# RadiativeTransfer/RadiativeTransfer.jl

Hardware: AMD Instinct MI355X
Metric: spectral points/sec (whole node), O2-A band IQU scene (higher is better)
Workload: dtype f64; 1 GPU; C2: N=60 (20 streams x 3 Stokes), Nz=40, M=3, S=10000/GPU (10000 in total), sum(ndoubl)=185, Lambertian surface, 3 VZA; collective=none, devices=one GPU per rank

## Files before the change

### include/momcore.h

```cpp
#ifndef MOMCORE_H
#define MOMCORE_H

#include <stddef.h>

#ifdef __cplusplus
extern "C" {
#endif

typedef struct mom_handle mom_t;

enum {
  MOM_OK = 0,
  MOM_EINVAL = -1,
  MOM_EHIP = -2,
  MOM_ESTATE = -3,
  MOM_ESINGULAR = -4,
  MOM_EUNSUPPORTED = -5
};

enum {
  MOM_ADDED_R_PM = 0, MOM_ADDED_R_MP = 1, MOM_ADDED_T_MM = 2, MOM_ADDED_T_PP = 3,
  MOM_ADDED_J0P = 4, MOM_ADDED_J0M = 5,
  MOM_COMP_R_MP = 6, MOM_COMP_R_PM = 7, MOM_COMP_T_PP = 8, MOM_COMP_T_MM = 9,
  MOM_COMP_J0P = 10, MOM_COMP_J0M = 11,
  MOM_SURF_R_PM = 12, MOM_SURF_R_MP = 13, MOM_SURF_T_MM = 14, MOM_SURF_T_PP = 15,
  MOM_SURF_J0P = 16, MOM_SURF_J0M = 17
};


int mom_create(mom_t **out, int device, int N, int nStokes, int S, int max_m, int dtype);
int mom_destroy(mom_t *h);
const char *mom_last_error(const mom_t *h);
const char *mom_last_global_error(void);
int mom_sync(mom_t *h);
int mom_check(mom_t *h);

int mom_set_streams(mom_t *h, const double *qp_muN, const double *wt_muN, int N, int imu0_1based, double mu0,
                    const double *I0, const double *D, int strict_reference_indexing);


int mom_elemental(mom_t *h, int m, int ndoubl, const double *tau_sum, const double *dtau, const double *varpi,
                  const double *Zpp, const double *Zmp, int z_batch);

int mom_doubling(mom_t *h, int ndoubl, double *expk);

int mom_interaction(mom_t *h, int iface, int with_surface_layer);

int mom_copy_added_to_composite(mom_t *h);

int mom_surface_lambertian(mom_t *h, int m, double albedo, const double *tau_tot);

int mom_elemental_inelastic_rrs(mom_t *h, int m, int ndoubl, int nRaman, const int *i_l1l0, const double *varpi_l1l0,
                                const double *fscattRayl, const double *tau_sum, const double *dtau, const double *varpi,
                                const double *Zpp_l1l0, const double *Zmp_l1l0, double *ier_mp, double *iet_pp,
                                double *ier_pm, double *iet_mm, double *ieJ0p, double *ieJ0m);

enum {
  MOM_IE_ADDED_R_PM = 18, MOM_IE_ADDED_R_MP = 19, MOM_IE_ADDED_T_MM = 20, MOM_IE_ADDED_T_PP = 21,
  MOM_IE_ADDED_J0P = 22, MOM_IE_ADDED_J0M = 23,
  MOM_IE_COMP_R_MP = 24, MOM_IE_COMP_R_PM = 25, MOM_IE_COMP_T_PP = 26, MOM_IE_COMP_T_MM = 27,
  MOM_IE_COMP_J0P = 28, MOM_IE_COMP_J0M = 29
};
int mom_rrs_set(mom_t *h, int nRaman, const int *i_l1l0, const double *varpi_l1l0, int rrs_strict_reference);
int mom_rrs_set_shard(mom_t *h, int nSpec_global, int n_glob0, int n1_lo, int n1_hi);
int mom_rrs_elemental(mom_t *h, int m, int ndoubl, const double *tau_sum, const double *dtau, const double *varpi,
                      const double *Zpp, const double *Zmp, const double *fscattRayl, const double *Zpp_l1l0,
                      const double *Zmp_l1l0);
int mom_rrs_doubling(mom_t *h, int ndoubl, double *expk);
int mom_rrs_interaction(mom_t *h, int iface, int with_surface_layer);
int mom_rrs_copy_added_to_composite(mom_t *h);
int mom_rrs_surface_lambertian(mom_t *h, int m, double albedo, const double *tau_tot);
int mom_rrs_upload(mom_t *h, int which, const double *src);
int mom_rrs_download(mom_t *h, int which, double *dst);
int mom_scene_set_rrs(mom_t *h, const double *fscattRayl, const double *Zpp_l1l0, const double *Zmp_l1l0);
int mom_rt_run_rrs(mom_t *h);
int mom_get_RT_rrs(mom_t *h, double *R_SFI, double *T_SFI, double *ieR_SFI, double *ieT_SFI, double *gpu_ms);
int mom_get_hdr_rrs(mom_t *h, double *hdr, double *bhr_uw, double *bhr_dw);
int mom_rrs_timers(mom_t *h, double *ms, int *launches, int n);
int mom_rrs_check_padding(mom_t *h, unsigned long long *violations);
size_t mom_rrs_spectra_count(mom_t *h, int per);
int mom_get_spectra_rrs_device(mom_t *h, int per, void *d_local);
int mom_allgather_rrs_device(mom_t *h, int per, void *d_global);

int mom_batch_inv(mom_t *h, int n, int batch, const double *A, double *X);
int mom_batched_mul(mom_t *h, int n, int batch, const double *A, const double *B, double *C);
int mom_batched_mul_dual(mom_t *h, int n, int batch, int P, const double *A, const double *dA, const double *B,
                         const double *dB, double *C, double *dC);
int mom_batch_inv_dual(mom_t *h, int n, int batch, int P, const double *A, const double *dA, double *X, double *dX);

int mom_upload(mom_t *h, int which, const double *src);
int mom_download(mom_t *h, int which, double *dst);

int mom_postprocess(mom_t *h, int m, int nVza, const int *node_1based, const double *vaz_deg, double weight,
                    double *R_SFI, double *T_SFI);

int mom_scene_set(mom_t *h, int Nz, int K, int M, const double *tau, const double *varpi, const double *zw,
                  const double *Zpp, const double *Zmp, const int *ndoubl, const int *iface, const double *tau_sum,
                  double albedo, int nVza, const int *node_1based, const double *cos_mphi, const double *sin_mphi);

int mom_absorption_begin(mom_t *h, int Nz, const double *grid);
int mom_absorption_set_lines(mom_t *h, int nLines, const double *nu0, const double *S0, const double *gamma_air,
                             const double *gamma_self, const double *E_lower, const double *n_air, const double *delta_air,
                             const double *sqrt_mol_weight, const int *iso_index, int nIso, int nTmax, const int *nT,
                             const double *tips_T, const double *tips_Q, const double *tips_z);
int mom_voigt_tau_abs_layer(mom_t *h, int iz_1based, double pressure, double temperature, double vmr, double wing_cutoff,
                            double factor);
int mom_voigt_tau_abs_profile(mom_t *h, int Nz, const double *pressure, const double *temperature, double vmr, double wing_cutoff,
                              const double *factor, double *gpu_ms);
int mom_absorption_get_prefactors(mom_t *h, int n, double *nu, double *gamma_d, double *y, double *S, int *ind_start_1based,
                                  int *ind_stop_1based);
int mom_voigt_tau_abs(mom_t *h, int iz_1based, int nLines, const double *nu, const double *gamma_d, const double *y,
                      const double *S, const int *ind_start_1based, const int *ind_stop_1based, double factor);
int mom_absorption_set(mom_t *h, int Nz, const double *tau_abs);
int mom_absorption_get(mom_t *h, double *tau_abs);
int mom_voigt_tau_abs_dual(mom_t *h, int iz_1based, int nLines, const double *nu, const double *gamma_d, const double *y,
                           const double *S, const double *dnu, const double *dgamma_d, const double *dy, const double *dS,
                           const int *ind_start_1based, const int *ind_stop_1based, double factor);
int mom_voigt_tau_abs_profile_dual(mom_t *h, int Nz, const double *pressure, const double *temperature, double vmr,
                                   double wing_cutoff, const double *factor, double *gpu_ms);
int mom_absorption_get_partials(mom_t *h, double *dtau_abs);
int mom_absorption_get_prefactor_partials(mom_t *h, int n, double *dnu, double *dgamma_d, double *dy, double *dS);
enum { MOM_BROADENING_VOIGT = 0, MOM_BROADENING_DOPPLER = 1, MOM_BROADENING_LORENTZ = 2 };
enum { MOM_CEF_HW32SD = 0, MOM_CEF_HW32VOIGT = 1 };
int mom_absorption_set_model(mom_t *h, int broadening, int cef);
int mom_lineshape_tau_abs(mom_t *h, int iz_1based, int nLines, const double *nu, const double *gamma_d, const double *gamma_l,
                          const double *y, const double *S, const int *ind_start_1based, const int *ind_stop_1based, double factor);
int mom_lineshape_tau_abs_dual(mom_t *h, int iz_1based, int nLines, const double *nu, const double *gamma_d, const double *gamma_l,
                               const double *y, const double *S, const double *dnu, const double *dgamma_d, const double *dgamma_l,
                               const double *dy, const double *dS, const int *ind_start_1based, const int *ind_stop_1based,
                               double factor);
int mom_absorption_get_gamma_l(mom_t *h, int n, double *gamma_l, double *dgamma_l);
int mom_scene_set_optics(mom_t *h, int Nz, int nAer, int M, const double *tau_rayl, double varpi_rayl,
                         const double *tau_aer, const double *omega_aer, const double *ft_aer, const double *Zpp,
                         const double *Zmp, double albedo, int nVza, const int *node_1based, const double *cos_mphi,
                         const double *sin_mphi);
int mom_scene_get_layers(mom_t *h, int *ndoubl, int *iface, double *tau, double *varpi, double *zw, double *tau_sum);
int mom_scene_set_optics_bands(mom_t *h, int Nz, int nAer, int nBand, const int *band_start, int M, const double *tau_rayl,
                               const double *varpi_rayl, const double *tau_aer, const double *omega_aer, const double *ft_aer,
                               const double *Zpp, const double *Zmp, double albedo, int nVza, const int *node_1based,
                               const double *cos_mphi, const double *sin_mphi);

int mom_scene_set_surface(mom_t *h, int kind, int M, const double *Rsurf, const double *albedo_spec);

int mom_rt_run(mom_t *h);

int mom_scene_set_partials(mom_t *h, int P, const double *dtau, const double *dvarpi, const double *dzw, const double *dZpp,
                           const double *dZmp, const double *dalbedo, const double *dRsurf, const double *dalbedo_spec);
int mom_rt_run_dual(mom_t *h);
int mom_get_RT_partials(mom_t *h, double *dR_SFI, double *dT_SFI);
int mom_get_hdr_partials(mom_t *h, double *dhdr, double *dbhr_uw, double *dbhr_dw);
int mom_scene_set_optics_partials(mom_t *h, int P, const double *w_abs, const double *w_rayl, const double *dtau_aer,
                                  const double *domega_aer, const double *dft_aer, const double *dZpp, const double *dZmp,
                                  const double *dalbedo, const double *dRsurf, const double *dalbedo_spec);
int mom_scene_get_partials(mom_t *h, double *dtau, double *dvarpi, double *dzw);
int mom_scene_set_optics_bands_partials(mom_t *h, int P, const double *w_abs, const double *w_rayl, const double *dtau_aer,
                                        const double *domega_aer, const double *dft_aer, const double *dZpp, const double *dZmp,
                                        const double *dalbedo, const double *dRsurf, const double *dalbedo_spec);

int mom_rt_run_multisensor(mom_t *h, int nSensors, const int *sensor_levels, double *uwJ, double *dwJ);

int mom_get_RT(mom_t *h, double *R_SFI, double *T_SFI);
int mom_get_hdr(mom_t *h, double *hdr, double *bhr_uw, double *bhr_dw);
int mom_get_RT_device(mom_t *h, void *dR_SFI, void *dT_SFI);

enum { MOM_COMM_ID_BYTES = 128 };
int mom_comm_unique_id(void *id_out, size_t bytes);
int mom_comm_init(mom_t *h, int rank, int nranks, const void *nccl_id);
int mom_comm_destroy(mom_t *h);
int mom_allgather(mom_t *h, const void *d_local, void *d_global, size_t count);
int mom_allgather_RT_device(mom_t *h, void *d_global);
int mom_allgather_RT(mom_t *h, double *R_SFI_global, double *T_SFI_global);

int mom_timers(mom_t *h, double *ms, int n, int *kernel_launches);

int mom_set_option(mom_t *h, int option, int value);

int mom_strip2_resumed(mom_t *h, int *units, int *left);
enum { MOM_OPT_INVERSE = 0, MOM_OPT_FORCE_GENERIC = 1, MOM_OPT_M0_REDUCTION = 2, MOM_OPT_SMALL_WG = 3, MOM_OPT_STAGGER = 4,
       MOM_OPT_SMALL_N = 5, MOM_OPT_LAYER_SWEEP = 6, MOM_OPT_STRIP_PAD = 7, MOM_OPT_LEAN = 8, MOM_OPT_OVERLAP = 9,
       MOM_OPT_RRS_KERNELS = 10, MOM_OPT_DUAL_WORKSPACE_MB = 11, MOM_OPT_STRIP2 = 12, MOM_OPT_STRIP2_SCHED = 13,
       MOM_OPT_ZERO_SKIP = 14, MOM_OPT_LUT_BATCH = 15, MOM_OPT_SOURCES_ONLY = 16, MOM_OPT_ELEMENTAL = 17 };

int mom_lut_create(mom_t *h, int nNu, double nu_first, double nu_step, int nP, double p_first, double p_step, int nT, double t_first,
                   double t_step, int *lut);
int mom_lut_set_table(mom_t *h, int lut, const double *sigma);
int mom_lut_build(mom_t *h, int lut, double vmr, double wing_cutoff, double *gpu_ms);
int mom_lut_get_table(mom_t *h, int lut, double *sigma);
int mom_lut_get_coefficients(mom_t *h, int lut, double *c);
int mom_lut_xsec(mom_t *h, int lut, int n, const double *nu, double p, double T, double *sigma, double *J);
int mom_lut_tau_abs_profile(mom_t *h, int lut, int Nz, const double *pressure, const double *temperature, const double *factor,
                            double *gpu_ms);
int mom_lut_tau_abs_profile_dual(mom_t *h, int lut, int Nz, const double *pressure, const double *temperature, const double *factor,
                                 double *gpu_ms);
int mom_lut_destroy(mom_t *h, int lut);

int mom_voigt_xsec(int device, int nLines, const double *nu, const double *gamma_d, const double *y,
                   const double *S, const int *ind_start_1based, const int *ind_stop_1based, int nGrid,
                   const double *grid, double *sigma);

int mom_voigt_xsec_dual(int device, int nLines, const double *nu, const double *gamma_d, const double *y, const double *S,
                        const double *dnu, const double *dgamma_d, const double *dy, const double *dS,
                        const int *ind_start_1based, const int *ind_stop_1based, int nGrid, const double *grid,
                        double *sigma, double *dsigma);

int mom_lineshape_xsec(int device, int broadening, int cef, int nLines, const double *nu, const double *gamma_d,
                       const double *gamma_l, const double *y, const double *S, const int *ind_start_1based,
                       const int *ind_stop_1based, int nGrid, const double *grid, double *sigma);

int mom_lineshape_xsec_dual(int device, int broadening, int cef, int nLines, const double *nu, const double *gamma_d,
                            const double *gamma_l, const double *y, const double *S, const double *dnu,
                            const double *dgamma_d, const double *dgamma_l, const double *dy, const double *dS,
                            const int *ind_start_1based, const int *ind_stop_1based, int nGrid, const double *grid,
                            double *sigma, double *dsigma);

double mom_voigt_last_kernel_ms(void);

enum { MOM_MIE_MAX_WEIGHT_ROWS = 4, MOM_MIE_FULL_K = 1 };
int mom_mie_nai2(int device, int nR, const double *r, int nW, const double *w, double lambda, double n_r, double n_i,
                 int n_mu, const double *w_mu, int n_max, const double *pi_tab, const double *tau_tab, int l_max,
                 const double *P, const double *P2, const double *R2, const double *T2, int flags, double *bulk_f,
                 double *C, double *greek, double *gpu_ms);

int mom_mie_coefficients(int device, int nX, const double *x, double n_r, double n_i, int n_max, double *a_re, double *a_im,
                         double *b_re, double *b_im);

enum { MOM_MIE_DUAL_MAX_WEIGHT_ROWS = 3, MOM_MIE_INDEX_ROWS = 2 };
int mom_mie_nai2_dual(int device, int nR, const double *r, int nW, const double *w, double lambda, double n_r, double n_i,
                      int n_mu, const double *w_mu, int n_max, const double *pi_tab, const double *tau_tab, int l_max,
                      const double *P, const double *P2, const double *R2, const double *T2, int flags, double *bulk_f,
                      double *C, double *greek, double *gpu_ms);

int mom_mie_coefficients_dual(int device, int nX, const double *x, double n_r, double n_i, int n_max, double *a_re, double *a_im,
                              double *b_re, double *b_im, double *da_re, double *da_im, double *db_re, double *db_im);

int mom_mie_tables(int device, int n_mu, const double *mu, int n_max, int l_max, double *pi_tab, double *tau_tab, double *P,
                   double *P2, double *R2, double *T2);

int mom_mie_nai2_spectral(int device, int nR, const double *r, int nW, const double *w, int nL, const double *lambda,
                          const double *n_r, const double *n_i, int n_mu, const double *mu, const double *w_mu, int n_max,
                          int l_max, int flags, int max_batch, double *bulk_f, double *C, double *greek, double *gpu_ms);

int mom_mie_nai2_spectral_dual(int device, int nR, const double *r, int nW, const double *w, int nL, const double *lambda,
                               const double *n_r, const double *n_i, int n_mu, const double *mu, const double *w_mu, int n_max,
                               int l_max, int flags, int max_batch, double *bulk_f, double *C, double *greek, double *gpu_ms);

enum { MOM_PCW_MAX_ORDER = 640 };
int mom_mie_pcw(int device, int nR, const double *r, const double *w, double lambda, double n_r, double n_i, int N_max, int flags,
                double *greek, double *C, double *gpu_ms);

enum { MOM_WIGNER_MAX_TABLE_BYTES = 1073741824 };
int mom_wigner_tables(int device, int m_max, int n_max, int l_max, double *A, double *B);

int mom_pcw_pair_averages(int device, int nR, const double *r, const double *w, double lambda, double n_r, double n_i, int N_max,
                          double *anam_re, double *anam_im, double *anbm_re, double *anbm_im, double *bnam_re, double *bnam_im,
                          double *bnbm_re, double *bnbm_im);

int mom_z_moments(int device, int nStokes, int n_mu, const double *mu, int nG, int l_pad, const int *l_max, const double *greek,
                  int m_first, int M, int set_inner, double *Zpp, double *Zmp, double *gpu_ms);

int mom_scene_stage_greeks(mom_t *h, int which, int nG, int l_pad, const int *l_max, const double *greek, int M);
int mom_scene_stage_greek_partials(mom_t *h, int P, int nD, const int *basis, const int *partial, int l_pad, const int *l_max,
                                   const double *dgreek);
int mom_scene_get_bases(mom_t *h, int which, int *edge, int *blocks, double *Zpp, double *Zmp);

#ifdef __cplusplus
}
#endif
#endif
```

### radiativetransfer.jl_amd/_lib.py

```python
from __future__ import annotations

import ctypes as C
import os
from pathlib import Path

import numpy as np

PKG_DIR = Path(__file__).resolve().parent
LIB_PATH = Path(os.environ["MOM_LIBRARY"]) if os.environ.get("MOM_LIBRARY") else PKG_DIR / "libmomcore.so"

c_dp = C.POINTER(C.c_double)
c_ip = C.POINTER(C.c_int)
c_h = C.c_void_p

MOM_OK, MOM_EINVAL, MOM_EHIP, MOM_ESTATE, MOM_ESINGULAR, MOM_EUNSUPPORTED = 0, -1, -2, -3, -4, -5
_CODES = {MOM_EINVAL: "MOM_EINVAL", MOM_EHIP: "MOM_EHIP", MOM_ESTATE: "MOM_ESTATE", MOM_ESINGULAR: "MOM_ESINGULAR",
          MOM_EUNSUPPORTED: "MOM_EUNSUPPORTED"}

ADDED = dict(r_pm=0, r_mp=1, t_mm=2, t_pp=3, j0p=4, j0m=5)
COMP = dict(R_mp=6, R_pm=7, T_pp=8, T_mm=9, J0p=10, J0m=11)
SURF = dict(r_pm=12, r_mp=13, t_mm=14, t_pp=15, j0p=16, j0m=17)
IE_ADDED = dict(ier_pm=18, ier_mp=19, iet_mm=20, iet_pp=21, ieJ0p=22, ieJ0m=23)
IE_COMP = dict(ieR_mp=24, ieR_pm=25, ieT_pp=26, ieT_mm=27, ieJ0p=28, ieJ0m=29)

MOM_OPT_INVERSE, MOM_OPT_FORCE_GENERIC, MOM_OPT_M0_REDUCTION, MOM_OPT_SMALL_WG, MOM_OPT_STAGGER, MOM_OPT_SMALL_N, MOM_OPT_LAYER_SWEEP = 0, 1, 2, 3, 4, 5, 6
MOM_OPT_STRIP_PAD = 7
MOM_OPT_LEAN = 8
MOM_OPT_OVERLAP = 9
MOM_OPT_RRS_KERNELS = 10
MOM_OPT_DUAL_WORKSPACE_MB = 11
MOM_OPT_STRIP2 = 12
MOM_OPT_STRIP2_SCHED = 13
MOM_OPT_ZERO_SKIP = 14
MOM_OPT_LUT_BATCH = 15
MOM_OPT_SOURCES_ONLY = 16
MOM_OPT_ELEMENTAL = 17

BROADENING_VOIGT, BROADENING_DOPPLER, BROADENING_LORENTZ = 0, 1, 2
CEF_HW32SD, CEF_HW32VOIGT = 0, 1
MOM_MIE_FULL_K = 1
MOM_PCW_MAX_ORDER, MOM_WIGNER_MAX_TABLE_BYTES = 640, 1 << 30
MOM_MIE_DUAL_MAX_WEIGHT_ROWS, MOM_MIE_INDEX_ROWS = 3, 2


class MomError(RuntimeError):
    def __init__(self, code, msg):
        super().__init__(f"{_CODES.get(code, code)}: {msg}")
        self.code = code


SIGNATURES = {
    "mom_create": (C.c_int, [C.POINTER(c_h), C.c_int, C.c_int, C.c_int, C.c_int, C.c_int, C.c_int]),
    "mom_destroy": (C.c_int, [c_h]),
    "mom_last_error": (C.c_char_p, [c_h]),
    "mom_last_global_error": (C.c_char_p, []),
    "mom_sync": (C.c_int, [c_h]),
    "mom_check": (C.c_int, [c_h]),
    "mom_set_streams": (C.c_int, [c_h, c_dp, c_dp, C.c_int, C.c_int, C.c_double, c_dp, c_dp, C.c_int]),
    "mom_elemental": (C.c_int, [c_h, C.c_int, C.c_int, c_dp, c_dp, c_dp, c_dp, c_dp, C.c_int]),
    "mom_doubling": (C.c_int, [c_h, C.c_int, c_dp]),
    "mom_interaction": (C.c_int, [c_h, C.c_int, C.c_int]),
    "mom_copy_added_to_composite": (C.c_int, [c_h]),
    "mom_surface_lambertian": (C.c_int, [c_h, C.c_int, C.c_double, c_dp]),
    "mom_elemental_inelastic_rrs": (C.c_int, [c_h, C.c_int, C.c_int, C.c_int, c_ip] + [c_dp] * 13),
    "mom_rrs_set": (C.c_int, [c_h, C.c_int, c_ip, c_dp, C.c_int]),
    "mom_rrs_set_shard": (C.c_int, [c_h, C.c_int, C.c_int, C.c_int, C.c_int]),
    "mom_rrs_elemental": (C.c_int, [c_h, C.c_int, C.c_int] + [c_dp] * 8),
    "mom_rrs_doubling": (C.c_int, [c_h, C.c_int, c_dp]),
    "mom_rrs_interaction": (C.c_int, [c_h, C.c_int, C.c_int]),
    "mom_rrs_copy_added_to_composite": (C.c_int, [c_h]),
    "mom_rrs_surface_lambertian": (C.c_int, [c_h, C.c_int, C.c_double, c_dp]),
    "mom_rrs_upload": (C.c_int, [c_h, C.c_int, c_dp]),
    "mom_rrs_download": (C.c_int, [c_h, C.c_int, c_dp]),
    "mom_scene_set_rrs": (C.c_int, [c_h, c_dp, c_dp, c_dp]),
    "mom_rt_run_rrs": (C.c_int, [c_h]),
    "mom_get_RT_rrs": (C.c_int, [c_h, c_dp, c_dp, c_dp, c_dp, c_dp]),
    "mom_get_hdr_rrs": (C.c_int, [c_h, c_dp, c_dp, c_dp]),
    "mom_rrs_timers": (C.c_int, [c_h, c_dp, c_ip, C.c_int]),
    "mom_batch_inv": (C.c_int, [c_h, C.c_int, C.c_int, c_dp, c_dp]),
    "mom_batched_mul": (C.c_int, [c_h, C.c_int, C.c_int, c_dp, c_dp, c_dp]),
    "mom_batched_mul_dual": (C.c_int, [c_h, C.c_int, C.c_int, C.c_int, c_dp, c_dp, c_dp, c_dp, c_dp, c_dp]),
    "mom_batch_inv_dual": (C.c_int, [c_h, C.c_int, C.c_int, C.c_int, c_dp, c_dp, c_dp, c_dp]),
    "mom_upload": (C.c_int, [c_h, C.c_int, c_dp]),
    "mom_download": (C.c_int, [c_h, C.c_int, c_dp]),
    "mom_scene_set": (C.c_int, [c_h, C.c_int, C.c_int, C.c_int, c_dp, c_dp, c_dp, c_dp, c_dp, c_ip, c_ip, c_dp,
                                C.c_double, C.c_int, c_ip, c_dp, c_dp]),
    "mom_absorption_begin": (C.c_int, [c_h, C.c_int, c_dp]),
    "mom_absorption_set_lines": (C.c_int, [c_h, C.c_int] + [c_dp] * 8 + [c_ip, C.c_int, C.c_int, c_ip, c_dp, c_dp, c_dp]),
    "mom_voigt_tau_abs_layer": (C.c_int, [c_h, C.c_int, C.c_double, C.c_double, C.c_double, C.c_double, C.c_double]),
    "mom_voigt_tau_abs_profile": (C.c_int, [c_h, C.c_int, c_dp, c_dp, C.c_double, C.c_double, c_dp, c_dp]),
    "mom_absorption_get_prefactors": (C.c_int, [c_h, C.c_int, c_dp, c_dp, c_dp, c_dp, c_ip, c_ip]),
    "mom_voigt_tau_abs": (C.c_int, [c_h, C.c_int, C.c_int, c_dp, c_dp, c_dp, c_dp, c_ip, c_ip, C.c_double]),
    "mom_absorption_set": (C.c_int, [c_h, C.c_int, c_dp]),
    "mom_absorption_get": (C.c_int, [c_h, c_dp]),
    "mom_voigt_tau_abs_dual": (C.c_int, [c_h, C.c_int, C.c_int] + [c_dp] * 8 + [c_ip, c_ip, C.c_double]),
    "mom_voigt_tau_abs_profile_dual": (C.c_int, [c_h, C.c_int, c_dp, c_dp, C.c_double, C.c_double, c_dp, c_dp]),
    "mom_absorption_get_partials": (C.c_int, [c_h, c_dp]),
    "mom_absorption_get_prefactor_partials": (C.c_int, [c_h, C.c_int, c_dp, c_dp, c_dp, c_dp]),
    "mom_absorption_set_model": (C.c_int, [c_h, C.c_int, C.c_int]),
    "mom_lineshape_tau_abs": (C.c_int, [c_h, C.c_int, C.c_int] + [c_dp] * 5 + [c_ip, c_ip, C.c_double]),
    "mom_lineshape_tau_abs_dual": (C.c_int, [c_h, C.c_int, C.c_int] + [c_dp] * 10 + [c_ip, c_ip, C.c_double]),
    "mom_absorption_get_gamma_l": (C.c_int, [c_h, C.c_int, c_dp, c_dp]),
    "mom_scene_set_optics": (C.c_int, [c_h, C.c_int, C.c_int, C.c_int, c_dp, C.c_double, c_dp, c_dp, c_dp, c_dp, c_dp,
                                       C.c_double, C.c_int, c_ip, c_dp, c_dp]),
    "mom_scene_set_optics_bands": (C.c_int, [c_h, C.c_int, C.c_int, C.c_int, c_ip, C.c_int, c_dp, c_dp, c_dp, c_dp, c_dp, c_dp, c_dp,
                                             C.c_double, C.c_int, c_ip, c_dp, c_dp]),
    "mom_scene_set_optics_bands_partials": (C.c_int, [c_h, C.c_int] + [c_dp] * 10),
    "mom_scene_get_layers": (C.c_int, [c_h, c_ip, c_ip, c_dp, c_dp, c_dp, c_dp]),
    "mom_scene_set_surface": (C.c_int, [c_h, C.c_int, C.c_int, c_dp, c_dp]),
    "mom_rt_run": (C.c_int, [c_h]),
    "mom_scene_set_partials": (C.c_int, [c_h, C.c_int] + [c_dp] * 8),
    "mom_scene_set_optics_partials": (C.c_int, [c_h, C.c_int] + [c_dp] * 10),
    "mom_scene_get_partials": (C.c_int, [c_h, c_dp, c_dp, c_dp]),
    "mom_rt_run_dual": (C.c_int, [c_h]),
    "mom_get_RT_partials": (C.c_int, [c_h, c_dp, c_dp]),
    "mom_get_hdr_partials": (C.c_int, [c_h, c_dp, c_dp, c_dp]),
    "mom_rt_run_multisensor": (C.c_int, [c_h, C.c_int, c_ip, c_dp, c_dp]),
    "mom_get_RT": (C.c_int, [c_h, c_dp, c_dp]),
    "mom_get_hdr": (C.c_int, [c_h, c_dp, c_dp, c_dp]),
    "mom_get_RT_device": (C.c_int, [c_h, C.c_void_p, C.c_void_p]),
    "mom_postprocess": (C.c_int, [c_h, C.c_int, C.c_int, c_ip, c_dp, C.c_double, c_dp, c_dp]),
    "mom_comm_unique_id": (C.c_int, [C.c_void_p, C.c_size_t]),
    "mom_comm_init": (C.c_int, [c_h, C.c_int, C.c_int, C.c_void_p]),
    "mom_comm_destroy": (C.c_int, [c_h]),
    "mom_allgather": (C.c_int, [c_h, C.c_void_p, C.c_void_p, C.c_size_t]),
    "mom_rrs_check_padding": (C.c_int, [c_h, C.POINTER(C.c_ulonglong)]),
    "mom_rrs_spectra_count": (C.c_size_t, [c_h, C.c_int]),
    "mom_get_spectra_rrs_device": (C.c_int, [c_h, C.c_int, C.c_void_p]),
    "mom_allgather_rrs_device": (C.c_int, [c_h, C.c_int, C.c_void_p]),
    "mom_allgather_RT_device": (C.c_int, [c_h, C.c_void_p]),
    "mom_allgather_RT": (C.c_int, [c_h, c_dp, c_dp]),
    "mom_timers": (C.c_int, [c_h, c_dp, C.c_int, c_ip]),
    "mom_set_option": (C.c_int, [c_h, C.c_int, C.c_int]),
    "mom_strip2_resumed": (C.c_int, [c_h, c_ip, c_ip]),
    "mom_lut_create": (C.c_int, [c_h, C.c_int, C.c_double, C.c_double, C.c_int, C.c_double, C.c_double, C.c_int, C.c_double, C.c_double,
                                 c_ip]),
    "mom_lut_set_table": (C.c_int, [c_h, C.c_int, c_dp]),
    "mom_lut_build": (C.c_int, [c_h, C.c_int, C.c_double, C.c_double, c_dp]),
    "mom_lut_get_table": (C.c_int, [c_h, C.c_int, c_dp]),
    "mom_lut_get_coefficients": (C.c_int, [c_h, C.c_int, c_dp]),
    "mom_lut_xsec": (C.c_int, [c_h, C.c_int, C.c_int, c_dp, C.c_double, C.c_double, c_dp, c_dp]),
    "mom_lut_tau_abs_profile": (C.c_int, [c_h, C.c_int, C.c_int, c_dp, c_dp, c_dp, c_dp]),
    "mom_lut_tau_abs_profile_dual": (C.c_int, [c_h, C.c_int, C.c_int, c_dp, c_dp, c_dp, c_dp]),
    "mom_lut_destroy": (C.c_int, [c_h, C.c_int]),
    "mom_voigt_xsec": (C.c_int, [C.c_int, C.c_int, c_dp, c_dp, c_dp, c_dp, c_ip, c_ip, C.c_int, c_dp, c_dp]),
    "mom_voigt_xsec_dual": (C.c_int, [C.c_int, C.c_int] + [c_dp] * 8 + [c_ip, c_ip, C.c_int, c_dp, c_dp, c_dp]),
    "mom_lineshape_xsec": (C.c_int, [C.c_int, C.c_int, C.c_int, C.c_int] + [c_dp] * 5 + [c_ip, c_ip, C.c_int, c_dp, c_dp]),
    "mom_lineshape_xsec_dual": (C.c_int, [C.c_int, C.c_int, C.c_int, C.c_int] + [c_dp] * 10 + [c_ip, c_ip, C.c_int, c_dp, c_dp, c_dp]),
    "mom_voigt_last_kernel_ms": (C.c_double, []),
    "mom_mie_nai2": (C.c_int, [C.c_int, C.c_int, c_dp, C.c_int, c_dp, C.c_double, C.c_double, C.c_double, C.c_int, c_dp, C.c_int, c_dp,
                               c_dp, C.c_int, c_dp, c_dp, c_dp, c_dp, C.c_int, c_dp, c_dp, c_dp, c_dp]),
    "mom_mie_coefficients": (C.c_int, [C.c_int, C.c_int, c_dp, C.c_double, C.c_double, C.c_int, c_dp, c_dp, c_dp, c_dp]),
    "mom_mie_nai2_dual": (C.c_int, [C.c_int, C.c_int, c_dp, C.c_int, c_dp, C.c_double, C.c_double, C.c_double, C.c_int, c_dp, C.c_int,
                                    c_dp, c_dp, C.c_int, c_dp, c_dp, c_dp, c_dp, C.c_int, c_dp, c_dp, c_dp, c_dp]),
    "mom_mie_coefficients_dual": (C.c_int, [C.c_int, C.c_int, c_dp, C.c_double, C.c_double, C.c_int] + [c_dp] * 8),
    "mom_mie_tables": (C.c_int, [C.c_int, C.c_int, c_dp, C.c_int, C.c_int] + [c_dp] * 6),
    "mom_mie_nai2_spectral": (C.c_int, [C.c_int, C.c_int, c_dp, C.c_int, c_dp, C.c_int, c_dp, c_dp, c_dp, C.c_int, c_dp, c_dp, C.c_int,
                                        C.c_int, C.c_int, C.c_int, c_dp, c_dp, c_dp, c_dp]),
    "mom_mie_nai2_spectral_dual": (C.c_int, [C.c_int, C.c_int, c_dp, C.c_int, c_dp, C.c_int, c_dp, c_dp, c_dp, C.c_int, c_dp, c_dp,
                                             C.c_int, C.c_int, C.c_int, C.c_int, c_dp, c_dp, c_dp, c_dp]),
    "mom_mie_pcw": (C.c_int, [C.c_int, C.c_int, c_dp, c_dp, C.c_double, C.c_double, C.c_double, C.c_int, C.c_int, c_dp, c_dp, c_dp]),
    "mom_wigner_tables": (C.c_int, [C.c_int, C.c_int, C.c_int, C.c_int, c_dp, c_dp]),
    "mom_pcw_pair_averages": (C.c_int, [C.c_int, C.c_int, c_dp, c_dp, C.c_double, C.c_double, C.c_double, C.c_int] + [c_dp] * 8),
    "mom_z_moments": (C.c_int, [C.c_int, C.c_int, C.c_int, c_dp, C.c_int, C.c_int, c_ip, c_dp, C.c_int, C.c_int, C.c_int, c_dp, c_dp, c_dp]),
    "mom_scene_stage_greeks": (C.c_int, [c_h, C.c_int, C.c_int, C.c_int, c_ip, c_dp, C.c_int]),
    "mom_scene_stage_greek_partials": (C.c_int, [c_h, C.c_int, C.c_int, c_ip, c_ip, C.c_int, c_ip, c_dp]),
    "mom_scene_get_bases": (C.c_int, [c_h, C.c_int, c_ip, c_ip, c_dp, c_dp]),
}

_lib = None


def load():
    global _lib
    if _lib is not None:
        return _lib
    if not LIB_PATH.exists():
        raise MomError(MOM_EHIP, f"{LIB_PATH} not found - build it with `make -C {PKG_DIR / 'csrc'}` "
                                 "(hipcc --offload-arch=gfx950); there is no CPU fallback")
    lib = C.CDLL(str(LIB_PATH))
    for name, (res, args) in SIGNATURES.items():
        fn = getattr(lib, name)
        fn.restype = res
        fn.argtypes = args
    _lib = lib
    return lib


def f64(a):
    return np.ascontiguousarray(a, dtype=np.float64)


def i32(a):
    return np.ascontiguousarray(a, dtype=np.int32)


def dp(a: np.ndarray):
    assert a.dtype == np.float64 and a.flags["C_CONTIGUOUS"]
    return a.ctypes.data_as(c_dp)


def ip(a: np.ndarray):
    assert a.dtype == np.int32 and a.flags["C_CONTIGUOUS"]
    return a.ctypes.data_as(c_ip)


class Handle:

    def __init__(self, N: int, nStokes: int, S: int, max_m: int = 1, device: int = 0, dtype: int = 0):
        self.lib = load()
        self.N, self.nS, self.S, self.M = int(N), int(nStokes), int(S), int(max_m)
        self._h = c_h()
        rc = self.lib.mom_create(C.byref(self._h), device, self.N, self.nS, self.S, self.M, int(dtype))
        if rc != MOM_OK:
            msg = self.lib.mom_last_global_error().decode()
            if self._h:
                self.lib.mom_destroy(self._h)
                self._h = c_h()
            raise MomError(rc, msg)

    def check(self, rc):
        if rc != MOM_OK:
            raise MomError(rc, self.lib.mom_last_error(self._h).decode())

    def close(self):
        if getattr(self, "_h", None):
            self.lib.mom_destroy(self._h)
            self._h = c_h()

    def __del__(self):
        try:
            self.close()
        except Exception:
            pass

    def __enter__(self):
        return self

    def __exit__(self, *a):
        self.close()

    def set_option(self, option, value):
        self.check(self.lib.mom_set_option(self._h, option, value))

    def sync(self):
        self.check(self.lib.mom_sync(self._h))

    def check_async(self):
        self.check(self.lib.mom_check(self._h))

    def set_streams(self, qp_muN, wt_muN, imu0_1based, mu0, I0, D, strict=True):
        qp, wt, I0, D = f64(qp_muN), f64(wt_muN), f64(I0), f64(D)
        self.check(self.lib.mom_set_streams(self._h, dp(qp), dp(wt), len(qp), int(imu0_1based), float(mu0), dp(I0),
                                            dp(D), 1 if strict else 0))

    def elemental(self, m, nd, tau_sum, dtau, varpi, Zpp, Zmp, z_batch):
        a = [f64(x) for x in (tau_sum, dtau, varpi, Zpp, Zmp)]
        self.check(self.lib.mom_elemental(self._h, int(m), int(nd), *[dp(x) for x in a], int(z_batch)))

    def doubling(self, nd, expk):
        e = f64(expk).copy()
        self.check(self.lib.mom_doubling(self._h, int(nd), dp(e)))
        return e

    def interaction(self, iface, with_surface_layer=False):
        self.check(self.lib.mom_interaction(self._h, int(iface), 1 if with_surface_layer else 0))

    def copy_added_to_composite(self):
        self.check(self.lib.mom_copy_added_to_composite(self._h))

    def surface_lambertian(self, m, albedo, tau_tot):
        t = f64(tau_tot)
        self.check(self.lib.mom_surface_lambertian(self._h, int(m), float(albedo), dp(t)))

    def upload(self, which, src):
        s = f64(src).reshape(-1)
        self.check(self.lib.mom_upload(self._h, int(which), dp(s)))

    def download(self, which):
        k = which % 6
        out = np.empty((self.N * self.N if k < 4 else self.N) * self.S)
        self.check(self.lib.mom_download(self._h, int(which), dp(out)))
        return out

    def elemental_inelastic_rrs(self, m, ndoubl, i_l1l0, varpi_l1l0, fscatt, tau_sum, dtau, varpi, Zpp, Zmp):
        il = i32(i_l1l0)
        nR = len(il)
# ... 289 lines not shown
                               cos_mphi, sin_mphi):
        bs = i32(np.asarray(band_start).reshape(-1))
        nBand = bs.size - 1
        tr = np.ascontiguousarray(np.asarray(tau_rayl, dtype=np.float64).T).reshape(-1)
        ta = np.asarray(tau_aer, dtype=np.float64)
        nAer = ta.shape[1] if ta.ndim == 3 and ta.size else 0
        vr = f64(varpi_rayl).reshape(-1)
        taf = np.ascontiguousarray(ta.transpose(0, 2, 1)).reshape(-1) if nAer else np.zeros(1)
        om, ft = (f64(omega_aer).reshape(-1), f64(ft_aer).reshape(-1)) if nAer else (np.zeros(1), np.zeros(1))
        assert vr.size == max(nBand, 1) and (not nAer or (ta.shape[0] == nBand and om.size == ft.size == nBand * nAer))
        zp, zm = (None if z is None else dp(f64(z).reshape(-1)) for z in (Zpp, Zmp))
        node = i32(node)
        cm, sm = f64(cos_mphi).reshape(-1), f64(sin_mphi).reshape(-1)
        self.nVza = len(node)
        self._Nz, self._K = int(Nz), 1 + nAer * nBand
        self.check(self.lib.mom_scene_set_optics_bands(self._h, int(Nz), nAer, nBand, ip(bs), int(M), dp(tr), dp(vr), dp(taf), dp(om),
                                                       dp(ft), zp, zm, float(albedo), len(node), ip(node), dp(cm), dp(sm)))

    def scene_stage_greeks(self, greeks, M, which=0):
        nG, l_pad, l_max, greek = pack_greeks(greeks, "scene_stage_greeks")
        self.check(self.lib.mom_scene_stage_greeks(self._h, int(which), nG, l_pad, ip(l_max), dp(greek), int(M)))

    def scene_stage_greek_partials(self, P, pairs):
        nD, l_pad, l_max, greek = pack_greeks([g for _, g in pairs], "scene_stage_greek_partials")
        basis, partial = i32([kp[0] for kp, _ in pairs]), i32([kp[1] for kp, _ in pairs])
        self.check(self.lib.mom_scene_stage_greek_partials(self._h, int(P), nD, ip(basis), ip(partial), l_pad, ip(l_max), dp(greek)))

    def scene_get_bases(self, which=0):
        e, b = np.zeros(1, dtype=np.int32), np.zeros(1, dtype=np.int32)
        self.check(self.lib.mom_scene_get_bases(self._h, int(which), ip(e), ip(b), None, None))
        edge, blocks = int(e[0]), int(b[0])
        Zpp, Zmp = np.empty((blocks, edge, edge)), np.empty((blocks, edge, edge))
        if Zpp.size:
            self.check(self.lib.mom_scene_get_bases(self._h, int(which), ip(e), ip(b), dp(Zpp), dp(Zmp)))
        return edge, Zpp, Zmp

    def scene_get_layers(self, Nz, K, arrays=True):
        nd, iface = np.zeros(Nz, dtype=np.int32), np.zeros(Nz, dtype=np.int32)
        S = self.S
        bufs = [np.empty(S * Nz), np.empty(S * Nz), np.empty(K * S * Nz), np.empty(S * (Nz + 1))] if arrays else [None] * 4
        self.check(self.lib.mom_scene_get_layers(self._h, ip(nd), ip(iface), *[dp(b) if b is not None else None for b in bufs]))
        return (nd, iface) + tuple(bufs)

    def scene_set_surface(self, kind, M=0, Rsurf=None, albedo_spec=None):
        r = f64(Rsurf).reshape(-1) if Rsurf is not None else None
        al = f64(albedo_spec).reshape(-1) if albedo_spec is not None else None
        self.check(self.lib.mom_scene_set_surface(self._h, int(kind), int(M), dp(r) if r is not None else None,
                                                  dp(al) if al is not None else None))

    def rt_run(self):
        self.check(self.lib.mom_rt_run(self._h))

    def scene_set_partials(self, P, dtau=None, dvarpi=None, dzw=None, dZpp=None, dZmp=None, dalbedo=None, dRsurf=None,
                           dalbedo_spec=None):
        bufs = [None if x is None else f64(x).reshape(-1) for x in (dtau, dvarpi, dzw, dZpp, dZmp, dalbedo, dRsurf, dalbedo_spec)]
        self.dual_P = int(P)
        self.check(self.lib.mom_scene_set_partials(self._h, int(P), *[None if b is None else dp(b) for b in bufs]))

    def scene_set_optics_partials(self, P, w_abs=None, w_rayl=None, dtau_aer=None, domega_aer=None, dft_aer=None, dZpp=None,
                                  dZmp=None, dalbedo=None, dRsurf=None, dalbedo_spec=None):
        bufs = [None if x is None else f64(x).reshape(-1)
                for x in (w_abs, w_rayl, dtau_aer, domega_aer, dft_aer, dZpp, dZmp, dalbedo, dRsurf, dalbedo_spec)]
        self.check(self.lib.mom_scene_set_optics_partials(self._h, int(P), *[None if b is None else dp(b) for b in bufs]))
        self.dual_P = int(P)

    def scene_set_optics_bands_partials(self, P, w_abs=None, w_rayl=None, dtau_aer=None, domega_aer=None, dft_aer=None, dZpp=None,
                                        dZmp=None, dalbedo=None, dRsurf=None, dalbedo_spec=None):
        bufs = [None if x is None else f64(x).reshape(-1)
                for x in (w_abs, w_rayl, dtau_aer, domega_aer, dft_aer, dZpp, dZmp, dalbedo, dRsurf, dalbedo_spec)]
        self.check(self.lib.mom_scene_set_optics_bands_partials(self._h, int(P), *[None if b is None else dp(b) for b in bufs]))
        self.dual_P = int(P)

    def scene_get_partials(self):
        P, S, Nz, K = getattr(self, "dual_P", 0), self.S, getattr(self, "_Nz", 1), getattr(self, "_K", 1)
        n = max(P * S * Nz, 1)
        dt, dv, dz = np.empty(n), np.empty(n), np.empty(K * n)
        self.check(self.lib.mom_scene_get_partials(self._h, dp(dt), dp(dv), dp(dz)))
        tr = lambda a: np.transpose(a.reshape(P, Nz, S), (0, 2, 1)).copy()
        return tr(dt), tr(dv), np.transpose(dz.reshape(P, Nz, S, K), (0, 3, 2, 1)).copy()

    def rt_run_dual(self):
        self.check(self.lib.mom_rt_run_dual(self._h))

    def get_RT_partials(self):
        P = self.dual_P
        n = self.nVza * self.nS * self.S * P
        dR, dT = np.empty(n), np.empty(n)
        self.check(self.lib.mom_get_RT_partials(self._h, dp(dR), dp(dT)))
        shp = (P, self.S, self.nS, self.nVza)
        return np.transpose(dR.reshape(shp), (0, 3, 2, 1)).copy(), np.transpose(dT.reshape(shp), (0, 3, 2, 1)).copy()

    def get_hdr_partials(self):
        P = self.dual_P
        n, f = self.nVza * self.nS * self.S * P, self.nS * self.S * P
        dH, up, dw = np.empty(n), np.empty(f), np.empty(f)
        self.check(self.lib.mom_get_hdr_partials(self._h, dp(dH), dp(up), dp(dw)))
        tr = lambda x: np.transpose(x.reshape(P, self.S, self.nS), (0, 2, 1)).copy()
        return np.transpose(dH.reshape(P, self.S, self.nS, self.nVza), (0, 3, 2, 1)).copy(), tr(up), tr(dw)

    def rt_run_multisensor(self, sensor_levels):
        lv = np.ascontiguousarray(sensor_levels, dtype=np.int32)
        n = self.nVza * self.nS * self.S * len(lv)
        uw, dw = np.empty(n), np.empty(n)
        self.check(self.lib.mom_rt_run_multisensor(self._h, len(lv), ip(lv), dp(uw), dp(dw)))
        shp = (len(lv), self.S, self.nS, self.nVza)
        tr = lambda a: np.transpose(a.reshape(shp), (0, 3, 2, 1)).copy()
        return tr(uw), tr(dw)

    def get_RT(self):
        n = self.nVza * self.nS * self.S
        R, T = np.empty(n), np.empty(n)
        self.check(self.lib.mom_get_RT(self._h, dp(R), dp(T)))
        shp = (self.S, self.nS, self.nVza)
        return np.transpose(R.reshape(shp), (2, 1, 0)).copy(), np.transpose(T.reshape(shp), (2, 1, 0)).copy()

    def get_hdr(self):
        n = self.nVza * self.nS * self.S
        H, up, dw = np.empty(n), np.empty(self.nS * self.S), np.empty(self.nS * self.S)
        self.check(self.lib.mom_get_hdr(self._h, dp(H), dp(up), dp(dw)))
        return (np.transpose(H.reshape(self.S, self.nS, self.nVza), (2, 1, 0)).copy(),
                up.reshape(self.S, self.nS).T.copy(), dw.reshape(self.S, self.nS).T.copy())

    def get_RT_device(self, dR_ptr: int, dT_ptr: int):
        self.check(self.lib.mom_get_RT_device(self._h, C.c_void_p(dR_ptr), C.c_void_p(dT_ptr)))

    def postprocess(self, m, node_1based, vaz_deg, weight, R_SFI, T_SFI):
        node, vaz = i32(node_1based), f64(vaz_deg)
        self.check(self.lib.mom_postprocess(self._h, int(m), len(node), ip(node), dp(vaz), float(weight), dp(R_SFI),
                                            dp(T_SFI)))

    def comm_init(self, rank: int, nranks: int, nccl_id: bytes):
        buf = C.create_string_buffer(bytes(nccl_id), COMM_ID_BYTES)
        self.check(self.lib.mom_comm_init(self._h, int(rank), int(nranks), C.cast(buf, C.c_void_p)))
        self.comm_size = int(nranks)

    def comm_destroy(self):
        self.check(self.lib.mom_comm_destroy(self._h))

    def allgather_RT_device(self, d_global_ptr: int):
        self.check(self.lib.mom_allgather_RT_device(self._h, C.c_void_p(d_global_ptr)))

    def allgather_RT(self):
        n = self.nVza * self.nS * self.S * self.comm_size
        R, T = np.empty(n), np.empty(n)
        self.check(self.lib.mom_allgather_RT(self._h, dp(R), dp(T)))
        shp = (self.S * self.comm_size, self.nS, self.nVza)
        return np.transpose(R.reshape(shp), (2, 1, 0)).copy(), np.transpose(T.reshape(shp), (2, 1, 0)).copy()

    def strip2_resumed(self):
        u, l = C.c_int(0), C.c_int(0)
        self.check(self.lib.mom_strip2_resumed(self._h, C.byref(u), C.byref(l)))
        return u.value, l.value

    def timers(self):
        ms = np.zeros(8)
        nl = C.c_int(0)
        self.check(self.lib.mom_timers(self._h, dp(ms), 8, C.byref(nl)))
        return dict(layers_ms=ms[0], surface_ms=ms[1], postprocess_ms=ms[2], total_ms=ms[3], layer_launches=nl.value,
                    full_layers_ms=ms[4], reduced_layers_ms=ms[5], full_launches=int(ms[6]), reduced_launches=int(ms[7]))


COMM_ID_BYTES = 128


def comm_unique_id() -> bytes:
    buf = C.create_string_buffer(COMM_ID_BYTES)
    rc = load().mom_comm_unique_id(C.cast(buf, C.c_void_p), COMM_ID_BYTES)
    if rc != MOM_OK:
        raise MomError(rc, load().mom_last_global_error().decode())
    return buf.raw


def voigt_xsec(nu, gamma_d, y, S, ind_start, ind_stop, grid, device: int = 0):
    lib = load()
    a = [f64(x) for x in (nu, gamma_d, y, S)]
    i0, i1, g = i32(ind_start), i32(ind_stop), f64(grid)
    sigma = np.empty(len(g))
    rc = lib.mom_voigt_xsec(device, len(a[0]), *[dp(x) for x in a], ip(i0), ip(i1), len(g), dp(g), dp(sigma))
    if rc != MOM_OK:
        raise MomError(rc, lib.mom_last_global_error().decode())
    return sigma


def _partials(x, n):
    if x is None:
        return None
    x = np.asarray(x, dtype=np.float64)
    assert x.shape == (n, 2), f"partials must be [nLines, 2], got {x.shape}"
    return np.ascontiguousarray(x.T).reshape(-1)


def voigt_xsec_dual(nu, gamma_d, y, S, dnu, dgamma_d, dy, dS, ind_start, ind_stop, grid, device: int = 0):
    lib = load()
    a = [f64(x) for x in (nu, gamma_d, y, S)]
    d = [_partials(x, len(a[0])) for x in (dnu, dgamma_d, dy, dS)]
    i0, i1, g = i32(ind_start), i32(ind_stop), f64(grid)
    sigma, dsigma = np.empty(len(g)), np.empty(2 * len(g))
    rc = lib.mom_voigt_xsec_dual(device, len(a[0]), *[dp(x) for x in a], *[None if x is None else dp(x) for x in d], ip(i0), ip(i1),
                                 len(g), dp(g), dp(sigma), dp(dsigma))
    if rc != MOM_OK:
        raise MomError(rc, lib.mom_last_global_error().decode())
    return sigma, dsigma.reshape(2, len(g)).T.copy()


def lineshape_xsec(broadening, cef, nu, gamma_d, gamma_l, y, S, ind_start, ind_stop, grid, device: int = 0):
    lib = load()
    a = [None if x is None else f64(x) for x in (nu, gamma_d, gamma_l, y, S)]
    i0, i1, g = i32(ind_start), i32(ind_stop), f64(grid)
    sigma = np.empty(len(g))
    rc = lib.mom_lineshape_xsec(device, int(broadening), int(cef), len(a[0]), *[None if x is None else dp(x) for x in a], ip(i0),
                                ip(i1), len(g), dp(g), dp(sigma))
    if rc != MOM_OK:
        raise MomError(rc, lib.mom_last_global_error().decode())
    return sigma


def lineshape_xsec_dual(broadening, cef, nu, gamma_d, gamma_l, y, S, dnu, dgamma_d, dgamma_l, dy, dS, ind_start, ind_stop, grid,
                        device: int = 0):
    lib = load()
    a = [None if x is None else f64(x) for x in (nu, gamma_d, gamma_l, y, S)]
    d = [_partials(x, len(a[0])) for x in (dnu, dgamma_d, dgamma_l, dy, dS)]
    i0, i1, g = i32(ind_start), i32(ind_stop), f64(grid)
    sigma, dsigma = np.empty(len(g)), np.empty(2 * len(g))
    rc = lib.mom_lineshape_xsec_dual(device, int(broadening), int(cef), len(a[0]), *[None if x is None else dp(x) for x in a],
                                     *[None if x is None else dp(x) for x in d], ip(i0), ip(i1), len(g), dp(g), dp(sigma), dp(dsigma))
    if rc != MOM_OK:
        raise MomError(rc, lib.mom_last_global_error().decode())
    return sigma, dsigma.reshape(2, len(g)).T.copy()


def voigt_last_kernel_ms() -> float:
    return float(load().mom_voigt_last_kernel_ms())


def _mie_nai2(dual: bool, r, w, lam, n_r, n_i, w_mu, pi_tab, tau_tab, P, P2, R2, T2, flags, device):
    lib = load()
    name = "mie_nai2_dual" if dual else "mie_nai2"
    r, w, w_mu = f64(r), f64(np.atleast_2d(w)), f64(w_mu)
    tabs = [f64(np.asarray(t, dtype=np.float64).T) for t in (pi_tab, tau_tab, P, P2, R2, T2)]
    nW, nR, n_mu = w.shape[0], len(r), len(w_mu)
    if w.shape[1] != nR or any(t.shape[1] != n_mu for t in tabs) or tabs[0].shape != tabs[1].shape or \
            any(t.shape != tabs[2].shape for t in tabs[3:]):
        raise ValueError(f"{name}: array shapes do not agree")
    n_max, l_max = tabs[0].shape[0], tabs[2].shape[0]
    nO = nW + MOM_MIE_INDEX_ROWS if dual else nW
    bulk, Cx, greek, ms = np.empty((nO, 4, n_mu)), np.empty((nO, 2)), np.empty((nO, 6, l_max)), np.zeros(3)
    fn = lib.mom_mie_nai2_dual if dual else lib.mom_mie_nai2
    rc = fn(device, nR, dp(r), nW, dp(w), float(lam), float(n_r), float(n_i), n_mu, dp(w_mu), n_max, dp(tabs[0]), dp(tabs[1]), l_max,
            *[dp(t) for t in tabs[2:]], int(flags), dp(bulk), dp(Cx), dp(greek), dp(ms))
    if rc != MOM_OK:
        raise MomError(rc, lib.mom_last_global_error().decode())
    return bulk, Cx, greek, ms


def mie_nai2(r, w, lam, n_r, n_i, w_mu, pi_tab, tau_tab, P, P2, R2, T2, flags: int = 0, device: int = 0):
    return _mie_nai2(False, r, w, lam, n_r, n_i, w_mu, pi_tab, tau_tab, P, P2, R2, T2, flags, device)


def mie_nai2_dual(r, w, lam, n_r, n_i, w_mu, pi_tab, tau_tab, P, P2, R2, T2, flags: int = 0, device: int = 0):
    return _mie_nai2(True, r, w, lam, n_r, n_i, w_mu, pi_tab, tau_tab, P, P2, R2, T2, flags, device)


def mie_coefficients(x, n_r, n_i, n_max: int, device: int = 0):
    lib = load()
    x = f64(np.atleast_1d(x))
    out = [np.empty((int(n_max), len(x))) for _ in range(4)]
    rc = lib.mom_mie_coefficients(device, len(x), dp(x), float(n_r), float(n_i), int(n_max), *[dp(o) for o in out])
    if rc != MOM_OK:
        raise MomError(rc, lib.mom_last_global_error().decode())
    return out[0] + 1j * out[1], out[2] + 1j * out[3]


def mie_coefficients_dual(x, n_r, n_i, n_max: int, device: int = 0):
    lib = load()
    x = f64(np.atleast_1d(x))
    out = [np.empty((int(n_max), len(x))) for _ in range(8)]
    rc = lib.mom_mie_coefficients_dual(device, len(x), dp(x), float(n_r), float(n_i), int(n_max), *[dp(o) for o in out])
    if rc != MOM_OK:
        raise MomError(rc, lib.mom_last_global_error().decode())
    return out[0] + 1j * out[1], out[2] + 1j * out[3], out[4] + 1j * out[5], out[6] + 1j * out[7]


def mie_tables(mu, n_max: int, l_max: int, device: int = 0):
    lib = load()
    mu = f64(np.atleast_1d(mu))
    n_mu, n_max, l_max = len(mu), int(n_max), int(l_max)
    out = [np.empty((max(n_max, 0), n_mu)) for _ in range(2)] + [np.empty((max(l_max, 0), n_mu)) for _ in range(4)]
    rc = lib.mom_mie_tables(device, n_mu, dp(mu), n_max, l_max, *[dp(o) for o in out])
    if rc != MOM_OK:
        raise MomError(rc, lib.mom_last_global_error().decode())
    return tuple(o.T for o in out)


def _mie_nai2_spectral(dual: bool, r, w, lam, n_r, n_i, mu, w_mu, n_max, l_max, flags, max_batch, device):
    lib = load()
    name = "mie_nai2_spectral_dual" if dual else "mie_nai2_spectral"
    r, w, mu, w_mu = f64(r), f64(np.atleast_2d(w)), f64(mu), f64(w_mu)
    lam, n_r, n_i = (f64(np.atleast_1d(a)) for a in (lam, n_r, n_i))
    nW, nR, n_mu, nL, l_max = w.shape[0], len(r), len(w_mu), len(lam), int(l_max)
    if w.shape[1] != nR or len(mu) != n_mu or len(n_r) != nL or len(n_i) != nL:
        raise ValueError(f"{name}: array shapes do not agree")
    nO = nW + MOM_MIE_INDEX_ROWS if dual else nW
    bulk, Cx = np.empty((nL, nO, 4, n_mu)), np.empty((nL, nO, 2))
    greek, ms = np.empty((nL, nO, 6, max(l_max, 0))), np.zeros(4)
    fn = lib.mom_mie_nai2_spectral_dual if dual else lib.mom_mie_nai2_spectral
    rc = fn(device, nR, dp(r), nW, dp(w), nL, dp(lam), dp(n_r), dp(n_i), n_mu, dp(mu), dp(w_mu), int(n_max), l_max, int(flags),
# ... 83 lines not shown
```

### radiativetransfer.jl_amd/csrc/mom_handle.hpp

```cpp
#pragma once
#include <hip/hip_runtime.h>

#include <algorithm>
#include <cmath>
#include <cstdio>
#include <cstdlib>
#include <string>
#include <vector>

#include "momcore.h"

#include "mom_diag.hpp"
#include "mom_entry.hpp"
#include "mom_host.hpp"

namespace momr { struct State; }

struct MomLut {
  bool live = false;
  int n[3] = {};
  double first[3] = {}, step[3] = {};
  bool has_table = false, has_coef = false;
  MomDevBuf<double> d_table;
  MomDevBuf<double> d_coef;
  MomDevBuf<double> d_nu;
};

struct MomGreekStage {
  bool live = false;
  int nG = 0, l_pad = 0, M = 0, P = 0;
  std::vector<int> l_max, basis, partial;
  std::vector<double> greek;
  void drop() { *this = MomGreekStage{}; }
};

struct mom_handle : MomSceneBufs<double> {
  int device = 0, N = 0, nS = 0, S = 0, M = 0;
  int dtype = 0;
  momf_scene *f32 = nullptr;
  bool lds_mode = true;
  int opt_inverse = 0, opt_force_generic = 0;
  hipStream_t stream = nullptr;
  mom::DevStreams q{};
  bool streams_set = false;
  std::vector<double> h_mu, h_wt;
  int strict = 1;
  MomDevBuf<double> added[6], surf[6], comp[6];
  bool op_layers = false;
  bool comp_pitched = false;
  bool comp_on_chip = false;
  MomDevBuf<double> d_post;
  void *comm = nullptr;
  int comm_rank = 0, comm_size = 1;
  MomDevBuf<double> d_gather;
  MomDevBuf<double> d_rrs_send;
  MomDevBuf<double> d_tau_abs, d_grid, d_lines, d_tau_rayl, d_layer_max, d_aer;
  MomDevBuf<int> d_aer_mode;
  int abs_Nz = 0;
  size_t lines_per = 0;
  int lines_nz = 1;
  int abs_broadening = 0, abs_cef = 0;
  MomDevBuf<double> d_prof;
  MomDevBuf<double> d_dtau_abs;
  MomDevBuf<double> d_dlines;
  bool optics_scene = false;
  bool optics_tables = false;
  int optics_nAer = 0;
  int optics_nBand = 0;
  std::vector<double> h_varpi_rayl;
  std::vector<double> h_tau_aer, h_omega_aer, h_ft_aer;
  MomDevBuf<int> d_band_start;
  MomDevBuf<double> d_varpi_band;
  MomDevBuf<double> d_optics_prm;
  MomDevBuf<double> d_vec[4];
  MomDevBuf<double> d_Zop[2];
  bool scene_set = false;
  MomGreekStage stage_z, stage_r, stage_d;
  int opt_m0 = 1;
  int opt_w4 = 1;
  int opt_stagger = 1;
  int opt_rrs_kernels = -1;
  int opt_overlap = 1;
  hipStream_t stream2 = nullptr;
  hipEvent_t ev_fork = nullptr, ev_join = nullptr, ev_go = nullptr;
  int dual_P = 0;
  bool dual_ran = false;
  MomDevBuf<double> d_dual_in[8];
  MomDevBuf<double> d_dual_out, d_dual_ts;
  MomDevBuf<char> dual_work;
  size_t opt_dual_budget = 0;
  MomDevBuf<double> d_Rsurf0;
  int opt_sweep = 1;
  MomDevBuf<double> comp_top[6];
  MomDevBuf<double> d_msJ[2];
  std::vector<MomDevBuf<double>> ms_comp;
  MomDevBuf<double> d_ms_out;
  int opt_pad = 1;
  int opt_lean = 3;
  MomDevBuf<int> d_resume;
  int opt_strip2 = 1;
  MomDevBuf<int> d_resume2;
  size_t resume2_units = 0;
  int resume2_nz = 0;
  int opt_strip2_sched = 1;
  MomDevBuf<int> d_sched2;
  int opt_zero_skip = 7;
  int opt_sources_only = 1;
  int opt_elemental = 1;
  MomDevBuf<double> d_etab, d_etab0;
  int nbw_0 = 0;
  int Nk = 0;
  mom::DevStreams qk{};
  int opt_small = 1;
  bool red0 = false;
  int N0 = 0, nS0 = 0;
  mom::DevStreams q0{};
  MomDevBuf<double> d_mu0, d_wt0, d_sg0, d_Zpp0, d_Zmp0, d_hdrJ0, d_scratch0;
  MomDevBuf<double> comp0[6];
  int G = 0;
  int num_cu = 256;
  MomDevBuf<int> d_info;
  hipEvent_t ev[4] = {};
  hipEvent_t ev_voigt[2] = {};
  std::vector<hipEvent_t> ev_full, ev_red;
  int launches = 0, launches_full = 0, launches_red = 0;
  momr::State *rrs = nullptr;
  MomDevBuf<double> d_fscatt, d_Zr[2];
  MomDevBuf<double> d_rrs_op[8];
  bool rrs_scene = false;
  double rrs_ms = 0.0;
  MomDevBuf<char> ws[4];
  MomLineTable lt{};
  MomDevBuf<double> d_lt;
  MomDevBuf<int> d_lt_i;
  double lt_Tmin = 0.0, lt_Tmax = 0.0;
  std::vector<MomLut> luts;
  MomDevBuf<double> d_lut_cp;
  MomDevBuf<double> d_lut_prm;
  MomDevBuf<double> d_lut_io;
  int opt_lut_batch = 0;
  double grid_min = 0.0, grid_max = 0.0;
  int grid_order = 0;
  std::string err;
};

#pragma GCC visibility push(hidden)
int fail(mom_t *h, int code, const char *msg);
int check_info(mom_t *h);
inline int mom_absorption_state(mom_t *h, const char *fn, bool table, bool lines) {
  const bool no_table = table && (!h->d_tau_abs || !h->d_grid);
  if (!no_table && !(lines && !h->d_lt)) return MOM_OK;
  char buf[200];
  snprintf(buf, sizeof buf, no_table ? "%s: call mom_absorption_begin with the spectral grid first" : "%s: call mom_absorption_set_lines first", fn);
  return fail(h, MOM_ESTATE, buf);
}
inline int mom_tips_range(mom_t *h, double T) {
  if (h->lt.nIso <= 0 || (h->lt_Tmin < T && T < h->lt_Tmax)) return MOM_OK;
  char buf[160];
  snprintf(buf, sizeof buf, "TIPS2017: T (%g) must be between %g K and %g K.", T, h->lt_Tmin, h->lt_Tmax);
  return fail(h, MOM_EINVAL, buf);
}
hipError_t mom_launch_combine(const mom::InterArgs &a, bool lds, int grid, size_t smem, hipStream_t st);
int scene_common(mom_t *h, int Nz, int K, int M, const double *Zpp, const double *Zmp, double albedo, int nVza,
                 const int *node_1based, const double *cos_mphi, const double *sin_mphi);
int mom_stage_claim(mom_t *h, const char *fn, int K, int M);
extern void (*g_rccl_destroy)(void *);
int mom_comm_allreduce_max(mom_t *h, double *d_buf, size_t count);
#pragma GCC visibility pop

#define HIPCHK(h, call)                                                                            \
  do {                                                                                             \
    hipError_t e__ = (call);                                                                       \
    if (e__ != hipSuccess) {                                                                       \
      char buf__[512];                                                                             \
      snprintf(buf__, sizeof buf__, "%s failed: %s (%s:%d)", #call, hipGetErrorString(e__), __FILE__, __LINE__); \
      return fail(h, MOM_EHIP, buf__);                                                             \
    }                                                                                              \
  } while (0)

#define F64_ONLY(h, name)                                                                                 \
  if ((h) && (h)->dtype != 0)                                                                             \
  return fail(h, MOM_EINVAL, name ": not available on a Float32 (dtype = 1) handle (scene-level path only)")
```

### radiativetransfer.jl_amd/csrc/mom_image_variants.hpp

```cpp
#pragma once
#include "mom_images.hpp"

constexpr int kSkipVariants = 4;
constexpr int kS2Skip[kSkipVariants] = {0, 1, 2, 3};
constexpr int kQ4Skip[kSkipVariants] = {0, 1, 2, 4};

inline int mom_skip_variant(const int (&skip)[kSkipVariants], int KS, int nbw) {
  if (nbw < 1 || nbw > KS) return 0;
  int v = 0;
  for (int c = 1; c < kSkipVariants; ++c)
    if (KS - skip[c] >= nbw) v = c;
  return v;
}
constexpr bool s2_row_blocks_change(int KS, int KW) { return KW < KS || 4 * ((KS + 3) / 4) - 1 > KS; }
inline bool s2_row_blocks_for(int KS, const MomLaunchForm &f) {
  return f.row_blocks && s2_row_blocks_change(KS, KS - kS2Skip[mom_skip_variant(kS2Skip, KS, f.nbw)]);
}
```

### radiativetransfer.jl_amd/csrc/mom_images.hpp

```cpp
#pragma once
#include <hip/hip_runtime.h>

#include <cstddef>

struct MomLaunchForm {
  int nbw = 0;
  bool row_blocks = false;
  bool sources_only = false;
  bool elemental_tab = false;
  int sched_mode = 0;
};

struct MomLayerImage {
  int N;
  hipError_t (*launch)(const void *layer_args, const MomLaunchForm &form, int grid, hipStream_t st);
  size_t (*lds_bytes)(int ns, int nS, int K);
  int (*per_cu)();
};

enum MomImageFamily {
  MOM_IMG_STRIP8,
  MOM_IMG_STRIP4,
  MOM_IMG_LEAN,
  MOM_IMG_LEAN6,
  MOM_IMG_STRIP2,
  MOM_IMG_QUAD,
  MOM_IMG_F32_STRIP8,
  MOM_IMG_F32_STRIP4,
};

#define MOM_IMAGE_LIST(X)                                                                                \
  X(STRIP8, 11) X(STRIP8, 13) X(STRIP8, 14) X(STRIP8, 15)                                               \
  X(STRIP4, 9) X(STRIP4, 10) X(STRIP4, 11)                                                              \
  X(LEAN, 9) X(LEAN, 10)                                                                                \
  X(LEAN6, 9) X(LEAN6, 10)                                                                              \
  X(STRIP2, 13) X(STRIP2, 14) X(STRIP2, 15)                                                             \
  X(QUAD, 5) X(QUAD, 6) X(QUAD, 7) X(QUAD, 8) X(QUAD, 9) X(QUAD, 10)                                    \
  X(F32_STRIP8, 11) X(F32_STRIP8, 13) X(F32_STRIP8, 14) X(F32_STRIP8, 15)                               \
  X(F32_STRIP4, 9) X(F32_STRIP4, 10) X(F32_STRIP4, 11) X(F32_STRIP4, 13) X(F32_STRIP4, 14) X(F32_STRIP4, 15)

#define MOM_IMAGE_SYM_(F, KS) mom_image_##F##_##KS
#define MOM_IMAGE_SYM(F, KS) MOM_IMAGE_SYM_(F, KS)
#define MOM_DEFINE_IMAGE(F, KS, ...)                                 \
  const MomLayerImage *MOM_IMAGE_SYM(F, KS)() {                      \
    static const MomLayerImage image = {4 * (KS), __VA_ARGS__};      \
    return &image;                                                   \
  }

#define MOM_IMAGE_DECL(F, KS) const MomLayerImage *MOM_IMAGE_SYM_(F, KS)();
MOM_IMAGE_LIST(MOM_IMAGE_DECL)
#undef MOM_IMAGE_DECL

inline const MomLayerImage *mom_find_image(MomImageFamily family, int N) {
  struct Entry { MomImageFamily family; const MomLayerImage *image; };
#define MOM_IMAGE_ENTRY(F, KS) {MOM_IMG_##F, MOM_IMAGE_SYM_(F, KS)()},
  static const Entry all[] = {MOM_IMAGE_LIST(MOM_IMAGE_ENTRY)};
#undef MOM_IMAGE_ENTRY
  for (const Entry &e : all)
    if (e.family == family && e.image->N == N) return e.image;
  return nullptr;
}

constexpr size_t kMomStrip2SchedInts = 1 + 2048;
```

### radiativetransfer.jl_amd/csrc/mom_q4.hpp

```cpp
#pragma once
#include "mom_entry.hpp"
#include "mom_elemental_tab.hpp"

namespace MOM_NS {

static_assert(kWaves == 1, "mom_q4.hpp: one wavefront per workgroup (-DMOM_WAVES=1)");

__device__ __forceinline__ real mma4(real a, real b, real c) { return __builtin_amdgcn_mfma_f64_4x4x4f64(a, b, c, 0, 0, 0); }

#ifndef Q4_MUL_VARIANT
#define Q4_MUL_VARIANT 0
#endif
template <int KS>
struct Q4Geom {
  static constexpr int N = 4 * KS, NB = KS, NJ = (KS + 3) / 4, LD = N;
  static constexpr int CP = 16 * ((N + 15) / 16);
};
__host__ __device__ inline size_t q4_lds_bytes(int N) { return ((size_t)3 * N * N + 8 * (size_t)N) * sizeof(real); }
__host__ __device__ inline bool q4_applies(int N, int ns, int K) {
  const int Nq = N / (ns > 0 ? ns : 1);
  return kF64 && N >= 20 && N <= 40 && N % 4 == 0 && ns >= 2 && N % ns == 0 && K <= 60 &&
         3 * Nq * Nq + 2 * ns * N + 3 + K <= N * N &&
         4 * q4_lds_bytes(N) <= kLdsPerCU;
}

struct Q4Lane {
  int k, c16;
  __device__ __forceinline__ Q4Lane() {
    int l = wg_lane();
    asm volatile("" : "+v"(l));
    k = l >> 4;
    c16 = l & 15;
  }
};

template <int KS> using Q4Mat = real[Q4Geom<KS>::NB][Q4Geom<KS>::NJ];

template <int KS>
__device__ __forceinline__ void q4_zero(real (&W)[Q4Geom<KS>::NB][Q4Geom<KS>::NJ]) {
#pragma unroll
  for (int K = 0; K < Q4Geom<KS>::NB; ++K)
#pragma unroll
    for (int J = 0; J < Q4Geom<KS>::NJ; ++J) W[K][J] = 0.0;
}
template <int KS>
__device__ __forceinline__ void q4_copy(real (&D)[Q4Geom<KS>::NB][Q4Geom<KS>::NJ], const real (&S)[Q4Geom<KS>::NB][Q4Geom<KS>::NJ]) {
#pragma unroll
  for (int K = 0; K < Q4Geom<KS>::NB; ++K)
#pragma unroll
    for (int J = 0; J < Q4Geom<KS>::NJ; ++J) D[K][J] = S[K][J];
}

template <int KS>
__device__ __forceinline__ void q4_load_T(const real *X, const Q4Lane &q, real (&W)[Q4Geom<KS>::NB][Q4Geom<KS>::NJ]) {
  using G = Q4Geom<KS>;
  const real *base = X + q.c16 + q.k * G::LD;
#pragma unroll
  for (int K = 0; K < G::NB; ++K)
#pragma unroll
    for (int J = 0; J < G::NJ; ++J) W[K][J] = (16 * J + q.c16 < G::N) ? base[16 * J + 4 * K * G::LD] : 0.0;
}
template <int KS>
__device__ __forceinline__ void q4_store_T(real *X, const Q4Lane &q, const real (&W)[Q4Geom<KS>::NB][Q4Geom<KS>::NJ]) {
  using G = Q4Geom<KS>;
  real *base = X + q.c16 + q.k * G::LD;
#pragma unroll
  for (int K = 0; K < G::NB; ++K)
#pragma unroll
    for (int J = 0; J < G::NJ; ++J)
      if (16 * J + q.c16 < G::N) base[16 * J + 4 * K * G::LD] = W[K][J];
}
template <int KS>
__device__ __forceinline__ void q4_load_glb_T(const gdouble *__restrict__ X, const Q4Lane &q, real (&W)[Q4Geom<KS>::NB][Q4Geom<KS>::NJ]) {
  using G = Q4Geom<KS>;
  const gdouble *base = X + q.c16 + q.k * G::CP;
#pragma unroll
  for (int K = 0; K < G::NB; ++K)
#pragma unroll
    for (int J = 0; J < G::NJ; ++J) W[K][J] = (16 * J + q.c16 < G::N) ? MOM_NT_LOAD(base + 16 * J + 4 * K * G::CP) : 0.0;
}
template <int KS>
__device__ __forceinline__ void q4_store_glb_T(gdouble *__restrict__ X, const Q4Lane &q, const real (&W)[Q4Geom<KS>::NB][Q4Geom<KS>::NJ]) {
  using G = Q4Geom<KS>;
  gdouble *base = X + q.c16 + q.k * G::CP;
#pragma unroll
  for (int K = 0; K < G::NB; ++K)
#pragma unroll
    for (int J = 0; J < G::NJ; ++J)
      if (16 * J + q.c16 < G::N) MOM_NT_STORE(W[K][J], base + 16 * J + 4 * K * G::CP);
}

template <int KS, int NV = 0, bool ZERO = false, int NBW = Q4Geom<KS>::NB>
__device__ __forceinline__ void q4_mul_c(const real *M, const real (&X)[Q4Geom<KS>::NB][Q4Geom<KS>::NJ],
                                         const real (&C0)[Q4Geom<KS>::NB][Q4Geom<KS>::NJ],
                                         real (&acc)[Q4Geom<KS>::NB][Q4Geom<KS>::NJ], const real *ride = nullptr,
                                         real (*accR)[Q4Geom<KS>::NJ] = nullptr) {
  using G = Q4Geom<KS>;
  static_assert(NBW >= 1 && NBW <= G::NB, "q4_mul_c: 1 <= NBW <= NB");
  constexpr int NZ = G::NB - NBW;
  int l = wg_lane();
  asm volatile("" : "+v"(l));
  const int k = l >> 4, i = l & 3;
  const real *base = M + k + i * G::LD;
#define Q4_XLIVE(K, J) ((K) < NBW || (J) == ((K) >> 2))
#if Q4_MUL_VARIANT == 2
#pragma unroll
  for (int I = 0; I < G::NB; ++I) {
    if (I >= NBW) {
#pragma unroll
      for (int J = 0; J < G::NJ; ++J) acc[I][J] = ZERO ? (real)0 : C0[I][J];
    }
#pragma unroll
    for (int K = 0; K < G::NB; ++K) {
      if (I >= NBW && K != I) continue;
      const real a = base[4 * K + 4 * I * G::LD];
#pragma unroll
      for (int J = 0; J < G::NJ; ++J)
        if (Q4_XLIVE(K, J)) acc[I][J] = mma4(a, X[K][J], (I < NBW && K == 0) ? (ZERO ? (real)0 : C0[I][J]) : acc[I][J]);
    }
  }
  if constexpr (NV > 0) {
    const real *rb = ride + k + i * G::N;
#pragma unroll
    for (int K = 0; K < G::NB; ++K) {
      const real a = (i < NV) ? rb[4 * K] : 0.0;
#pragma unroll
      for (int J = 0; J < G::NJ; ++J)
        if (Q4_XLIVE(K, J)) (*accR)[J] = mma4(a, X[K][J], (*accR)[J]);
    }
  }
  return;
#endif
  constexpr int NP = (NBW + 1) / 2;
  real an[2][G::NB];
  const real *rb = NV > 0 ? ride + k + i * G::N : nullptr;
#pragma unroll
  for (int h = 0; h < 2; ++h)
#pragma unroll
    for (int K = 0; K < G::NB; ++K) {
      if (h < NBW) an[h][K] = base[4 * K + 4 * h * G::LD];
      else if (NV > 0 && h == NBW) an[h][K] = (i < NV) ? rb[4 * K] : 0.0;
      else an[h][K] = 0.0;
    }
  real ad[NZ > 0 ? NZ : 1];
#pragma unroll
  for (int d = 0; d < NZ; ++d) ad[d] = base[4 * (NBW + d) + 4 * (NBW + d) * G::LD];
#pragma unroll
  for (int Pp = 0; Pp < NP; ++Pp) {
    const int I0 = 2 * Pp;
    const bool two = I0 + 1 < NBW;
    real ac[2][G::NB];
#pragma unroll
    for (int h = 0; h < 2; ++h)
#pragma unroll
      for (int K = 0; K < G::NB; ++K) ac[h][K] = an[h][K];
#pragma unroll
    for (int h = 0; h < 2; ++h) {
      const int In = I0 + 2 + h;
      if (In < NBW) {
#pragma unroll
        for (int K = 0; K < G::NB; ++K) an[h][K] = base[4 * K + 4 * In * G::LD];
      } else if (NV > 0 && In == NBW) {
#pragma unroll
        for (int K = 0; K < G::NB; ++K) an[h][K] = (i < NV) ? rb[4 * K] : 0.0;
      }
    }
#if Q4_MUL_VARIANT != 1
    __builtin_amdgcn_sched_barrier(0);
#endif
#pragma unroll
    for (int K = 0; K < G::NB; ++K) {
#pragma unroll
      for (int J = 0; J < G::NJ; ++J)
        if (Q4_XLIVE(K, J)) acc[I0][J] = mma4(ac[0][K], X[K][J], K == 0 ? (ZERO ? (real)0 : C0[I0][J]) : acc[I0][J]);
      if (two) {
#pragma unroll
        for (int J = 0; J < G::NJ; ++J)
          if (Q4_XLIVE(K, J)) acc[I0 + 1][J] = mma4(ac[1][K], X[K][J], K == 0 ? (ZERO ? (real)0 : C0[I0 + 1][J]) : acc[I0 + 1][J]);
      } else if (NV > 0) {
#pragma unroll
        for (int J = 0; J < G::NJ; ++J)
          if (Q4_XLIVE(K, J)) (*accR)[J] = mma4(ac[1][K], X[K][J], (*accR)[J]);
      }
    }
#if Q4_MUL_VARIANT != 1
    __builtin_amdgcn_sched_barrier(0);
#endif
  }
  if constexpr (NV > 0 && (NBW % 2) == 0) {
#pragma unroll
    for (int K = 0; K < G::NB; ++K) {
#pragma unroll
      for (int J = 0; J < G::NJ; ++J)
        if (Q4_XLIVE(K, J)) (*accR)[J] = mma4(an[0][K], X[K][J], (*accR)[J]);
    }
  }
#pragma unroll
  for (int d = 0; d < NZ; ++d) {
    const int I = NBW + d;
#pragma unroll
    for (int J = 0; J < G::NJ; ++J) {
      const real c0 = ZERO ? (real)0 : C0[I][J];
      acc[I][J] = (J == (I >> 2)) ? mma4(ad[d], X[I][J], c0) : c0;
    }
  }
#undef Q4_XLIVE
}

template <int KS, int NV, int NBW = Q4Geom<KS>::NB>
__device__ __forceinline__ void q4_ride(const real *ride, const real (&X)[Q4Geom<KS>::NB][Q4Geom<KS>::NJ], real (&accR)[Q4Geom<KS>::NJ]) {
  using G = Q4Geom<KS>;
  static_assert(NV >= 1 && NBW >= 1 && NBW <= G::NB, "q4_ride: NV >= 1, 1 <= NBW <= NB");
  int l = wg_lane();
  asm volatile("" : "+v"(l));
  const int k = l >> 4, i = l & 3;
  const real *rb = ride + k + i * G::N;
  real a[G::NB];
#pragma unroll
  for (int K = 0; K < G::NB; ++K) a[K] = (i < NV) ? rb[4 * K] : 0.0;
#pragma unroll
  for (int K = 0; K < G::NB; ++K)
#pragma unroll
    for (int J = 0; J < G::NJ; ++J)
      if (K < NBW || J == (K >> 2)) accR[J] = mma4(a[K], X[K][J], accR[J]);
}

template <int KS, int NV = 0, int NBW = Q4Geom<KS>::NB>
__device__ __forceinline__ void q4_mul(const real *M, const real (&X)[Q4Geom<KS>::NB][Q4Geom<KS>::NJ],
                                       real (&acc)[Q4Geom<KS>::NB][Q4Geom<KS>::NJ], const real *ride = nullptr,
                                       real (*accR)[Q4Geom<KS>::NJ] = nullptr) {
  q4_mul_c<KS, NV, false, NBW>(M, X, acc, acc, ride, accR);
}
template <int KS, int NV = 0, int NBW = Q4Geom<KS>::NB>
__device__ __forceinline__ void q4_mul_z(const real *M, const real (&X)[Q4Geom<KS>::NB][Q4Geom<KS>::NJ],
                                         real (&acc)[Q4Geom<KS>::NB][Q4Geom<KS>::NJ], const real *ride = nullptr,
                                         real (*accR)[Q4Geom<KS>::NJ] = nullptr) {
  q4_mul_c<KS, NV, true, NBW>(M, X, acc, acc, ride, accR);
}

#ifndef Q4_HORNER_SITES
#define Q4_HORNER_SITES 1
#endif
template <int KS, int NBW = Q4Geom<KS>::NB>
__device__ __forceinline__ void q4_horner(const real *M, const real (&C0)[Q4Geom<KS>::NB][Q4Geom<KS>::NJ], int p,
                                          real (&Y)[Q4Geom<KS>::NB][Q4Geom<KS>::NJ]) {
  q4_copy<KS>(Y, C0);
  MOM_STAMP(82);
#if Q4_HORNER_SITES == 2
  int n = p - 1;
#pragma nounroll
  for (; n >= 2; n -= 2) {
    real Z[Q4Geom<KS>::NB][Q4Geom<KS>::NJ];
    q4_mul_c<KS, 0, false, NBW>(M, Y, C0, Z);
    q4_mul_c<KS, 0, false, NBW>(M, Z, C0, Y);
  }
  if (n == 1) {
    real acc[Q4Geom<KS>::NB][Q4Geom<KS>::NJ];
    q4_mul_c<KS, 0, false, NBW>(M, Y, C0, acc);
    q4_copy<KS>(Y, acc);
  }
#else
#pragma nounroll
  for (int kk = 1; kk < p; ++kk) {
    real acc[Q4Geom<KS>::NB][Q4Geom<KS>::NJ];
    MOM_STAMP(74);
    q4_mul_c<KS, 0, false, NBW>(M, Y, C0, acc);
#ifdef MOM_DIAG_STAMPS
    if (kk == 1) { MOM_STAMP(75); } else { MOM_STAMP(77); }
    if (threadIdx.x == 0 && blockIdx.x == (gridDim.x >> 1)) mom_diag_acc[kk == 1 ? 78 : 79] += 1;
#endif
    q4_copy<KS>(Y, acc);
    MOM_STAMP(76);
  }
#endif
}

template <int KS>
__device__ __forceinline__ unsigned q4_sign_mask(const real *sg, const Q4Lane &q) {
  unsigned m = 0;
#pragma unroll
  for (int K = 0; K < Q4Geom<KS>::NB; ++K)
    if (sg[4 * K + q.k] < 0.0) m |= 1u << K;
  return m;
}
template <int KS>
__device__ __forceinline__ void q4_flip(real (&W)[Q4Geom<KS>::NB][Q4Geom<KS>::NJ], unsigned mask) {
#pragma unroll
  for (int K = 0; K < Q4Geom<KS>::NB; ++K)
#pragma unroll
    for (int J = 0; J < Q4Geom<KS>::NJ; ++J) {
      const real v = W[K][J];
      W[K][J] = ((mask >> K) & 1u) ? -v : v;
    }
}
__device__ __forceinline__ void q4_fence() { __builtin_amdgcn_fence(__ATOMIC_ACQ_REL, "workgroup"); __builtin_amdgcn_s_barrier(); }

__device__ __forceinline__ real q4_wave_sum(real v) {
  union { real d; int w[2]; } a, b;
#define Q4_DPP_ADD(ctrl)                                                                      \
  a.d = v;                                                                                    \
  b.w[0] = __builtin_amdgcn_update_dpp(0, a.w[0], ctrl, 0xf, 0xf, false);                     \
  b.w[1] = __builtin_amdgcn_update_dpp(0, a.w[1], ctrl, 0xf, 0xf, false);                     \
  v += b.d;
  Q4_DPP_ADD(0x111)
  Q4_DPP_ADD(0x112)
  Q4_DPP_ADD(0x114)
  Q4_DPP_ADD(0x118)
#undef Q4_DPP_ADD
  a.d = v;
  real s = 0.0;
#pragma unroll
  for (int row = 0; row < 4; ++row) {
    union { real d; int w[2]; } t;
    t.w[0] = __builtin_amdgcn_readlane(a.w[0], 16 * row + 15);
    t.w[1] = __builtin_amdgcn_readlane(a.w[1], 16 * row + 15);
    s += t.d;
  }
  return s;
}

__device__ __forceinline__ void make_ctx_q4(Ctx &c, int N, int inv_mode, real *smem) {
  c.N = N; c.Np = N; c.nc = N; c.ld = N; c.ldv = N;
  c.fd.init(N);
  c.inv_mode = inv_mode;
  c.qpre = 0; c.slot = 0; c.ptab = nullptr;
  const size_t msz = (size_t)N * N;
  c.r = smem; c.t = smem + msz; c.P = smem + 2 * msz; c.Q = nullptr; c.X = nullptr;
  real *p = smem + 3 * msz;
  c.mu = p; c.wt = p + N; c.sg = p + 2 * N; c.jp = p + 3 * N; c.jm = p + 4 * N; c.ei = p + 5 * N; c.v1 = p + 6 * N; c.v2 = p + 7 * N;
  c.j1p = c.j1m = c.Jp = c.Jm = c.prow = c.pcol = c.rowk = c.part = c.thr = nullptr;
  c.ipiv = c.sh = nullptr;
  c.bad = reinterpret_cast<int *>(c.P + msz - 2);
  c.tabE = c.tabZS = nullptr;
}

template <int KS, int NBW = Q4Geom<KS>::NB>
__device__ __forceinline__ real doubling_run_q4(Ctx &c, int nd, real expk, bool &bail) {
  using G = Q4Geom<KS>;
  constexpr int N = G::N, NB = G::NB, NJ = G::NJ;
  bail = false;
  if (nd == 0) return expk;
  const Q4Lane q;
  real *r = c.r, *t = c.t, *P = c.P;
  for (int it = 0; it < nd; ++it) {
    real rj[NJ];
    real ss = 0.0;
    real Rn[NB][NJ], T0[NB][NJ];
    q4_load_T<KS>(r, q, Rn);
    q4_load_T<KS>(t, q, T0);
    {
      real B[NB][NJ];
#pragma unroll
      for (int J = 0; J < NJ; ++J) rj[J] = 0.0;
      q4_mul_z<KS, 2, NBW>(r, Rn, B, c.jp, &rj);
#pragma unroll
      for (int K = 0; K < NB; ++K)
#pragma unroll
        for (int J = 0; J < NJ; ++J) ss += B[K][J] * B[K][J];
      q4_store_T<KS>(P, q, B);
    }
    MOM_STAMP(70);
    ss = q4_wave_sum(ss);
    const int p = __builtin_amdgcn_readfirstlane(neumann_terms_12(ss));
    if (p > kStripMaxP || c.inv_mode != 0) {
      bail = true;
      return expk;
    }
    MOM_STAMP(80);
#pragma unroll
    for (int J = 0; J < NJ; ++J) {
      const int col = 16 * J + q.c16;
      if (col < N) {
        if (q.k == 0) c.ei[col] = c.jm[col] * expk + rj[J];
        if (q.k == 1) c.v1[col] = c.jp[col] + expk * rj[J];
      }
    }
    q4_fence();
    MOM_STAMP(81);
    real Y[NB][NJ];
    q4_horner<KS, NBW>(P, T0, p, Y);
    MOM_STAMP(71);
    real aw[NJ];
    real Tn[NB][NJ];
    {
      real Zt[NB][NJ];
#pragma unroll
      for (int J = 0; J < NJ; ++J) aw[J] = 0.0;
      q4_mul_z<KS, 2, NBW>(r, Y, Zt, c.ei, &aw);
      q4_mul<KS, 0, NBW>(t, Zt, Rn);
    }
    q4_mul_z<KS, 0, NBW>(t, Y, Tn);
    const bool last = (it == nd - 1);
#pragma unroll
    for (int J = 0; J < NJ; ++J) {
      const int col = 16 * J + q.c16;
      const real sc = (last && col < N) ? c.sg[col] : 1.0;
#pragma unroll
      for (int K = 0; K < NB; ++K) Rn[K][J] = Rn[K][J] * sc;
      if (col < N) {
        if (q.k == 0) c.jm[col] = (c.jm[col] + aw[J]) * sc;
        if (q.k == 1) c.jp[col] = c.jp[col] * expk + aw[J];
      }
    }
    q4_store_T<KS>(r, q, Rn);
    q4_store_T<KS>(t, q, Tn);
    q4_fence();
    MOM_STAMP(72);
    expk = expk * expk;
  }
  MOM_STAMP(73);
  return expk;
}

template <int KS, int NBW = Q4Geom<KS>::NB, bool SRC = false>
__device__ __forceinline__ bool interaction_q4(Ctx &c, const CompPtrs &g) {
  using G = Q4Geom<KS>;
  constexpr int N = G::N, NB = G::NB, NJ = G::NJ, NN = N * N;
  const Q4Lane q;
  const int lane = wg_lane();
  real *r = c.r, *t = c.t, *P = c.P;
  {
    constexpr int U = (NN + 63) / 64;
    real vr[U];
#pragma unroll
    for (int u = 0; u < U; ++u) {
      const int e = lane + 64 * u;
      if (e < NN) {
        int i, j;
        c.fd.split(e, i, j);
        vr[u] = MOM_NT_LOAD(g.R_pm + i + j * G::CP);
      }
    }
#pragma unroll
    for (int u = 0; u < U; ++u) {
      const int e = lane + 64 * u;
      if (e < NN) P[e] = vr[u];
    }
  }
  q4_fence();
  MOM_STAMP(50);
  real W0[NB][NJ];
  real ss = 0.0;
  {
    real Bs[NB][NJ];
    {
      real rT[NB][NJ];
      q4_load_T<KS>(r, q, rT);
      q4_mul_z<KS, 0, NBW>(P, rT, Bs);
    }
#pragma unroll
    for (int K = 0; K < NB; ++K)
#pragma unroll
      for (int J = 0; J < NJ; ++J) ss += Bs[K][J] * Bs[K][J];
    {
      real tT[NB][NJ];
      q4_load_T<KS>(t, q, tT);
      q4_mul_z<KS, 0, NBW>(P, tT, W0);
    }
    q4_fence();
    q4_store_T<KS>(P, q, Bs);
  }
  q4_fence();
  ss = q4_wave_sum(ss);
  const int p = __builtin_amdgcn_readfirstlane(neumann_terms_12(ss));
  if (p > kStripMaxP) return false;
  MOM_STAMP(52);
  const unsigned mask = q4_sign_mask<KS>(c.sg, q);
  real Y1[NB][NJ], Y2[NB][NJ];
  constexpr int UT = (NN + 63) / 64;
  real vt[UT], vj;
  {
    real T1[NB][NJ];
    q4_load_glb_T<KS>(g.T_mm, q, T1);
    __builtin_amdgcn_sched_barrier(0);
    q4_horner<KS, NBW>(P, W0, p, Y2);
    if constexpr (!SRC) {
#pragma unroll
      for (int u = 0; u < UT; ++u) {
        const int e = lane + 64 * u;
        if (e < NN) {
          int i, j;
          c.fd.split(e, i, j);
          vt[u] = MOM_NT_LOAD(g.T_pp + i + j * G::CP);
        }
      }
    }
    vj = (lane < N) ? g.J0p[lane] : 0.0;
    __builtin_amdgcn_sched_barrier(0);
    q4_horner<KS, NBW>(P, T1, p, Y1);
  }
  q4_fence();
  MOM_STAMP(55);
  if constexpr (!SRC) {
#pragma unroll
    for (int u = 0; u < UT; ++u) {
      const int e = lane + 64 * u;
      if (e < NN) P[e] = vt[u];
    }
  }
  if (lane < N) c.v1[lane] = vj;
  real Radd[NB][NJ];
  if constexpr (!SRC) q4_load_glb_T<KS>(g.R_mp, q, Radd);
  q4_fence();
  MOM_STAMP(56);
  {
    {
      real Yf[NB][NJ], o[NB][NJ];
      q4_copy<KS>(Yf, Y1);
      q4_flip<KS>(Yf, mask);
      q4_mul_z<KS, 0, NBW>(t, Yf, o);
      q4_flip<KS>(o, mask);
      q4_store_glb_T<KS>(g.T_mm, q, o);
    }
    real V[NB][NJ], Vr[NJ], Rr[NJ];
#pragma unroll
    for (int J = 0; J < NJ; ++J) { Vr[J] = 0.0; Rr[J] = 0.0; }
    q4_mul_z<KS, 1, NBW>(r, Y1, V, c.jm, &Vr);
    if constexpr (SRC) {
      q4_ride<KS, 1, NBW>(c.v1, V, Rr);
    } else {
      q4_mul<KS, 1, NBW>(P, V, Radd, c.v1, &Rr);
      q4_store_glb_T<KS>(g.R_mp, q, Radd);
    }
#pragma unroll
    for (int J = 0; J < NJ; ++J) {
      const int col = 16 * J + q.c16;
      if (col < N && q.k == 0) g.J0m[col] = g.J0m[col] + (Rr[J] + Vr[J]);
    }
  }
  MOM_STAMP(58);
  {
    real T21[NB][NJ], Tr[NJ], Or[NJ];
    q4_load_T<KS>(t, q, T21);
#pragma unroll
    for (int J = 0; J < NJ; ++J) { Tr[J] = 0.0; Or[J] = 0.0; }
    q4_mul<KS, 1, NBW>(r, Y2, T21, c.jm, &Tr);
    if constexpr (SRC) {
      q4_ride<KS, 1, NBW>(c.v1, T21, Or);
    } else {
      real o[NB][NJ];
      q4_mul_z<KS, 1, NBW>(P, T21, o, c.v1, &Or);
      q4_store_glb_T<KS>(g.T_pp, q, o);
    }
#pragma unroll
    for (int J = 0; J < NJ; ++J) {
      const int col = 16 * J + q.c16;
      if (col < N && q.k == 0) g.J0p[col] = c.jp[col] + (Or[J] + Tr[J]);
    }
    real acc[NB][NJ];
    q4_load_T<KS>(r, q, acc);
#pragma unroll
    for (int J = 0; J < NJ; ++J) {
      const int col = 16 * J + q.c16;
      const real sc = (col < N) ? c.sg[col] : 1.0;
#pragma unroll
      for (int K = 0; K < NB; ++K) acc[K][J] = acc[K][J] * sc;
    }
    q4_flip<KS>(Y2, mask);
    q4_mul<KS, 0, NBW>(t, Y2, acc);
    q4_flip<KS>(acc, mask);
    q4_store_glb_T<KS>(g.R_pm, q, acc);
  }
  q4_fence();
  MOM_STAMP(59);
  return true;
}

#if MOM_STRIP_KS >= 9
#define MOM_Q4_ATTR __attribute__((amdgpu_waves_per_eu(1, 1)))
#else
#define MOM_Q4_ATTR
#endif
template <int KS, int NBW = Q4Geom<KS>::NB, bool SRC = false, bool EL = false>
__global__ void __launch_bounds__(64) MOM_Q4_ATTR k_layer_q4(const LayerArgs a) {
  using G = Q4Geom<KS>;
  constexpr int N = G::N;
  const size_t total = (size_t)a.S * a.M;
  Ctx c;
  make_ctx_q4(c, N, a.q.inv_mode, mom_smem);
  const int ns = a.q.regular ? a.q.nS : 1, Nq = N / ns;
  c.tabE = c.P;
  c.tabZS = c.P + 3 * Nq * Nq;
  real *lay = c.tabZS + 2 * ns * N;
  const int nz = a.Nz_sweep;
  const int lane = wg_lane();
#ifdef MOM_DIAG_STAMPS
  if (threadIdx.x == 0 && blockIdx.x == (gridDim.x >> 1)) mom_diag_last = mom_diag_now();
#endif
  load_streams(c, a.q);
  q4_fence();
  for (size_t pt = blockIdx.x; pt < total; pt += gridDim.x) {
    const int n = (int)(pt % a.S), mrel = (int)(pt / a.S), m = a.m_first + mrel;
    const size_t NNs = (size_t)N * N;
    CompPtrs g = comp_ptrs(a.comp, N, comp_pitch(N), pt);
    int done = nz;
    for (int z = 0; z < nz; ++z) {
      const int LW = 3 + a.K;
      if (lane < LW) {
        const size_t o = (size_t)n + (size_t)a.S * z;
        lay[lane] = (lane == 0) ? as_global(a.tau)[o] : (lane == 1) ? as_global(a.varpi)[o] : (lane == 2) ? as_global(a.tau_sum)[o]
                                                                                                          : as_global(a.zw)[(size_t)a.K * o + (lane - 3)];
      }
      q4_fence();
      MOM_STAMP(43);
      const int nd = a.nd_z[z];
      const bool first = (z == 0) && (a.first != 0);
      const real tau = lay[0], varpi = lay[1], tau_sum = lay[2];
      const real dtau = ldexp(tau, -nd);
      real expk = exp(-dtau / a.q.mu0);
      ZMix zpp{as_global(a.Zpp) + NNs * a.K * mrel, lay + 3, a.K, N};
      ZMix zmp{as_global(a.Zmp) + NNs * a.K * mrel, lay + 3, a.K, N};
      if constexpr (EL) elemental_build_tab<false, 4, N, N>(c, a.q, a.etab, m, nd, tau_sum, dtau, varpi, zpp, zmp);
      else elemental_build(c, a.q, m, nd, tau_sum, dtau, varpi, zpp, zmp);
      MOM_STAMP(41);
      bool bail;
      expk = doubling_run_q4<KS, NBW>(c, nd, expk, bail);
      if (!bail) {
        if (first) {
          store_added_as_composite(c, g);
          q4_fence();
          MOM_STAMP(42);
        } else {
          bail = !interaction_q4<KS, NBW, SRC>(c, g);
        }
      }
      if (bail) {
        done = z;
        break;
      }
    }
    if (lane == 0) a.resume[pt] = done;
  }
}

}
```

### radiativetransfer.jl_amd/csrc/mom_scene.hip

```cpp
#include "mom_handle.hpp"
#include "mom_elemental_tab.hpp"
#include "mom_images.hpp"
#include "mom_reduce.hpp"

using namespace mom;

struct PostArgs {
  int N, nS, S, M, nVza, red0, N0, nS0;
  int hdr_all;
  int zeroT_hi;
  const int *node;
  const double *cos_mphi, *sin_mphi;
  const double *J0p, *J0m;
  const double *J0p0, *J0m0;
  const double *hdrJ;
  const double *hdrJm;
  double *R, *T, *hdr;
};
__global__ void k_postprocess(PostArgs a) {
  const size_t idx = (size_t)blockIdx.x * blockDim.x + threadIdx.x;
  const size_t total = (size_t)a.nVza * a.nS * a.S;
  if (idx >= total) return;
  const int v = (int)(idx % a.nVza);
  const int k = (int)((idx / a.nVza) % a.nS);
  const size_t s = idx / ((size_t)a.nVza * a.nS);
  const int row = (a.node[v] - 1) * a.nS + k;
  double r = 0.0, t = 0.0, h = 0.0;
  for (int m = 0; m < a.M; ++m) {
    const double weight = (m == 0) ? 0.5 : 1.0;
    const double cs = weight * ((k < 2) ? a.cos_mphi[v + (size_t)a.nVza * m] : a.sin_mphi[v + (size_t)a.nVza * m]);
    if (m == 0 && a.red0) {
      if (k < a.nS0) {
        const size_t o = (size_t)(a.node[v] - 1) * a.nS0 + k + (size_t)a.N0 * s;
        r += cs * a.J0m0[o];
        t += cs * a.J0p0[o];
        h += cs * a.hdrJ[o];
      }
    } else {
      const size_t o = row + (size_t)a.N * (s + (size_t)a.S * m);
      r += cs * a.J0m[o];
      if (!(a.zeroT_hi && m > 0)) t += cs * a.J0p[o];
      if (m == 0) h += cs * a.hdrJ[row + (size_t)a.N * s];
      else if (a.hdr_all) h += cs * a.hdrJm[o];
    }
  }
  a.R[idx] = r;
  a.T[idx] = t;
  a.hdr[idx] = h;
}

__global__ void k_stream_tables(const double *mu, int ns, int Nq, double *out) {
  const int e = blockIdx.x * blockDim.x + threadIdx.x;
  if (e >= Nq * Nq) return;
  const int jq = e / Nq, iq = e - jq * Nq;
  const double mui = mu[iq * ns], muj = mu[jq * ns];
  out[e] = (1 / mui) + (1 / muj);
  out[Nq * Nq + e] = muj / (mui + muj);
  out[2 * Nq * Nq + e] = muj / (mui - muj);
}
static int stream_tables(mom_t *h, const DevStreams &q, MomDevBuf<double> &buf) {
  buf.reset();
  if (!q.regular || q.nS < 1 || q.N % q.nS != 0) return MOM_OK;
  const int Nq = q.N / q.nS;
  HIPCHK(h, buf.renew(3 * (size_t)Nq * Nq));
  hipLaunchKernelGGL(k_stream_tables, dim3((Nq * Nq + 255) / 256), dim3(256), 0, h->stream, q.mu, q.nS, Nq, buf.get());
  HIPCHK(h, hipGetLastError());
  return MOM_OK;
}

static bool strip_size(int N) { return mom_find_image(MOM_IMG_STRIP4, N) || mom_find_image(MOM_IMG_STRIP8, N); }
static int strip_pad(int N) { return mom_strip_pad(strip_size, N); }

static std::vector<double> stream_mu(const mom_t *h) {
  std::vector<double> mu((size_t)(h->N / h->nS));
  for (size_t i = 0; i < mu.size(); ++i) mu[i] = h->h_mu[i * h->nS];
  return mu;
}
static int stage_greeks(mom_t *h, const char *fn, MomGreekStage &st, int nG, int l_pad, const int *l_max, const double *greek, int M) {
  const std::string f(fn);
  if (h->dtype != 0) return fail(h, MOM_EUNSUPPORTED, (f + ": Greek coefficients are staged on Float64 handles only").c_str());
  if (!h->streams_set) return fail(h, MOM_ESTATE, (f + ": call mom_set_streams first").c_str());
  if (h->N % h->nS != 0) return fail(h, MOM_EINVAL, (f + ": the operator edge is not a whole number of streams").c_str());
  if (M > h->M) return fail(h, MOM_EINVAL, (f + ": more moments than the handle was created for").c_str());
  const std::vector<double> mu = stream_mu(h);
  if (const char *bad = mom_zmom_check(h->nS, (int)mu.size(), mu.data(), nG, l_pad, l_max, greek, 0, M))
    return fail(h, MOM_EINVAL, (f + ": " + bad).c_str());
  st.drop();
  st.nG = nG; st.l_pad = l_pad; st.M = M;
  st.l_max.assign(l_max, l_max + nG);
  st.greek.assign(greek, greek + (size_t)nG * 6 * l_pad);
  st.live = true;
  return MOM_OK;
}

extern "C" int mom_scene_stage_greeks(mom_t *h, int which, int nG, int l_pad, const int *l_max, const double *greek, int M) {
  if (!h) return fail(nullptr, MOM_EINVAL, "null handle");
  if (which != 0 && which != 1) return fail(h, MOM_EINVAL, "mom_scene_stage_greeks: which must be 0 (elastic bases) or 1 (the Raman set)");
  if (which == 0 && nG > 64) return fail(h, MOM_EINVAL, "mom_scene_stage_greeks: at most 64 phase-matrix bases");
  if (which == 1 && nG != 1) return fail(h, MOM_EINVAL, "mom_scene_stage_greeks: the Raman stage is one Greek set (nG = 1)");
  return stage_greeks(h, "mom_scene_stage_greeks", which ? h->stage_r : h->stage_z, nG, l_pad, l_max, greek, M);
}

extern "C" int mom_scene_stage_greek_partials(mom_t *h, int P, int nD, const int *basis, const int *partial, int l_pad,
                                              const int *l_max, const double *dgreek) {
  if (!h) return fail(nullptr, MOM_EINVAL, "null handle");
  const char *fn = "mom_scene_stage_greek_partials";
  if (P < 1 || P > 64 || nD < 1 || !basis || !partial) return fail(h, MOM_EINVAL, "mom_scene_stage_greek_partials: 1 <= P <= 64, nD >= 1, basis and partial given");
  for (int d = 0; d < nD; ++d) {
    if (basis[d] < 0 || basis[d] >= 64 || partial[d] < 0 || partial[d] >= P)
      return fail(h, MOM_EINVAL, "mom_scene_stage_greek_partials: basis within 0..63 and partial within 0..P-1");
    for (int e = 0; e < d; ++e)
      if (basis[e] == basis[d] && partial[e] == partial[d]) {
        char buf[160];
        snprintf(buf, sizeof buf, "%s: the pair (basis %d, partial %d) is named twice", fn, basis[d], partial[d]);
        return fail(h, MOM_EINVAL, buf);
      }
  }
  MomGreekStage st;
  const int rc = stage_greeks(h, fn, st, nD, l_pad, l_max, dgreek, 1);
  if (rc) return rc;
  st.P = P;
  st.basis.assign(basis, basis + nD);
  st.partial.assign(partial, partial + nD);
  h->stage_d = std::move(st);
  return MOM_OK;
}

int mom_stage_claim(mom_t *h, const char *fn, int K, int M) {
  const MomGreekStage &st = h->stage_z;
  char buf[256];
  if (!st.live) {
    snprintf(buf, sizeof buf, "%s: bad argument", fn);
    return fail(h, MOM_EINVAL, buf);
  }
  if (st.nG == K && st.M == M) return MOM_OK;
  snprintf(buf, sizeof buf, "%s: K = %d, M = %d, but the staged Greek sets (mom_scene_stage_greeks) are K = %d, M = %d", fn, K, M, st.nG, st.M);
  return fail(h, MOM_EINVAL, buf);
}

static int stage_bases(mom_t *h, int K, int M, int Nk, int N0, bool *red_ok) {
  MomGreekStage st = std::move(h->stage_z);
  h->stage_z.drop();
  if (!st.live || st.nG != K || st.M != M) return fail(h, MOM_EINVAL, "the scene's setter: no staged Greek sets of this K and M");
  const std::vector<double> mu = stream_mu(h);
  std::vector<int> slot((size_t)K * M);
  for (size_t e = 0; e < slot.size(); ++e) slot[e] = (int)e;
  const size_t nZ = (size_t)Nk * Nk * K * M, nZ0 = (size_t)N0 * N0 * K;
  MomZmomPlan pl;
  HIPCHK(h, mom_zmom_plan(pl, h->nS, (int)mu.size(), mu.data(), K, st.l_pad, st.l_max.data(), st.greek.data(), 0, M, slot.data(), h->stream));
  HIPCHK(h, h->d_Zpp.renew(nZ));
  HIPCHK(h, h->d_Zmp.renew(nZ));
  if (Nk != h->N) {
    HIPCHK(h, hipMemsetAsync(h->d_Zpp, 0, nZ * sizeof(double), h->stream));
    HIPCHK(h, hipMemsetAsync(h->d_Zmp, 0, nZ * sizeof(double), h->stream));
  }
  if (N0 > 0) {
    HIPCHK(h, h->d_Zpp0.renew(nZ0));
    HIPCHK(h, h->d_Zmp0.renew(nZ0));
    HIPCHK(h, hipMemsetAsync(h->d_Zpp0, 0, nZ0 * sizeof(double), h->stream));
    HIPCHK(h, hipMemsetAsync(h->d_Zmp0, 0, nZ0 * sizeof(double), h->stream));
  }
  HIPCHK(h, mom_zmom_launch(pl, h->stream, h->d_Zpp, h->d_Zmp, Nk, N0 > 0 ? h->d_Zpp0.get() : nullptr, N0 > 0 ? h->d_Zmp0.get() : nullptr, N0));
  int coupled = 0;
  if (N0 > 0) HIPCHK(h, mom_zmom_couples(pl, h->stream, K, h->d_Zpp, h->d_Zmp, Nk, &coupled));
  HIPCHK(h, hipStreamSynchronize(h->stream));
  if (coupled) {
    *red_ok = false;
    h->d_Zpp0.reset(); h->d_Zmp0.reset();
  }
  return MOM_OK;
}

extern "C" int mom_scene_set(mom_t *h, int Nz, int K, int M, const double *tau, const double *varpi, const double *zw,
                             const double *Zpp, const double *Zmp, const int *ndoubl, const int *iface,
                             const double *tau_sum, double albedo, int nVza, const int *node_1based,
                             const double *cos_mphi, const double *sin_mphi) {
  if (!h) return fail(nullptr, MOM_EINVAL, "null handle");
  if (!h->streams_set) return fail(h, MOM_ESTATE, "mom_scene_set: call mom_set_streams first");
  if (Nz <= 0 || K <= 0 || M <= 0 || M > h->M || nVza <= 0 || !tau || !varpi || !zw || (Zpp == nullptr) != (Zmp == nullptr) || !ndoubl ||
      !iface || !tau_sum || !node_1based || !cos_mphi || !sin_mphi)
    return fail(h, MOM_EINVAL, "mom_scene_set: bad argument");
  if (!Zpp) {
    const int rc = mom_stage_claim(h, "mom_scene_set", K, M);
    if (rc) return rc;
  }
  if (K > 64) return fail(h, MOM_EINVAL, "mom_scene_set: at most 64 phase-matrix bases (Rayleigh + aerosol types)");
  for (int z = 0; z < Nz; ++z)
    if (ndoubl[z] < 0 || ndoubl[z] > 60 || iface[z] < 0 || iface[z] > 3)
      return fail(h, MOM_EINVAL, "mom_scene_set: ndoubl/iface out of range");
  HIPCHK(h, hipSetDevice(h->device));
  const size_t S = h->S;
  h->scene_set = false;
  h->optics_scene = false;
  int rc;
  if (h->f32) {
    for (int v = 0; v < nVza; ++v)
      if (node_1based[v] < 1 || node_1based[v] * h->nS > h->N) return fail(h, MOM_EINVAL, "mom_scene_set: bad view node");
    if ((rc = momf_scene_set(h->f32, Nz, K, M, tau, varpi, zw, Zpp, Zmp, ndoubl, iface, tau_sum, albedo, nVza, node_1based,
                             cos_mphi, sin_mphi)))
      return fail(h, rc, momf_error(h->f32));
    h->Nz = Nz; h->K = K; h->scene_M = M; h->nVza = nVza; h->albedo = albedo; h->surf_kind = 0;
    h->nd.assign(ndoubl, ndoubl + Nz);
    h->iface.assign(iface, iface + Nz);
    h->scene_set = true;
    return MOM_OK;
  }
  HIPCHK(h, mom_upload(h->d_tau, tau, S * Nz, h->stream));
  HIPCHK(h, mom_upload(h->d_varpi, varpi, S * Nz, h->stream));
  HIPCHK(h, mom_upload(h->d_zw, zw, (size_t)K * S * Nz, h->stream));
  HIPCHK(h, mom_upload(h->d_tau_sum, tau_sum, S * (Nz + 1), h->stream));
  if ((rc = scene_common(h, Nz, K, M, Zpp, Zmp, albedo, nVza, node_1based, cos_mphi, sin_mphi))) return rc;
  h->nd.assign(ndoubl, ndoubl + Nz);
  h->iface.assign(iface, iface + Nz);
  h->scene_set = true;
  return MOM_OK;
}

int scene_common(mom_t *h, int Nz, int K, int M, const double *Zpp, const double *Zmp, double albedo, int nVza,
                 const int *node_1based, const double *cos_mphi, const double *sin_mphi) {
  for (int v = 0; v < nVza; ++v)
    if (node_1based[v] < 1 || node_1based[v] * h->nS > h->N) return fail(h, MOM_EINVAL, "mom_scene_set: bad view node");
  const size_t S = h->S, NN = (size_t)h->N * h->N;
  for (auto &b : h->d_dual_in) b.reset();
  h->dual_P = 0; h->dual_ran = false;
  h->stage_d.drop();
  const int Nk = (h->opt_pad && !(h->N <= 32 && h->opt_small)) ? strip_pad(h->N) : h->N;
  h->Nk = Nk;
  h->qk = h->q;
  h->qk.N = Nk;
  h->nbw_0 = 0;
  const bool staged = !Zpp;
  bool red_ok = h->opt_m0 && h->nS >= 3 && h->q.regular && !(h->N <= 4 && h->opt_small && nVza <= 4 && K <= 4) &&
                (staged ? mom_m0_source(h->q.I0, h->nS) : mom_m0_reducible(h->q.I0, h->N, h->nS, K, Zpp, Zmp));
  int N0 = 0;
  if (red_ok) {
    const int N0r = mom_m0_edge(h->N, h->nS);
    N0 = h->opt_pad ? strip_pad(N0r) : N0r;
    if (h->opt_pad && h->opt_lean >= 3 && N0 == N0r && N0r > 16 && N0r < 32 && (N0r % 4) != 0) N0 = N0r + 2;
  }
  for (MomDevBuf<double> *b : {&h->d_mu0, &h->d_wt0, &h->d_sg0, &h->d_Zpp0, &h->d_Zmp0, &h->d_hdrJ0, &h->d_scratch0}) b->reset();
  if (staged) {
    const int rc = stage_bases(h, K, M, Nk, N0, &red_ok);
    if (rc) return rc;
  } else if (Nk == h->N) {
    HIPCHK(h, mom_upload(h->d_Zpp, Zpp, NN * K * M, h->stream));
    HIPCHK(h, mom_upload(h->d_Zmp, Zmp, NN * K * M, h->stream));
  } else {
    const std::vector<double> zp = mom_pad_blocks(Zpp, h->N, Nk, (size_t)K * M), zm = mom_pad_blocks(Zmp, h->N, Nk, (size_t)K * M);
    HIPCHK(h, mom_upload(h->d_Zpp, zp.data(), zp.size(), h->stream));
    HIPCHK(h, mom_upload(h->d_Zmp, zm.data(), zm.size(), h->stream));
    HIPCHK(h, hipStreamSynchronize(h->stream));
  }
  HIPCHK(h, mom_upload(h->d_node, node_1based, (size_t)nVza, h->stream));
  HIPCHK(h, mom_upload(h->d_cos, cos_mphi, (size_t)nVza * M, h->stream));
  HIPCHK(h, mom_upload(h->d_sin, sin_mphi, (size_t)nVza * M, h->stream));
  h->d_R.reset(); h->d_hdr.reset(); h->d_T = nullptr;
  HIPCHK(h, h->d_R.renew(2 * (size_t)nVza * h->nS * S));
  h->d_T = h->d_R + (size_t)nVza * h->nS * S;
  HIPCHK(h, h->d_hdr.renew((size_t)nVza * h->nS * S));
  if (!h->d_hdrJ) {
    HIPCHK(h, h->d_hdrJ.renew((size_t)(h->N + kMomPadMax) * S));
    HIPCHK(h, h->d_bhr_uw.renew((size_t)h->nS * S));
    HIPCHK(h, h->d_bhr_dw.renew((size_t)h->nS * S));
  }
  {
    const int N = h->N, nS = h->nS;
    const bool ok = red_ok;
    for (auto &b : h->comp0) b.reset();
    h->red0 = ok;
    if (ok) {
      const int nS0 = kMomM0Stokes;
      h->N0 = N0; h->nS0 = nS0;
      const MomM0Cut cut = staged ? mom_m0_cut_streams(h->h_mu.data(), h->h_wt.data(), N, nS, N0)
                                  : mom_m0_cut(h->h_mu.data(), h->h_wt.data(), N, nS, K, N0, Zpp, Zmp);
      h->nbw_0 = mom_q4_nbw(cut.wt.data(), N0);
      HIPCHK(h, mom_upload(h->d_mu0, cut.mu.data(), (size_t)N0, h->stream));
      HIPCHK(h, mom_upload(h->d_wt0, cut.wt.data(), (size_t)N0, h->stream));
      HIPCHK(h, mom_upload(h->d_sg0, cut.sg.data(), (size_t)N0, h->stream));
      if (!staged) {
        HIPCHK(h, mom_upload(h->d_Zpp0, cut.Zpp.data(), cut.Zpp.size(), h->stream));
        HIPCHK(h, mom_upload(h->d_Zmp0, cut.Zmp.data(), cut.Zmp.size(), h->stream));
      }
      for (int k = 0; k < 6; ++k) {
        const size_t cnt = ((k < 4) ? (size_t)comp_pitch(N0) * N0 : (size_t)N0) * S;
        HIPCHK(h, h->comp0[k].renew(cnt));
        HIPCHK(h, hipMemsetAsync(h->comp0[k], 0, cnt * sizeof(double), h->stream));
      }
      HIPCHK(h, h->d_hdrJ0.renew((size_t)N0 * S));
      const size_t scr = (size_t)h->G * kGenericBufs * mat_elems(N0) + (size_t)ld_for(N0) * np_for(N0);
      HIPCHK(h, h->d_scratch0.renew(scr));
      HIPCHK(h, hipMemsetAsync(h->d_scratch0, 0, scr * sizeof(double), h->stream));
      HIPCHK(h, hipMemsetAsync(h->d_bhr_uw, 0, (size_t)h->nS * S * sizeof(double), h->stream));
      HIPCHK(h, hipMemsetAsync(h->d_bhr_dw, 0, (size_t)h->nS * S * sizeof(double), h->stream));
      DevStreams &q0 = h->q0;
      q0 = h->q;
      q0.mu = h->d_mu0; q0.wt = h->d_wt0; q0.sg = h->d_sg0;
      q0.N = N0; q0.nS = nS0;
      for (int k = nS0; k < 4; ++k) { q0.I0[k] = 0.0; q0.D[k] = 1.0; }
    }
  }
  {
    int rc;
    if ((rc = stream_tables(h, h->qk, h->d_etab))) return rc;
    h->d_etab0.reset();
    if (h->red0 && (rc = stream_tables(h, h->q0, h->d_etab0))) return rc;
  }
  HIPCHK(h, hipStreamSynchronize(h->stream));
  h->Nz = Nz; h->K = K; h->scene_M = M; h->nVza = nVza; h->albedo = albedo;
  h->surf_kind = 0;
  return MOM_OK;
}

extern "C" int mom_scene_set_surface(mom_t *h, int kind, int M, const double *Rsurf, const double *albedo_spec) {
  if (!h) return fail(nullptr, MOM_EINVAL, "null handle");
  if (!h->scene_set) return fail(h, MOM_ESTATE, "mom_scene_set_surface: call mom_scene_set first");
  if (kind < 0 || kind > 2 || (kind == 1 && (!Rsurf || M != h->scene_M)) || (kind == 2 && !albedo_spec))
    return fail(h, MOM_EINVAL, "mom_scene_set_surface: bad argument");
  HIPCHK(h, hipSetDevice(h->device));
  const int N = h->N, nS = h->nS;
  const size_t NN = (size_t)N * N, S = h->S;
  int rc;
  if (h->f32) {
    if ((rc = momf_scene_set_surface(h->f32, kind, M, Rsurf, albedo_spec))) return fail(h, rc, momf_error(h->f32));
    h->surf_kind = kind;
    return MOM_OK;
  }
  if (kind == 1) {
    if (h->Nk == N) {
      HIPCHK(h, mom_upload(h->d_Rsurf, Rsurf, NN * M, h->stream));
    } else {
      const std::vector<double> rp = mom_pad_blocks(Rsurf, N, h->Nk, (size_t)M);
      HIPCHK(h, mom_upload(h->d_Rsurf, rp.data(), rp.size(), h->stream));
      HIPCHK(h, hipStreamSynchronize(h->stream));
    }
    HIPCHK(h, h->d_hdrJm.renew((size_t)h->Nk * S * M));
    if (h->red0) {
      std::vector<double> r0;
      if (!mom_m0_cut_brdf(Rsurf, N, nS, h->N0, r0)) return fail(h, MOM_EINVAL, kMomM0BrdfCouples);
      HIPCHK(h, mom_upload(h->d_Rsurf0, r0.data(), r0.size(), h->stream));
    }
  } else if (kind == 2) {
    HIPCHK(h, mom_upload(h->d_albedo_spec, albedo_spec, S, h->stream));
  }
  HIPCHK(h, hipStreamSynchronize(h->stream));
  h->surf_kind = kind;
  return MOM_OK;
}

static int single_launch_begin(mom_t *h) {
  while (h->ev_full.size() < 2) { hipEvent_t e; HIPCHK(h, hipEventCreate(&e)); h->ev_full.push_back(e); }
  HIPCHK(h, hipEventRecord(h->ev[0], h->stream));
  HIPCHK(h, hipEventRecord(h->ev_full[0], h->stream));
  return MOM_OK;
}
static int single_launch_end(mom_t *h) {
  HIPCHK(h, hipEventRecord(h->ev_full[1], h->stream));
  for (int k = 1; k < 4; ++k) HIPCHK(h, hipEventRecord(h->ev[k], h->stream));
  h->launches = 1; h->launches_full = 1; h->launches_red = 0;
  return MOM_OK;
}

static int rt_run_small(mom_t *h) {
  const int Nz = h->Nz;
  if (!h->d_smtab) HIPCHK(h, h->d_smtab.renew(3 * 16));
  double tab[48];
  mom_small_tables(h->h_mu.data(), h->N, tab);
  HIPCHK(h, hipMemcpyAsync(h->d_smtab, tab, sizeof tab, hipMemcpyHostToDevice, h->stream));
  {
    HIPCHK(h, h->d_ndif.reserve(2 * (size_t)Nz, h->stream));
    std::vector<int> v(h->nd);
    v.insert(v.end(), h->iface.begin(), h->iface.end());
    HIPCHK(h, hipMemcpyAsync(h->d_ndif, v.data(), v.size() * sizeof(int), hipMemcpyHostToDevice, h->stream));
    HIPCHK(h, hipStreamSynchronize(h->stream));
  }
  if (h->K > 4) return fail(h, MOM_EINVAL, "mom_rt_run: the N <= 4 sweep kernel handles at most 4 phase-matrix bases");
  MomSmallSweepArgs a{};
  HIPCHK(h, mom_fill_small_args(a, *h, h->q, h->S, h->d_info, h->opt_small != 2, h->stream));
  int rc = single_launch_begin(h);
  if (rc) return rc;
  HIPCHK(h, momsm_launch_sweep(&a, h->N, h->stream));
  return single_launch_end(h);
}

static bool wave_sweep_applies(const mom_t *h) { return mom_wave_sweep_applies(*h, h->N, h->nS, h->opt_small, h->opt_force_generic); }
static int rt_run_wave(mom_t *h) {
  const int Nz = h->Nz;
  HIPCHK(h, h->d_ndif.reserve(2 * (size_t)Nz, h->stream));
  HIPCHK(h, hipMemcpyAsync(h->d_ndif, h->nd.data(), (size_t)Nz * sizeof(int), hipMemcpyHostToDevice, h->stream));
  MomWaveSweepArgs a{};
  mom_fill_wave_args(a, *h, h->q, h->S, h->d_info, h->opt_small == 1);
  int rc = single_launch_begin(h);
  if (rc) return rc;
  HIPCHK(h, momw_launch_sweep(&a, h->stream));
  if ((rc = single_launch_end(h))) return rc;
  HIPCHK(h, hipStreamSynchronize(h->stream));
  return MOM_OK;
}

enum Finisher { kFinStrip4, kFinStrip8, kFinGen4, kFinGen8 };

static Finisher choose_finisher(const mom_t *h, const DevStreams &q, int ns_tab, bool lds) {
  const MomLayerImage *s4 = mom_find_image(MOM_IMG_STRIP4, q.N);
  if (lds && h->opt_w4 && np_for(q.N) <= 48 &&
      2 * (s4 ? s4->lds_bytes(ns_tab, q.nS, h->K) : mom4_lds_bytes(q.N, true)) + 2048 <= 160 * 1024)
    return s4 ? kFinStrip4 : kFinGen4;
  return (lds && mom_find_image(MOM_IMG_STRIP8, q.N)) ? kFinStrip8 : kFinGen8;
}

struct FirstStage {
  const MomLayerImage *image;
  MomImageFamily family;
};
static FirstStage choose_first_stage(const mom_t *h, Finisher fin, const DevStreams &q, int ns_tab) {
  auto applying = [&](MomImageFamily f) {
    const MomLayerImage *im = mom_find_image(f, q.N);
    return FirstStage{(im && im->lds_bytes(ns_tab, q.nS, h->K) > 0) ? im : nullptr, f};
  };
  if (fin == kFinGen4 && h->opt_lean >= 3) return applying(MOM_IMG_QUAD);
  if (fin == kFinStrip8 && h->opt_strip2) return applying(MOM_IMG_STRIP2);
  if (fin == kFinStrip4 && h->opt_lean) {
    const FirstStage lean = applying(MOM_IMG_LEAN);
    if (lean.image && h->opt_lean >= 2) {
      const FirstStage alt = applying(h->opt_lean >= 3 ? MOM_IMG_QUAD : MOM_IMG_LEAN6);
      if (alt.image) return alt;
    }
    return lean;
  }
  return FirstStage{nullptr, MOM_IMG_LEAN};
}

static int launch_first_stage(mom_t *h, const FirstStage &fs, LayerArgs &a, int nbw, bool multi_target, bool sources_only, hipStream_t st) {
  const int nzr = a.Nz_sweep;
  bool ok = fs.image && nzr > 0 && !multi_target && a.q.inv_mode == 0;
  for (int k = 1; k < nzr && ok; ++k) ok = (a.iface_z[k] == 3);
  if (ok && !a.first) ok = (a.iface_z[0] == 3);
  if (!ok) return MOM_OK;
  const size_t units = (size_t)a.S * a.M;
  const bool two_buffer = (fs.family == MOM_IMG_STRIP2);
  MomDevBuf<int> &table = two_buffer ? h->d_resume2 : h->d_resume;
  HIPCHK(h, table.reserve(units, st));
  a.resume = table;
  int per_cu = fs.image->per_cu();
  const bool quad = (fs.family == MOM_IMG_QUAD);
  MomLaunchForm form;
  if (h->opt_zero_skip & (quad ? 1 : two_buffer ? 2 : 0)) form.nbw = nbw;
  form.row_blocks = two_buffer && (h->opt_zero_skip & 4);
  form.sources_only = sources_only && (two_buffer || quad);
  form.elemental_tab = (two_buffer || quad) && mom_elemental_tab_applies(a.q, a.K, a.etab);
  if (two_buffer) {
    h->resume2_units = units; h->resume2_nz = nzr;
    if (h->opt_strip2_sched) {
      const size_t ints = kMomStrip2SchedInts;
      if (!h->d_sched2) HIPCHK(h, h->d_sched2.renew(ints));
      HIPCHK(h, hipMemsetAsync(h->d_sched2, 0, ((h->opt_strip2_sched & 2) ? ints : 1) * sizeof(int), st));
      a.sched = h->d_sched2;
      form.sched_mode = h->opt_strip2_sched;
    }
  }
#ifdef MOM_EXPERIMENTS
  if (fs.family == MOM_IMG_LEAN || fs.family == MOM_IMG_LEAN6) {
    static const int lean_per_cu = getenv("MOM_LEAN_PER_CU") ? atoi(getenv("MOM_LEAN_PER_CU")) : 0;
    if (lean_per_cu > 0) per_cu = lean_per_cu;
  }
#endif
  const int grid = (int)std::min<size_t>(units, (size_t)per_cu * h->num_cu);
  HIPCHK(h, fs.image->launch(&a, form, grid, st));
  h->launches++;
  return MOM_OK;
}

static int launch_layer_images(mom_t *h, LayerArgs &a, int nbw, bool multi_target, bool sources_only, hipStream_t st) {
  const DevStreams &q = a.q;
  const size_t units = (size_t)a.S * a.M;
  const bool lds = (q.N <= 64) && !h->opt_force_generic;
  const int ns_tab = q.regular ? q.nS : 1;
  const Finisher fin = choose_finisher(h, q, ns_tab, lds);
  const int rc = launch_first_stage(h, choose_first_stage(h, fin, q, ns_tab), a, nbw, multi_target, sources_only, st);
  if (rc) return rc;
  if (fin == kFinStrip4 || fin == kFinStrip8) {
    const MomLayerImage *im = mom_find_image(fin == kFinStrip4 ? MOM_IMG_STRIP4 : MOM_IMG_STRIP8, q.N);
    if (fin == kFinStrip8 && units >= 8 * (size_t)h->num_cu && h->opt_stagger && a.resume == nullptr) {
      const double f = (double)q.N / 60.0, unit_us = f * f * f * (44.0 + 17.0 * a.nd);
      a.stagger = (int)(unit_us * 100.0 / 32.0);
    }
    const int grid = (int)std::min<size_t>(units, (size_t)im->per_cu() * h->num_cu);
    HIPCHK(h, im->launch(&a, MomLaunchForm{}, grid, st));
  } else if (fin == kFinGen4) {
    HIPCHK(h, mom4_launch_layer(&a, a.iface, true, (int)((a.S >= 2048) ? a.S : units), mom4_lds_bytes(q.N, true), st));
  } else {
    const int grid = lds ? (int)((a.S >= 2048) ? a.S : units) : (int)std::min<size_t>(units, (size_t)h->G);
    HIPCHK(h, mom_gen_launch_layer(&a, a.iface, lds, grid, lds_bytes(q.N, lds), st));
  }
  h->launches++;
  return MOM_OK;
}

struct TargetSpec {
  int ntgt = 0;
  double *tgt[kMaxTargets][6] = {};
  std::vector<signed char> act;
};

template <class Comp6>
static int rt_run_core(mom_t *h, int za, int zb, bool allow_red, const Comp6 &compF, bool do_surface, bool do_post,
                       bool cont = false, const TargetSpec *tg = nullptr) {
  const size_t S = h->S;
  const int M = h->scene_M;
  const bool red0 = h->red0 && allow_red;
  const int nzr = zb - za;
  while (h->ev_full.size() < 2 * (size_t)h->Nz + 2) { hipEvent_t e; HIPCHK(h, hipEventCreate(&e)); h->ev_full.push_back(e); }
  while (h->ev_red.size() < 2 * (size_t)h->Nz + 2) { hipEvent_t e; HIPCHK(h, hipEventCreate(&e)); h->ev_red.push_back(e); }
  const int Nk = h->Nk;
  const size_t NN = (size_t)Nk * Nk;
  bool can_sweep = h->opt_sweep && nzr <= kMaxSweepLayers && nzr > 1;
  for (int z = za + 2; z < zb && can_sweep; ++z) can_sweep = (h->iface[z] == h->iface[za + 1]);
  if (cont && can_sweep) can_sweep = (h->iface[za] == h->iface[za + 1]);
  for (int z = za; z < zb && can_sweep; ++z) can_sweep = (h->nd[z] <= 127);
  hipStream_t cur = h->stream;
  const int nbw_k = mom_q4_nbw(h->h_wt.data(), h->N);
  auto launch_layer = [&](int z, const DevStreams &q, int nbw, int m_first, int Mcount, const double *Zpp, const double *Zmp,
                          const auto &comp, double *scratch) -> int {
    LayerArgs a{};
    a.q = q; a.S = h->S; a.M = Mcount; a.K = h->K; a.m_first = m_first;
    const bool sweep = z < 0;
    if (sweep) {
      z = za;
      a.Nz_sweep = nzr;
      int ndsum = 0;
      for (int k = 0; k < nzr; ++k) { a.nd_z[k] = (signed char)h->nd[za + k]; a.iface_z[k] = (signed char)h->iface[za + k]; ndsum += h->nd[za + k]; }
      a.nd = ndsum / nzr; a.iface = h->iface[za + 1]; a.first = cont ? 0 : 1;
    } else {
      a.nd = h->nd[z]; a.iface = h->iface[z]; a.first = (z == za) && !cont;
    }
    a.tau = h->d_tau + S * z; a.varpi = h->d_varpi + S * z; a.zw = h->d_zw + (size_t)h->K * S * z;
    a.tau_sum = h->d_tau_sum + S * z;
    a.Zpp = Zpp; a.Zmp = Zmp;
    for (int k = 0; k < 6; ++k) a.comp[k] = comp[k];
    if (tg) {
      a.ntgt = tg->ntgt;
      for (int t = 0; t < tg->ntgt; ++t)
        for (int k = 0; k < 6; ++k) a.tgt[t][k] = tg->tgt[t][k];
      const int rows = sweep ? nzr : 1, r0 = sweep ? 0 : (z - za);
      for (int r = 0; r < rows; ++r)
        for (int t = 0; t < kMaxTargets; ++t) a.act_z[r][t] = tg->act[(size_t)(r0 + r) * kMaxTargets + t];
    }
    a.scratch = scratch; a.info = h->d_info;
    if (h->opt_elemental) a.etab = (&q == &h->q0) ? h->d_etab0.get() : h->d_etab.get();
    const bool unobserved = h->opt_sources_only && allow_red && !tg && (&q == &h->q0 || m_first >= 1);
    return launch_layer_images(h, a, nbw, tg != nullptr, unobserved, cur);
  };
  const bool two = red0 && can_sweep && h->opt_overlap && M > 1 && !tg && h->stream2 && !h->opt_force_generic &&
                   mom_find_image(MOM_IMG_STRIP2, Nk) != nullptr;
  HIPCHK(h, hipEventRecord(h->ev[0], h->stream));
  for (int z = (can_sweep ? -1 : za); z < (can_sweep ? 0 : zb); ++z) {
    int rc;
    const int e = can_sweep ? 0 : z - za;
    if (red0) {
      if (two) {
        HIPCHK(h, hipEventRecord(h->ev_fork, h->stream));
        HIPCHK(h, hipStreamWaitEvent(h->stream2, h->ev_fork, 0));
        cur = h->stream2;
        HIPCHK(h, hipEventRecord(h->ev_go, cur));
        HIPCHK(h, hipStreamWaitEvent(h->stream, h->ev_go, 0));
        HIPCHK(h, hipEventRecord(h->ev_red[2 * e], cur));
        if ((rc = launch_layer(z, h->q0, h->nbw_0, 0, 1, h->d_Zpp0, h->d_Zmp0, h->comp0, h->d_scratch0))) return rc;
        HIPCHK(h, hipEventRecord(h->ev_red[2 * e + 1], cur));
        h->launches_red++;
        cur = h->stream;
      }
      if (M > 1) {
        double *comp1[6];
        for (int k = 0; k < 6; ++k) comp1[k] = compF[k] + ((k < 4) ? (size_t)comp_pitch(Nk) * Nk : (size_t)Nk) * S;
        HIPCHK(h, hipEventRecord(h->ev_full[2 * e], h->stream));
        if ((rc = launch_layer(z, h->qk, nbw_k, 1, M - 1, h->d_Zpp + NN * h->K, h->d_Zmp + NN * h->K, comp1, h->d_scratch))) return rc;
        HIPCHK(h, hipEventRecord(h->ev_full[2 * e + 1], h->stream));
        h->launches_full++;
      }
      if (!two) {
        HIPCHK(h, hipEventRecord(h->ev_red[2 * e], h->stream));
        if ((rc = launch_layer(z, h->q0, h->nbw_0, 0, 1, h->d_Zpp0, h->d_Zmp0, h->comp0, h->d_scratch0))) return rc;
        HIPCHK(h, hipEventRecord(h->ev_red[2 * e + 1], h->stream));
        h->launches_red++;
      }
    } else {
      HIPCHK(h, hipEventRecord(h->ev_full[2 * e], h->stream));
      if ((rc = launch_layer(z, h->qk, nbw_k, 0, M, h->d_Zpp, h->d_Zmp, compF, h->d_scratch))) return rc;
      HIPCHK(h, hipEventRecord(h->ev_full[2 * e + 1], h->stream));
      h->launches_full++;
    }
  }
  HIPCHK(h, hipEventRecord(h->ev[1], h->stream));
  for (int m = 0; do_surface && m < ((h->surf_kind == 1) ? M : 1); ++m) {
    SurfArgs a{};
    const bool red = red0 && m == 0;
    const DevStreams &q = red ? h->q0 : h->qk;
    a.q = q; a.S = h->S; a.iface = h->iface[h->Nz - 1];
    a.albedo = h->albedo; a.tau_tot = h->d_tau_sum + S * h->Nz;
    a.kind = h->surf_kind; a.m = m; a.albedo_spec = h->d_albedo_spec;
    a.Rsurf = (h->surf_kind == 1) ? (red ? h->d_Rsurf0 : h->d_Rsurf + NN * m) : nullptr;
    for (int k = 0; k < 6; ++k)
      a.comp[k] = red ? h->comp0[k] : compF[k] + ((k < 4) ? (size_t)comp_pitch(Nk) * Nk : (size_t)Nk) * S * m;
    a.hdrJ = red ? h->d_hdrJ0 : (m == 0 ? h->d_hdrJ : h->d_hdrJm + (size_t)Nk * S * m);
    a.bhr_uw = h->d_bhr_uw; a.bhr_dw = h->d_bhr_dw; a.nS_out = h->nS;
    a.scratch = red ? h->d_scratch0 : h->d_scratch; a.info = h->d_info;
    const bool lds = (q.N <= 64) && !h->opt_force_generic;
    const size_t sm = lds_bytes(q.N, lds);
    const int grid = lds ? (int)S : (int)std::min<size_t>(S, (size_t)h->G);
    const hipStream_t sst = (two && red) ? h->stream2 : h->stream;
    if (lds && h->opt_w4 && np_for(q.N) <= 48 && 2 * mom4_lds_bytes(q.N, true) + 2048 <= 160 * 1024) {
      HIPCHK(h, mom4_launch_surface(&a, true, (int)S, mom4_lds_bytes(q.N, true), sst));
    } else {
      HIPCHK(h, mom_launch_ldsm(MOM_LDSM(k_surface), lds, grid, kThreads, sm, sst, a));
    }
  }
  if (two) {
    HIPCHK(h, hipEventRecord(h->ev_join, h->stream2));
    HIPCHK(h, hipStreamWaitEvent(h->stream, h->ev_join, 0));
  }
  HIPCHK(h, hipEventRecord(h->ev[2], h->stream));
  if (do_post) {
    const size_t total = (size_t)h->nVza * h->nS * S;
    PostArgs pa{};
    pa.N = Nk; pa.nS = h->nS; pa.S = h->S; pa.M = M; pa.nVza = h->nVza; pa.red0 = red0 ? 1 : 0;
    pa.N0 = h->N0; pa.nS0 = h->nS0;
    pa.node = h->d_node; pa.cos_mphi = h->d_cos; pa.sin_mphi = h->d_sin;
    pa.J0p = compF[4]; pa.J0m = compF[5]; pa.J0p0 = h->comp0[4]; pa.J0m0 = h->comp0[5];
    pa.hdrJ = red0 ? h->d_hdrJ0 : h->d_hdrJ;
    pa.hdr_all = (h->surf_kind == 1) ? 1 : 0; pa.zeroT_hi = (h->surf_kind == 2) ? 1 : 0; pa.hdrJm = h->d_hdrJm;
    pa.R = h->d_R; pa.T = h->d_T; pa.hdr = h->d_hdr;
    hipLaunchKernelGGL(k_postprocess, dim3((unsigned)((total + 255) / 256)), dim3(256), 0, h->stream, pa);
    HIPCHK(h, hipGetLastError());
  }
  HIPCHK(h, hipEventRecord(h->ev[3], h->stream));
  return MOM_OK;
}

extern "C" int mom_rt_run(mom_t *h) {
  if (!h) return fail(nullptr, MOM_EINVAL, "null handle");
  if (!h->scene_set) return fail(h, MOM_ESTATE, "mom_rt_run: call mom_scene_set first");
  HIPCHK(h, hipSetDevice(h->device));
  if (h->f32) {
    const int rc = momf_rt_run(h->f32);
    return rc ? fail(h, rc, momf_error(h->f32)) : MOM_OK;
  }
  h->launches = 0; h->launches_full = 0; h->launches_red = 0;
  h->comp_pitched = true;
  h->comp_on_chip = true;
  if (h->N <= 4 && h->opt_small && !h->opt_force_generic && h->nVza <= 4 && h->surf_kind == 0 && h->K <= 4) return rt_run_small(h);
  if (wave_sweep_applies(h)) return rt_run_wave(h);
  h->comp_on_chip = false;
  return rt_run_core(h, 0, h->Nz, true, h->comp, true, true);
}

extern "C" int mom_rt_run_multisensor(mom_t *h, int nSensors, const int *sensor_levels, double *uwJ, double *dwJ) {
  if (!h) return fail(nullptr, MOM_EINVAL, "null handle");
  F64_ONLY(h, "mom_rt_run_multisensor");
  if (!h->scene_set) return fail(h, MOM_ESTATE, "mom_rt_run_multisensor: call mom_scene_set first");
  if (nSensors <= 0 || !sensor_levels || !uwJ || !dwJ) return fail(h, MOM_EINVAL, "mom_rt_run_multisensor: bad argument");
  for (int i = 0; i < nSensors; ++i)
    if (sensor_levels[i] < 0 || sensor_levels[i] >= h->Nz)
      return fail(h, MOM_EINVAL, "mom_rt_run_multisensor: sensor level must be in 0..Nz-1 (0 = TOA/BOA, L = below layer L)");
  HIPCHK(h, hipSetDevice(h->device));
  const size_t S = h->S;
  const int M = h->scene_M, Nk = h->Nk;
  const size_t out1 = (size_t)h->nVza * h->nS * S;
  h->launches = 0; h->launches_full = 0; h->launches_red = 0;
  h->comp_pitched = true;
  h->comp_on_chip = false;
  if (!h->comp_top[0]) {
    const int Na = h->N + kMomPadMax;
    for (int k = 0; k < 6; ++k) {
      const size_t perc = (k < 4) ? (size_t)comp_pitch(Na) * Na : (size_t)Na;
      HIPCHK(h, h->comp_top[k].renew(perc * S * h->M));
    }
    for (int k = 0; k < 2; ++k) HIPCHK(h, h->d_msJ[k].renew((size_t)Na * S * h->M));
  }
  HIPCHK(h, h->d_ms_out.reserve(2 * out1 * nSensors, h->stream));
  double *d_uw = h->d_ms_out, *d_dw = h->d_ms_out + out1 * nSensors;
  const int Na = h->N + kMomPadMax;
  const size_t blk[6] = {(size_t)comp_pitch(Na) * Na, (size_t)comp_pitch(Na) * Na, (size_t)comp_pitch(Na) * Na,
                         (size_t)comp_pitch(Na) * Na, (size_t)Na, (size_t)Na};
  const int per_chunk = (kMaxTargets - 1) / 2;
  for (int c0 = 0; c0 < nSensors; c0 += per_chunk) {
    const int nc = std::min(per_chunk, nSensors - c0);
    const size_t need = (size_t)2 * nc;
    if (h->ms_comp.size() < 6 * need) h->ms_comp.resize(6 * need);
    for (size_t sidx = 0; sidx < need; ++sidx)
      for (int k = 0; k < 6; ++k) HIPCHK(h, h->ms_comp[6 * sidx + k].reserve(blk[k] * S * h->M, h->stream));
    std::vector<int> ord(nc);
    for (int i = 0; i < nc; ++i) ord[i] = c0 + i;
    std::stable_sort(ord.begin(), ord.end(), [&](int x, int y) { return sensor_levels[x] < sensor_levels[y]; });
    TargetSpec tg;
    tg.act.assign((size_t)h->Nz * kMaxTargets, 0);
    int maxL = 0;
    for (int i = 0; i < nc; ++i) maxL = std::max(maxL, sensor_levels[c0 + i]);
    int nt = 0;
    for (int k = 0; k < 6; ++k) tg.tgt[0][k] = h->comp_top[k];
    nt = 1;
    for (int z = 0; z < maxL; ++z) tg.act[(size_t)z * kMaxTargets + 0] = (z == 0) ? 1 : 2;
    std::vector<int> snap_t(nc, -1), bot_t(nc, -1);
    for (int i = 0; i < nc; ++i) {
      const int L = sensor_levels[ord[i]], Lnext = (i + 1 < nc) ? sensor_levels[ord[i + 1]] : h->Nz;
      if (L > 0) {
        snap_t[i] = nt;
        for (int k = 0; k < 6; ++k) tg.tgt[nt][k] = h->ms_comp[(size_t)(2 * i) * 6 + k];
        tg.act[(size_t)(L - 1) * kMaxTargets + nt] = 3;
        ++nt;
      }
      bot_t[i] = nt;
      for (int k = 0; k < 6; ++k) tg.tgt[nt][k] = h->ms_comp[(size_t)(2 * i + 1) * 6 + k];
      for (int z = L; z < Lnext; ++z) tg.act[(size_t)z * kMaxTargets + nt] = (z == L) ? 1 : 2;
      ++nt;
    }
    tg.ntgt = nt;
    int rc;
    if ((rc = rt_run_core(h, 0, h->Nz, false, h->comp, false, false, false, &tg))) return rc;
    for (int i = nc - 2; i >= 0; --i) {
      const int L = sensor_levels[ord[i]], Lnext = sensor_levels[ord[i + 1]];
      if (L == Lnext) {
        for (int k = 0; k < 6; ++k)
          HIPCHK(h, hipMemcpyAsync(tg.tgt[bot_t[i]][k], tg.tgt[bot_t[i + 1]][k], blk[k] * S * h->M * sizeof(double), hipMemcpyDeviceToDevice, h->stream));
        continue;
      }
      InterArgs a{};
      a.q = h->qk; a.S = h->S; a.M = M;
      for (int k = 0; k < 6; ++k) { a.top[k] = tg.tgt[bot_t[i]][k]; a.bot[k] = tg.tgt[bot_t[i + 1]][k]; }
      a.scratch = h->d_scratch; a.info = h->d_info;
      const bool lds = (Nk <= 64) && !h->opt_force_generic;
      const size_t sm = lds_bytes(Nk, lds);
      const size_t units = S * M;
      const int grid = (int)(lds ? units : std::min<size_t>(units, (size_t)h->G));
      HIPCHK(h, mom_launch_combine(a, lds, grid, sm, h->stream));
    }
    for (int i = 0; i < nc; ++i) {
      const int ims = ord[i], L = sensor_levels[ims];
      double *bot[6], *top[6];
      for (int k = 0; k < 6; ++k) { bot[k] = tg.tgt[bot_t[i]][k]; top[k] = (L > 0) ? tg.tgt[snap_t[i]][k] : nullptr; }
      if ((rc = rt_run_core(h, h->Nz, h->Nz, false, bot, true, L == 0))) return rc;
      if (L > 0) {
        InterArgs a{};
        a.q = h->qk; a.S = h->S; a.M = M;
        for (int k = 0; k < 6; ++k) { a.top[k] = top[k]; a.bot[k] = bot[k]; }
        a.dwJ = h->d_msJ[0]; a.uwJ = h->d_msJ[1]; a.scratch = h->d_scratch; a.info = h->d_info;
        const bool lds = (Nk <= 64) && !h->opt_force_generic;
        const size_t sm = lds_bytes(Nk, lds);
        const size_t units = S * M;
        const int grid = (int)(lds ? units : std::min<size_t>(units, (size_t)h->G));
        HIPCHK(h, mom_launch_ldsm(MOM_LDSM(k_interlayer), lds, grid, kThreads, sm, h->stream, a));
        PostArgs pa{};
        pa.N = Nk; pa.nS = h->nS; pa.S = h->S; pa.M = M; pa.nVza = h->nVza; pa.red0 = 0;
        pa.node = h->d_node; pa.cos_mphi = h->d_cos; pa.sin_mphi = h->d_sin;
        pa.J0p = h->d_msJ[0]; pa.J0m = h->d_msJ[1];
        pa.hdrJ = h->d_hdrJ; pa.hdr_all = 0; pa.zeroT_hi = 0; pa.hdrJm = nullptr;
        pa.R = h->d_R; pa.T = h->d_T; pa.hdr = h->d_hdr;
        hipLaunchKernelGGL(k_postprocess, dim3((unsigned)((out1 + 255) / 256)), dim3(256), 0, h->stream, pa);
        HIPCHK(h, hipGetLastError());
      }
      HIPCHK(h, hipMemcpyAsync(d_uw + out1 * ims, h->d_R, out1 * sizeof(double), hipMemcpyDeviceToDevice, h->stream));
      HIPCHK(h, hipMemcpyAsync(d_dw + out1 * ims, h->d_T, out1 * sizeof(double), hipMemcpyDeviceToDevice, h->stream));
    }
  }
  HIPCHK(h, hipMemcpyAsync(uwJ, d_uw, out1 * nSensors * sizeof(double), hipMemcpyDeviceToHost, h->stream));
  HIPCHK(h, hipMemcpyAsync(dwJ, d_dw, out1 * nSensors * sizeof(double), hipMemcpyDeviceToHost, h->stream));
  return check_info(h);
}

int mom_partials_check(mom_t *h, const char *fn, int P, const double *dZpp, const double *dZmp) {
  char buf[200];
  if (!(P >= 0 && P <= 64 && ((dZpp == nullptr) == (dZmp == nullptr)))) {
    snprintf(buf, sizeof buf, "%s: 0 <= P <= 64; dZpp and dZmp come together", fn);
    return fail(h, MOM_EINVAL, buf);
  }
  const MomGreekStage &st = h->stage_d;
  if (dZpp || !st.live) return MOM_OK;
  if (st.P != P) {
    snprintf(buf, sizeof buf, "%s: P = %d, but the staged Greek partials (mom_scene_stage_greek_partials) are P = %d", fn, P, st.P);
    return fail(h, MOM_EINVAL, buf);
  }
  for (int b : st.basis)
    if (b >= h->K) {
      snprintf(buf, sizeof buf, "%s: the staged Greek partials name basis %d, the scene has K = %d", fn, b, h->K);
      return fail(h, MOM_EINVAL, buf);
    }
  return MOM_OK;
}
static int stage_partials(mom_t *h) {
  MomGreekStage st = std::move(h->stage_d);
  h->stage_d.drop();
  const int K = h->K, M = h->scene_M, Nk = h->Nk, nD = st.nG;
  const size_t nZ = (size_t)Nk * Nk * K * M * h->dual_P;
  const std::vector<double> mu = stream_mu(h);
  std::vector<int> slot((size_t)nD * M);
  for (int mi = 0; mi < M; ++mi)
    for (int d = 0; d < nD; ++d) slot[d + (size_t)nD * mi] = st.basis[d] + K * (mi + M * st.partial[d]);
  MomZmomPlan pl;
  HIPCHK(h, mom_zmom_plan(pl, h->nS, (int)mu.size(), mu.data(), nD, st.l_pad, st.l_max.data(), st.greek.data(), 0, M, slot.data(), h->stream));
  HIPCHK(h, h->d_dual_in[3].renew(nZ));
  HIPCHK(h, h->d_dual_in[4].renew(nZ));
// ... 185 lines not shown
```

### radiativetransfer.jl_amd/csrc/momcore.hip

```cpp
#include "mom_handle.hpp"
#include "mom_ops.hpp"
#include "mom_rrs.hpp"

using namespace mom;



struct DualArgs {
  int N, S, P;
  const double *A, *dA, *B, *dB;
  double *C, *dC;
  double *scratch;
  int *info;
};

template <bool LDSM>
__global__ void __launch_bounds__(kThreads) k_batched_mul_dual(DualArgs a) {
  const int N = a.N;
  Ctx c;
  make_ctx<LDSM>(c, N, 1, mom_smem, LDSM ? nullptr : a.scratch + (size_t)blockIdx.x * kGenericBufs * mat_elems(N));
  zero_padding<LDSM>(c);
  __syncthreads();
  const size_t NN = (size_t)N * N;
  const int ld = c.ld;
// ... 34 lines not shown
    __syncthreads();
    if (N <= 64) wg_inverse_reg(N, c.P, ld, c.part, c.prow, c.ipiv, c.bad);
    else wg_inverse(N, c.fd, c.P, ld, c.prow, c.pcol, c.rowk, c.ipiv, c.sh, c.bad);
    wg_copy_mat(N, c.fd, c.P, ld, a.C + NN * pt, N);
    for (int ip = 0; ip < a.P; ++ip) {
      const size_t o = NN * (pt + (size_t)a.S * ip);
      __syncthreads();
      wg_copy_mat(N, c.fd, a.dA + o, N, c.Q, ld);
      __syncthreads();
      double *r = c.r;
      wg_gemm<false, !LDSM>(N, ElP{c.P, ld}, ElP{c.Q, ld}, [=](int i, int j, double v) { r[i + j * ld] = v; });
      __syncthreads();
      double *dX = a.dC + o;
      wg_gemm<false, !LDSM>(N, ElP{c.r, ld}, ElP{c.P, ld}, [=](int i, int j, double v) { dX[i + (size_t)j * N] = -v; });
    }
    __syncthreads();
  }
  if (threadIdx.x == 0 && *c.bad) atomicMax(a.info, *c.bad);
}


static thread_local std::string g_err;

int fail(mom_t *h, int code, const char *msg) {
  if (h) h->err = msg;
  g_err = msg;
  return code;
}

static size_t smem_bytes(const mom_t *h) { return lds_bytes(h->N, h->lds_mode); }

void mom_set_global_error(const char *msg) { g_err = msg ? msg : ""; }
extern "C" const char *mom_last_global_error(void) { return g_err.c_str(); }
extern "C" const char *mom_last_error(const mom_t *h) { return h ? h->err.c_str() : g_err.c_str(); }

static int ensure_op_layers(mom_t *h) {
  if (h->op_layers) return MOM_OK;
  const size_t NN = (size_t)h->N * h->N;
  for (int k = 0; k < 6; ++k) {
    const size_t per = ((k < 4) ? NN : (size_t)h->N) * h->S;
    HIPCHK(h, h->added[k].renew(per));
    HIPCHK(h, h->surf[k].renew(per));
    HIPCHK(h, hipMemsetAsync(h->added[k], 0, per * sizeof(double), h->stream));
    HIPCHK(h, hipMemsetAsync(h->surf[k], 0, per * sizeof(double), h->stream));
  }
  h->op_layers = true;
  return MOM_OK;
}
static int op_composite_ready(mom_t *h, const char *who) {
  if (h->comp_pitched) {
    char buf[192];
    snprintf(buf, sizeof buf, "%s: the composite layer holds scene-level (mom_rt_run) state; start the operator-level "
             "sequence with mom_copy_added_to_composite or mom_upload", who);
    return fail(h, MOM_ESTATE, buf);
  }
  return MOM_OK;
}

extern "C" int mom_create(mom_t **out, int device, int N, int nStokes, int S, int max_m, int dtype) {
  if (!out || N <= 0 || S <= 0 || max_m <= 0 || nStokes <= 0 || nStokes > 4 || N % nStokes != 0)
    return fail(nullptr, MOM_EINVAL, "mom_create: bad argument");
  if (dtype != 0 && dtype != 1) return fail(nullptr, MOM_EINVAL, "mom_create: dtype must be 0 (Float64) or 1 (Float32)");
  int ndev = 0;
  hipError_t e = hipGetDeviceCount(&ndev);
  if (e != hipSuccess || ndev <= 0) return fail(nullptr, MOM_EHIP, "mom_create: no HIP device available");
  if (device < 0 || device >= ndev) return fail(nullptr, MOM_EINVAL, "mom_create: device index out of range");
  mom_t *h = new mom_t();
  h->device = device; h->N = N; h->nS = nStokes; h->S = S; h->M = max_m; h->dtype = dtype;
  h->lds_mode = (N <= 64);
  *out = h;
  HIPCHK(h, hipSetDevice(device));
  HIPCHK(h, hipStreamCreate(&h->stream));
  {
    int lo = 0, hi = 0;
    HIPCHK(h, hipDeviceGetStreamPriorityRange(&lo, &hi));
    HIPCHK(h, hipStreamCreateWithPriority(&h->stream2, hipStreamNonBlocking, hi));
    HIPCHK(h, hipEventCreateWithFlags(&h->ev_fork, hipEventDisableTiming));
    HIPCHK(h, hipEventCreateWithFlags(&h->ev_join, hipEventDisableTiming));
    HIPCHK(h, hipEventCreateWithFlags(&h->ev_go, hipEventDisableTiming));
  }
  const size_t NN = (size_t)N * N;
  const int Na = N + kMomPadMax;
  HIPCHK(h, h->d_mu.renew(Na));
  HIPCHK(h, h->d_wt.renew(Na));
  HIPCHK(h, h->d_sg.renew(Na));
  (void)NN;
  for (int k = 0; k < 6 && dtype == 0; ++k) {
    const size_t perc = (k < 4) ? (size_t)comp_pitch(Na) * Na : (size_t)Na;
    HIPCHK(h, h->comp[k].renew(perc * S * max_m));
    HIPCHK(h, hipMemsetAsync(h->comp[k], 0, perc * S * max_m * sizeof(double), h->stream));
  }
  for (int k = 0; k < 4; ++k) HIPCHK(h, h->d_vec[k].renew(S));
  HIPCHK(h, h->d_info.renew(1));
  HIPCHK(h, hipMemsetAsync(h->d_info, 0, sizeof(int), h->stream));
  h->G = 1024;
  {
    hipDeviceProp_t prop;
    HIPCHK(h, hipGetDeviceProperties(&prop, device));
    h->num_cu = prop.multiProcessorCount > 0 ? prop.multiProcessorCount : 256;
  }
  if (dtype == 1) {
    for (int k = 0; k < 4; ++k) HIPCHK(h, hipEventCreate(&h->ev[k]));
    HIPCHK(h, hipStreamSynchronize(h->stream));
    const int rc = momf_create(&h->f32, device, h->stream, N, nStokes, S, max_m, h->d_info);
    if (rc) return fail(h, rc, momf_error(h->f32));
    return MOM_OK;
  }
  HIPCHK(h, h->d_scratch.renew((size_t)h->G * kGenericBufs * mat_elems(N) + (size_t)ld_for(N) * np_for(N)));
  HIPCHK(h, hipMemsetAsync(h->d_scratch, 0, ((size_t)h->G * kGenericBufs * mat_elems(N) + (size_t)ld_for(N) * np_for(N)) * sizeof(double), h->stream));
  for (int k = 0; k < 4; ++k) HIPCHK(h, hipEventCreate(&h->ev[k]));
  HIPCHK(h, hipStreamSynchronize(h->stream));
  return MOM_OK;
}

extern "C" int mom_destroy(mom_t *h) {
  if (!h) return MOM_OK;
  (void)hipSetDevice(h->device);
  (void)hipStreamSynchronize(h->stream);
  if (h->f32) momf_destroy(h->f32);
  momr::destroy(h->rrs);
  if (h->comm && g_rccl_destroy) g_rccl_destroy(h->comm);
  for (int k = 0; k < 4; ++k) if (h->ev[k]) (void)hipEventDestroy(h->ev[k]);
  for (int k = 0; k < 2; ++k) if (h->ev_voigt[k]) (void)hipEventDestroy(h->ev_voigt[k]);
  for (auto e : h->ev_full) (void)hipEventDestroy(e);
  for (auto e : h->ev_red) (void)hipEventDestroy(e);
  if (h->ev_fork) (void)hipEventDestroy(h->ev_fork);
  if (h->ev_join) (void)hipEventDestroy(h->ev_join);
  if (h->ev_go) (void)hipEventDestroy(h->ev_go);
  if (h->stream2) (void)hipStreamDestroy(h->stream2);
  if (h->stream) (void)hipStreamDestroy(h->stream);
  delete h;
  return MOM_OK;
}

extern "C" int mom_sync(mom_t *h) {
  if (!h) return fail(nullptr, MOM_EINVAL, "null handle");
  HIPCHK(h, hipSetDevice(h->device));
  HIPCHK(h, hipStreamSynchronize(h->stream));
  return MOM_OK;
}

extern "C" int mom_strip2_resumed(mom_t *h, int *units, int *left) {
  if (!h || !units || !left) return fail(h, MOM_EINVAL, "mom_strip2_resumed: null argument");
  HIPCHK(h, hipSetDevice(h->device));
  HIPCHK(h, hipStreamSynchronize(h->stream));
  *units = (int)h->resume2_units; *left = 0;
  if (!h->d_resume2 || h->resume2_units == 0) { *units = 0; return MOM_OK; }
  std::vector<int> r(h->resume2_units);
  HIPCHK(h, hipMemcpy(r.data(), h->d_resume2, r.size() * sizeof(int), hipMemcpyDeviceToHost));
  for (int v : r) *left += (v < h->resume2_nz);
  return MOM_OK;
}

extern "C" int mom_check(mom_t *h) {
  if (!h) return fail(nullptr, MOM_EINVAL, "null handle");
  HIPCHK(h, hipSetDevice(h->device));
  return check_info(h);
}

extern "C" int mom_set_option(mom_t *h, int option, int value) {
  if (!h) return fail(nullptr, MOM_EINVAL, "null handle");
  if (option == MOM_OPT_INVERSE) { h->opt_inverse = value; h->q.inv_mode = value; h->qk.inv_mode = value; h->q0.inv_mode = value; }
  else if (option == MOM_OPT_M0_REDUCTION) h->opt_m0 = value;
  else if (option == MOM_OPT_SMALL_WG) h->opt_w4 = value;
  else if (option == MOM_OPT_STAGGER) h->opt_stagger = value;
  else if (option == MOM_OPT_SMALL_N) { h->opt_small = value; h->scene_set = false; }
  else if (option == MOM_OPT_LAYER_SWEEP) h->opt_sweep = value;
  else if (option == MOM_OPT_STRIP_PAD) { h->opt_pad = value; h->scene_set = false; }
  else if (option == MOM_OPT_LEAN) { h->opt_lean = value; h->scene_set = false; }
  else if (option == MOM_OPT_OVERLAP) h->opt_overlap = value;
  else if (option == MOM_OPT_STRIP2) h->opt_strip2 = value;
  else if (option == MOM_OPT_STRIP2_SCHED) {
    if (value < 0 || value > 3) return fail(h, MOM_EINVAL, "mom_set_option: MOM_OPT_STRIP2_SCHED takes a mask of bits 0 and 1");
    h->opt_strip2_sched = value;
  }
  else if (option == MOM_OPT_ZERO_SKIP) {
    if (value < 0 || value > 7) return fail(h, MOM_EINVAL, "mom_set_option: MOM_OPT_ZERO_SKIP takes a mask of bits 0, 1 and 2");
    h->opt_zero_skip = value;
  }
  else if (option == MOM_OPT_SOURCES_ONLY) h->opt_sources_only = value;
  else if (option == MOM_OPT_ELEMENTAL) h->opt_elemental = value;
  else if (option == MOM_OPT_LUT_BATCH) {
    if (value < 0) return fail(h, MOM_EINVAL, "mom_set_option: MOM_OPT_LUT_BATCH takes a number of (p, T) nodes >= 0 (0 = the default of 64)");
    h->opt_lut_batch = value;
  }
  else if (option == MOM_OPT_DUAL_WORKSPACE_MB) {
    if (value < 0) return fail(h, MOM_EINVAL, "mom_set_option: MOM_OPT_DUAL_WORKSPACE_MB takes megabytes >= 0 (0 = 60 % of the free HBM)");
    h->opt_dual_budget = (size_t)value << 20;
  }
  else if (option == MOM_OPT_RRS_KERNELS) {
    if (value < 0 || value > 63 || ((value & momr::KOPT_EL_FUSE_ON) && (value & momr::KOPT_EL_FUSE_OFF)))
      return fail(h, MOM_EINVAL, "mom_set_option: MOM_OPT_RRS_KERNELS takes a mask of bits 0..5 (bits 4 and 5 exclude each other)");
    h->opt_rrs_kernels = value;
    if (h->rrs) h->rrs->kopt = value;
  }
  else if (option == MOM_OPT_FORCE_GENERIC) {
    h->opt_force_generic = value;
    h->lds_mode = (h->N <= 64) && !value;
  } else return fail(h, MOM_EINVAL, "mom_set_option: unknown option");
  if (h->f32) momf_set_options(h->f32, h->opt_inverse, h->opt_force_generic, h->opt_sweep, h->opt_small, h->opt_m0, h->opt_pad, h->opt_w4);
  return MOM_OK;
}

extern "C" int mom_set_streams(mom_t *h, const double *qp_muN, const double *wt_muN, int N, int imu0_1based, double mu0,
                               const double *I0, const double *D, int strict) {
  if (!h) return fail(nullptr, MOM_EINVAL, "null handle");
  if (N != h->N || !qp_muN || !wt_muN || !I0 || !D || imu0_1based < 1 || imu0_1based * h->nS > N)
    return fail(h, MOM_EINVAL, "mom_set_streams: bad argument");
  HIPCHK(h, hipSetDevice(h->device));
  h->h_mu.assign(qp_muN, qp_muN + N);
  h->h_wt.assign(wt_muN, wt_muN + N);
  h->strict = strict;
  h->stage_z.drop(); h->stage_r.drop(); h->stage_d.drop();
  std::vector<double> sg(N);
  for (int i = 0; i < N; ++i) {
    const int comp = strict ? ((i + 1) % h->nS) : (i % h->nS) + 1;
    sg[i] = (comp > 2) ? -1.0 : 1.0;
  }
  {
    std::vector<double> mu(qp_muN, qp_muN + N), wt(wt_muN, wt_muN + N);
    mu.resize(N + kMomPadMax, 1.0); wt.resize(N + kMomPadMax, 0.0); sg.resize(N + kMomPadMax, 1.0);
    HIPCHK(h, hipMemcpyAsync(h->d_mu, mu.data(), mu.size() * sizeof(double), hipMemcpyHostToDevice, h->stream));
    HIPCHK(h, hipMemcpyAsync(h->d_wt, wt.data(), wt.size() * sizeof(double), hipMemcpyHostToDevice, h->stream));
    HIPCHK(h, hipMemcpyAsync(h->d_sg, sg.data(), sg.size() * sizeof(double), hipMemcpyHostToDevice, h->stream));
    HIPCHK(h, hipStreamSynchronize(h->stream));
  }
  DevStreams &q = h->q;
  q.mu = h->d_mu; q.wt = h->d_wt; q.sg = h->d_sg;
  for (int k = 0; k < 4; ++k) { q.I0[k] = (k < h->nS) ? I0[k] : 0.0; q.D[k] = (k < h->nS) ? D[k] : 1.0; }
  q.N = N; q.nS = h->nS; q.imu0 = imu0_1based; q.mu0 = mu0; q.inv_mode = h->opt_inverse;
  q.regular = 1;
  for (int i = 0; i < N; ++i)
    if (qp_muN[i] != qp_muN[(i / h->nS) * h->nS]) q.regular = 0;
  if (h->f32) {
    momf_set_options(h->f32, h->opt_inverse, h->opt_force_generic, h->opt_sweep, h->opt_small, h->opt_m0, h->opt_pad, h->opt_w4);
    const int rc = momf_set_streams(h->f32, qp_muN, wt_muN, sg.data(), imu0_1based, mu0, I0, D, q.regular);
    if (rc) return fail(h, rc, momf_error(h->f32));
  }
  h->streams_set = true;
  h->scene_set = false;
  return MOM_OK;
}

static int grid_for(const mom_t *h, size_t total) {
  if (h->lds_mode) return (int)total;
  return (int)std::min<size_t>(total, (size_t)h->G);
}
int check_info(mom_t *h) {
  int info = 0;
  HIPCHK(h, hipMemcpyAsync(&info, h->d_info, sizeof(int), hipMemcpyDeviceToHost, h->stream));
  HIPCHK(h, hipStreamSynchronize(h->stream));
  if (info) {
    HIPCHK(h, hipMemsetAsync(h->d_info, 0, sizeof(int), h->stream));
    char buf[128];
    snprintf(buf, sizeof buf, "zero pivot at elimination step %d while inverting (I - R r)", info);
    return fail(h, MOM_ESINGULAR, buf);
  }
  return MOM_OK;
}

#define LAUNCH(h, KERN, grid, args) \
  HIPCHK(h, mom_launch_ldsm(MOM_LDSM(KERN), (h)->lds_mode, grid, kThreads, smem_bytes(h), (h)->stream, args))
#define LAUNCH2(h, KERN, TARG, grid, args) \
  HIPCHK(h, mom_launch_ldsm(MOM_LDSM(KERN, TARG), (h)->lds_mode, grid, kThreads, smem_bytes(h), (h)->stream, args))

extern "C" int mom_elemental(mom_t *h, int m, int ndoubl, const double *tau_sum, const double *dtau, const double *varpi,
                             const double *Zpp, const double *Zmp, int z_batch) {
  if (!h) return fail(nullptr, MOM_EINVAL, "null handle");
  if (!h->streams_set) return fail(h, MOM_ESTATE, "mom_elemental: call mom_set_streams first");
  if (!tau_sum || !dtau || !varpi || !Zpp || !Zmp || (z_batch != 1 && z_batch != h->S) || m < 0 || ndoubl < 0)
    return fail(h, MOM_EINVAL, "mom_elemental: bad argument");
  if (h->f32) {
    const int rc = momf_op_elemental(h->f32, m, ndoubl, tau_sum, dtau, varpi, Zpp, Zmp, z_batch);
    return rc ? fail(h, rc, momf_error(h->f32)) : MOM_OK;
  }
  HIPCHK(h, hipSetDevice(h->device));
  { const int rc_ = ensure_op_layers(h); if (rc_) return rc_; }
  const size_t NN = (size_t)h->N * h->N, zc = NN * z_batch;
  for (int k = 0; k < 2; ++k) HIPCHK(h, h->d_Zop[k].reserve(zc, h->stream));
  const size_t sb = (size_t)h->S * sizeof(double);
  HIPCHK(h, hipMemcpyAsync(h->d_vec[0], tau_sum, sb, hipMemcpyHostToDevice, h->stream));
  HIPCHK(h, hipMemcpyAsync(h->d_vec[1], dtau, sb, hipMemcpyHostToDevice, h->stream));
  HIPCHK(h, hipMemcpyAsync(h->d_vec[2], varpi, sb, hipMemcpyHostToDevice, h->stream));
  HIPCHK(h, hipMemcpyAsync(h->d_Zop[0], Zpp, zc * sizeof(double), hipMemcpyHostToDevice, h->stream));
  HIPCHK(h, hipMemcpyAsync(h->d_Zop[1], Zmp, zc * sizeof(double), hipMemcpyHostToDevice, h->stream));
  OpArgs a{};
  a.q = h->q; a.S = h->S; a.m = m; a.nd = ndoubl; a.z_batch = z_batch;
  a.tau_sum = h->d_vec[0]; a.dtau = h->d_vec[1]; a.varpi = h->d_vec[2]; a.Zpp = h->d_Zop[0]; a.Zmp = h->d_Zop[1];
  for (int k = 0; k < 6; ++k) a.added[k] = h->added[k];
  a.scratch = h->d_scratch; a.info = h->d_info;
  LAUNCH(h, k_op_elemental, grid_for(h, h->S), a);
  HIPCHK(h, hipStreamSynchronize(h->stream));
  return MOM_OK;
}

extern "C" int mom_doubling(mom_t *h, int ndoubl, double *expk) {
  if (!h) return fail(nullptr, MOM_EINVAL, "null handle");
  if (!h->streams_set) return fail(h, MOM_ESTATE, "mom_doubling: call mom_set_streams first");
  if (!expk || ndoubl < 0) return fail(h, MOM_EINVAL, "mom_doubling: bad argument");
  if (h->f32) {
    const int rc = momf_op_doubling(h->f32, ndoubl, expk);
    return rc ? fail(h, rc, momf_error(h->f32)) : check_info(h);
  }
  HIPCHK(h, hipSetDevice(h->device));
  { const int rc_ = ensure_op_layers(h); if (rc_) return rc_; }
  const size_t sb = (size_t)h->S * sizeof(double);
  HIPCHK(h, hipMemcpyAsync(h->d_vec[3], expk, sb, hipMemcpyHostToDevice, h->stream));
  OpArgs a{};
  a.q = h->q; a.S = h->S; a.nd = ndoubl; a.expk = h->d_vec[3];
  for (int k = 0; k < 6; ++k) a.added[k] = h->added[k];
  a.scratch = h->d_scratch; a.info = h->d_info;
  if (ndoubl > 0) LAUNCH(h, k_op_doubling, grid_for(h, h->S), a);
  HIPCHK(h, hipMemcpyAsync(expk, h->d_vec[3], sb, hipMemcpyDeviceToHost, h->stream));
  return check_info(h);
}

extern "C" int mom_interaction(mom_t *h, int iface, int with_surface_layer) {
  if (!h) return fail(nullptr, MOM_EINVAL, "null handle");
  if (!h->streams_set) return fail(h, MOM_ESTATE, "mom_interaction: call mom_set_streams first");
  if (iface < 0 || iface > 3) return fail(h, MOM_EINVAL, "mom_interaction: iface must be 0..3");
  if (h->f32) {
    const int rc = momf_op_interaction(h->f32, iface, with_surface_layer);
    return rc ? fail(h, rc, momf_error(h->f32)) : check_info(h);
  }
  HIPCHK(h, hipSetDevice(h->device));
  { int rc_ = ensure_op_layers(h); if (rc_) return rc_; if ((rc_ = op_composite_ready(h, "mom_interaction"))) return rc_; }
  OpArgs a{};
  a.q = h->q; a.S = h->S; a.iface = iface;
  for (int k = 0; k < 6; ++k) { a.added[k] = with_surface_layer ? h->surf[k] : h->added[k]; a.comp[k] = h->comp[k]; }
  a.scratch = h->d_scratch; a.info = h->d_info;
  LAUNCH(h, k_op_interaction, grid_for(h, h->S), a);
  return check_info(h);
}
// ... 303 lines not shown
```

### radiativetransfer.jl_amd/csrc/momcore_q4.hip

```cpp
#ifndef MOM_STRIP_KS
#error "compile with -DMOM_STRIP_KS=<N/4>"
#endif
#include <hip/hip_runtime.h>

#include "mom_diag.hpp"
#include "mom_q4.hpp"
#include "mom_host.hpp"
#include "mom_image_variants.hpp"

using namespace MOM_NS;

static_assert(MOM_STRIP_KS > kQ4Skip[kSkipVariants - 1], "momcore_q4.hip: NB - 4 >= 1");
using LayerKernel = void (*)(LayerArgs);
static LayerKernel q4_kernel(int v, bool src, bool el) {
  return mom_with_int<0, kSkipVariants - 1>(v, [&](auto V) {
    return mom_with_bool(src, [&](auto SRC) {
      return mom_with_bool(el, [&](auto EL) -> LayerKernel { return k_layer_q4<MOM_STRIP_KS, MOM_STRIP_KS - kQ4Skip[V], SRC, EL>; });
    });
  });
}
static hipError_t image_launch(const void *layer_args, const MomLaunchForm &f, int grid, hipStream_t st) {
  const LayerKernel k = q4_kernel(mom_skip_variant(kQ4Skip, MOM_STRIP_KS, f.nbw), f.sources_only, f.elemental_tab);
  return mom_launch_lds(k, grid, 64, q4_lds_bytes(4 * MOM_STRIP_KS), st, *reinterpret_cast<const LayerArgs *>(layer_args));
}
static int query_per_cu() {
  const size_t smem = q4_lds_bytes(4 * MOM_STRIP_KS);
  int per_cu = 1 << 30;
  for (int key = 0; key < 4 * kSkipVariants; ++key) {
    const LayerKernel k = q4_kernel(key >> 2, (key & 1) != 0, (key & 2) != 0);
    int nb = 0;
    if (mom_allow_lds(reinterpret_cast<const void *>(k), smem) != hipSuccess ||
        hipOccupancyMaxActiveBlocksPerMultiprocessor(&nb, k, 64, smem) != hipSuccess || nb < 1)
      nb = 4;
    per_cu = std::min(per_cu, nb);
  }
  return per_cu;
}
static int image_per_cu() {
  static const int per_cu = query_per_cu();
  return per_cu;
}
static size_t image_lds_bytes(int ns, int, int K) { return q4_applies(4 * MOM_STRIP_KS, ns, K) ? q4_lds_bytes(4 * MOM_STRIP_KS) : 0; }
MOM_DEFINE_IMAGE(QUAD, MOM_STRIP_KS, image_launch, image_lds_bytes, image_per_cu)

#ifdef MOM_DIAG_STAMPS
#define MOM_CAT2(a, b) a##b
#define MOM_CAT(a, b) MOM_CAT2(a, b)
extern "C" int MOM_CAT(momq_q4_diag_read, MOM_STRIP_KS)(unsigned long long *out, int reset) {
  if (hipMemcpyFromSymbol(out, HIP_SYMBOL(mom_diag_acc), 128 * sizeof(unsigned long long)) != hipSuccess) return 1;
  if (reset) {
    unsigned long long z[128] = {0};
    if (hipMemcpyToSymbol(HIP_SYMBOL(mom_diag_acc), z, sizeof z) != hipSuccess) return 1;
  }
  return 0;
}
#endif
```

Before: 39540 spectral points/s.

## Restrict sources-only quad interaction chain to column groups holding viewing rows

In the sources-only quad kernel, the T_mm chain (load, Horner power, multiply, store and J0m update) now starts at a compile-time column group JLO. JLO is derived from the lowest 1-based node row across the viewing zenith angles, so 16-column groups below every requested VZA row are skipped. This is enabled by default by raising opt_sources_only to 2, and kernel variants are instantiated per JLO. The aim is to cut FMA and memory work on columns that do not feed the output. The cost is more kernel instantiations and a dependence on host-side node indices.

```diff
diff --git a/include/momcore.h b/include/momcore.h
--- a/include/momcore.h
+++ b/include/momcore.h
@@ -176,6 +176,7 @@
 int mom_set_option(mom_t *h, int option, int value);
 
 int mom_strip2_resumed(mom_t *h, int *units, int *left);
+int mom_live_rows_launched(mom_t *h, int *q4_jlo_full, int *q4_jlo_sub);
 enum { MOM_OPT_INVERSE = 0, MOM_OPT_FORCE_GENERIC = 1, MOM_OPT_M0_REDUCTION = 2, MOM_OPT_SMALL_WG = 3, MOM_OPT_STAGGER = 4,
        MOM_OPT_SMALL_N = 5, MOM_OPT_LAYER_SWEEP = 6, MOM_OPT_STRIP_PAD = 7, MOM_OPT_LEAN = 8, MOM_OPT_OVERLAP = 9,
        MOM_OPT_RRS_KERNELS = 10, MOM_OPT_DUAL_WORKSPACE_MB = 11, MOM_OPT_STRIP2 = 12, MOM_OPT_STRIP2_SCHED = 13,
diff --git a/radiativetransfer.jl_amd/_lib.py b/radiativetransfer.jl_amd/_lib.py
--- a/radiativetransfer.jl_amd/_lib.py
+++ b/radiativetransfer.jl_amd/_lib.py
@@ -133,6 +133,7 @@
     "mom_timers": (C.c_int, [c_h, c_dp, C.c_int, c_ip]),
     "mom_set_option": (C.c_int, [c_h, C.c_int, C.c_int]),
     "mom_strip2_resumed": (C.c_int, [c_h, c_ip, c_ip]),
+    "mom_live_rows_launched": (C.c_int, [c_h, c_ip, c_ip]),
     "mom_lut_create": (C.c_int, [c_h, C.c_int, C.c_double, C.c_double, C.c_int, C.c_double, C.c_double, C.c_int, C.c_double, C.c_double,
                                  c_ip]),
     "mom_lut_set_table": (C.c_int, [c_h, C.c_int, c_dp]),
@@ -728,6 +729,11 @@
         self.check(self.lib.mom_strip2_resumed(self._h, C.byref(u), C.byref(l)))
         return u.value, l.value
 
+    def live_rows_launched(self):
+        f, s = C.c_int(0), C.c_int(0)
+        self.check(self.lib.mom_live_rows_launched(self._h, C.byref(f), C.byref(s)))
+        return f.value, s.value
+
     def timers(self):
         ms = np.zeros(8)
         nl = C.c_int(0)
diff --git a/radiativetransfer.jl_amd/csrc/mom_handle.hpp b/radiativetransfer.jl_amd/csrc/mom_handle.hpp
--- a/radiativetransfer.jl_amd/csrc/mom_handle.hpp
+++ b/radiativetransfer.jl_amd/csrc/mom_handle.hpp
@@ -105,7 +105,9 @@
   int opt_strip2_sched = 1;
   MomDevBuf<int> d_sched2;
   int opt_zero_skip = 7;
-  int opt_sources_only = 1;
+  int opt_sources_only = 2;
+  std::vector<int> h_node;
+  int last_q4_jlo[2] = {0, 0};
   int opt_elemental = 1;
   MomDevBuf<double> d_etab, d_etab0;
   int nbw_0 = 0;
diff --git a/radiativetransfer.jl_amd/csrc/mom_image_variants.hpp b/radiativetransfer.jl_amd/csrc/mom_image_variants.hpp
--- a/radiativetransfer.jl_amd/csrc/mom_image_variants.hpp
+++ b/radiativetransfer.jl_amd/csrc/mom_image_variants.hpp
@@ -12,6 +12,16 @@
     if (KS - skip[c] >= nbw) v = c;
   return v;
 }
+inline int mom_q4_jlo(const int *node_1based, int nVza, int nS, int N) {
+  if (!node_1based || nVza < 1 || nS < 1) return 0;
+  int lo = N;
+  for (int v = 0; v < nVza; ++v) {
+    const int row = (node_1based[v] - 1) * nS;
+    if (row < 0 || row + nS > N) return 0;
+    if (row < lo) lo = row;
+  }
+  return lo / 16;
+}
 constexpr bool s2_row_blocks_change(int KS, int KW) { return KW < KS || 4 * ((KS + 3) / 4) - 1 > KS; }
 inline bool s2_row_blocks_for(int KS, const MomLaunchForm &f) {
   return f.row_blocks && s2_row_blocks_change(KS, KS - kS2Skip[mom_skip_variant(kS2Skip, KS, f.nbw)]);
diff --git a/radiativetransfer.jl_amd/csrc/mom_images.hpp b/radiativetransfer.jl_amd/csrc/mom_images.hpp
--- a/radiativetransfer.jl_amd/csrc/mom_images.hpp
+++ b/radiativetransfer.jl_amd/csrc/mom_images.hpp
@@ -7,6 +7,7 @@
   int nbw = 0;
   bool row_blocks = false;
   bool sources_only = false;
+  int q4_jlo = 0;
   bool elemental_tab = false;
   int sched_mode = 0;
 };
diff --git a/radiativetransfer.jl_amd/csrc/mom_q4.hpp b/radiativetransfer.jl_amd/csrc/mom_q4.hpp
--- a/radiativetransfer.jl_amd/csrc/mom_q4.hpp
+++ b/radiativetransfer.jl_amd/csrc/mom_q4.hpp
@@ -43,12 +43,12 @@
 #pragma unroll
     for (int J = 0; J < Q4Geom<KS>::NJ; ++J) W[K][J] = 0.0;
 }
-template <int KS>
+template <int KS, int JL = 0>
 __device__ __forceinline__ void q4_copy(real (&D)[Q4Geom<KS>::NB][Q4Geom<KS>::NJ], const real (&S)[Q4Geom<KS>::NB][Q4Geom<KS>::NJ]) {
 #pragma unroll
   for (int K = 0; K < Q4Geom<KS>::NB; ++K)
 #pragma unroll
-    for (int J = 0; J < Q4Geom<KS>::NJ; ++J) D[K][J] = S[K][J];
+    for (int J = JL; J < Q4Geom<KS>::NJ; ++J) D[K][J] = S[K][J];
 }
 
 template <int KS>
@@ -70,33 +70,34 @@
     for (int J = 0; J < G::NJ; ++J)
       if (16 * J + q.c16 < G::N) base[16 * J + 4 * K * G::LD] = W[K][J];
 }
-template <int KS>
+template <int KS, int JL = 0>
 __device__ __forceinline__ void q4_load_glb_T(const gdouble *__restrict__ X, const Q4Lane &q, real (&W)[Q4Geom<KS>::NB][Q4Geom<KS>::NJ]) {
   using G = Q4Geom<KS>;
   const gdouble *base = X + q.c16 + q.k * G::CP;
 #pragma unroll
   for (int K = 0; K < G::NB; ++K)
 #pragma unroll
-    for (int J = 0; J < G::NJ; ++J) W[K][J] = (16 * J + q.c16 < G::N) ? MOM_NT_LOAD(base + 16 * J + 4 * K * G::CP) : 0.0;
-}
-template <int KS>
+    for (int J = JL; J < G::NJ; ++J) W[K][J] = (16 * J + q.c16 < G::N) ? MOM_NT_LOAD(base + 16 * J + 4 * K * G::CP) : 0.0;
+}
+template <int KS, int JL = 0>
 __device__ __forceinline__ void q4_store_glb_T(gdouble *__restrict__ X, const Q4Lane &q, const real (&W)[Q4Geom<KS>::NB][Q4Geom<KS>::NJ]) {
   using G = Q4Geom<KS>;
   gdouble *base = X + q.c16 + q.k * G::CP;
 #pragma unroll
   for (int K = 0; K < G::NB; ++K)
 #pragma unroll
-    for (int J = 0; J < G::NJ; ++J)
+    for (int J = JL; J < G::NJ; ++J)
       if (16 * J + q.c16 < G::N) MOM_NT_STORE(W[K][J], base + 16 * J + 4 * K * G::CP);
 }
 
-template <int KS, int NV = 0, bool ZERO = false, int NBW = Q4Geom<KS>::NB>
+template <int KS, int NV = 0, bool ZERO = false, int NBW = Q4Geom<KS>::NB, int JL = 0>
 __device__ __forceinline__ void q4_mul_c(const real *M, const real (&X)[Q4Geom<KS>::NB][Q4Geom<KS>::NJ],
                                          const real (&C0)[Q4Geom<KS>::NB][Q4Geom<KS>::NJ],
                                          real (&acc)[Q4Geom<KS>::NB][Q4Geom<KS>::NJ], const real *ride = nullptr,
                                          real (*accR)[Q4Geom<KS>::NJ] = nullptr) {
   using G = Q4Geom<KS>;
   static_assert(NBW >= 1 && NBW <= G::NB, "q4_mul_c: 1 <= NBW <= NB");
+  static_assert(JL >= 0 && JL < G::NJ, "q4_mul_c: 0 <= JL < NJ");
   constexpr int NZ = G::NB - NBW;
   int l = wg_lane();
   asm volatile("" : "+v"(l));
@@ -108,14 +109,14 @@
   for (int I = 0; I < G::NB; ++I) {
     if (I >= NBW) {
 #pragma unroll
-      for (int J = 0; J < G::NJ; ++J) acc[I][J] = ZERO ? (real)0 : C0[I][J];
+      for (int J = JL; J < G::NJ; ++J) acc[I][J] = ZERO ? (real)0 : C0[I][J];
     }
 #pragma unroll
     for (int K = 0; K < G::NB; ++K) {
       if (I >= NBW && K != I) continue;
       const real a = base[4 * K + 4 * I * G::LD];
 #pragma unroll
-      for (int J = 0; J < G::NJ; ++J)
+      for (int J = JL; J < G::NJ; ++J)
         if (Q4_XLIVE(K, J)) acc[I][J] = mma4(a, X[K][J], (I < NBW && K == 0) ? (ZERO ? (real)0 : C0[I][J]) : acc[I][J]);
     }
   }
@@ -125,7 +126,7 @@
     for (int K = 0; K < G::NB; ++K) {
       const real a = (i < NV) ? rb[4 * K] : 0.0;
 #pragma unroll
-      for (int J = 0; J < G::NJ; ++J)
+      for (int J = JL; J < G::NJ; ++J)
         if (Q4_XLIVE(K, J)) (*accR)[J] = mma4(a, X[K][J], (*accR)[J]);
     }
   }
@@ -171,15 +172,15 @@
 #pragma unroll
     for (int K = 0; K < G::NB; ++K) {
 #pragma unroll
-      for (int J = 0; J < G::NJ; ++J)
+      for (int J = JL; J < G::NJ; ++J)
         if (Q4_XLIVE(K, J)) acc[I0][J] = mma4(ac[0][K], X[K][J], K == 0 ? (ZERO ? (real)0 : C0[I0][J]) : acc[I0][J]);
       if (two) {
 #pragma unroll
-        for (int J = 0; J < G::NJ; ++J)
+        for (int J = JL; J < G::NJ; ++J)
           if (Q4_XLIVE(K, J)) acc[I0 + 1][J] = mma4(ac[1][K], X[K][J], K == 0 ? (ZERO ? (real)0 : C0[I0 + 1][J]) : acc[I0 + 1][J]);
       } else if (NV > 0) {
 #pragma unroll
-        for (int J = 0; J < G::NJ; ++J)
+        for (int J = JL; J < G::NJ; ++J)
           if (Q4_XLIVE(K, J)) (*accR)[J] = mma4(ac[1][K], X[K][J], (*accR)[J]);
       }
     }
@@ -191,7 +192,7 @@
 #pragma unroll
     for (int K = 0; K < G::NB; ++K) {
 #pragma unroll
-      for (int J = 0; J < G::NJ; ++J)
+      for (int J = JL; J < G::NJ; ++J)
         if (Q4_XLIVE(K, J)) (*accR)[J] = mma4(an[0][K], X[K][J], (*accR)[J]);
     }
   }
@@ -199,7 +200,7 @@
   for (int d = 0; d < NZ; ++d) {
     const int I = NBW + d;
 #pragma unroll
-    for (int J = 0; J < G::NJ; ++J) {
+    for (int J = JL; J < G::NJ; ++J) {
       const real c0 = ZERO ? (real)0 : C0[I][J];
       acc[I][J] = (J == (I >> 2)) ? mma4(ad[d], X[I][J], c0) : c0;
     }
@@ -207,7 +208,7 @@
 #undef Q4_XLIVE
 }
 
-template <int KS, int NV, int NBW = Q4Geom<KS>::NB>
+template <int KS, int NV, int NBW = Q4Geom<KS>::NB, int JL = 0>
 __device__ __forceinline__ void q4_ride(const real *ride, const real (&X)[Q4Geom<KS>::NB][Q4Geom<KS>::NJ], real (&accR)[Q4Geom<KS>::NJ]) {
   using G = Q4Geom<KS>;
   static_assert(NV >= 1 && NBW >= 1 && NBW <= G::NB, "q4_ride: NV >= 1, 1 <= NBW <= NB");
@@ -221,55 +222,55 @@
 #pragma unroll
   for (int K = 0; K < G::NB; ++K)
 #pragma unroll
-    for (int J = 0; J < G::NJ; ++J)
+    for (int J = JL; J < G::NJ; ++J)
       if (K < NBW || J == (K >> 2)) accR[J] = mma4(a[K], X[K][J], accR[J]);
 }
 
-template <int KS, int NV = 0, int NBW = Q4Geom<KS>::NB>
+template <int KS, int NV = 0, int NBW = Q4Geom<KS>::NB, int JL = 0>
 __device__ __forceinline__ void q4_mul(const real *M, const real (&X)[Q4Geom<KS>::NB][Q4Geom<KS>::NJ],
                                        real (&acc)[Q4Geom<KS>::NB][Q4Geom<KS>::NJ], const real *ride = nullptr,
                                        real (*accR)[Q4Geom<KS>::NJ] = nullptr) {
-  q4_mul_c<KS, NV, false, NBW>(M, X, acc, acc, ride, accR);
-}
-template <int KS, int NV = 0, int NBW = Q4Geom<KS>::NB>
+  q4_mul_c<KS, NV, false, NBW, JL>(M, X, acc, acc, ride, accR);
+}
+template <int KS, int NV = 0, int NBW = Q4Geom<KS>::NB, int JL = 0>
 __device__ __forceinline__ void q4_mul_z(const real *M, const real (&X)[Q4Geom<KS>::NB][Q4Geom<KS>::NJ],
                                          real (&acc)[Q4Geom<KS>::NB][Q4Geom<KS>::NJ], const real *ride = nullptr,
                                          real (*accR)[Q4Geom<KS>::NJ] = nullptr) {
-  q4_mul_c<KS, NV, true, NBW>(M, X, acc, acc, ride, accR);
+  q4_mul_c<KS, NV, true, NBW, JL>(M, X, acc, acc, ride, accR);
 }
 
 #ifndef Q4_HORNER_SITES
 #define Q4_HORNER_SITES 1
 #endif
-template <int KS, int NBW = Q4Geom<KS>::NB>
+template <int KS, int NBW = Q4Geom<KS>::NB, int JL = 0>
 __device__ __forceinline__ void q4_horner(const real *M, const real (&C0)[Q4Geom<KS>::NB][Q4Geom<KS>::NJ], int p,
                                           real (&Y)[Q4Geom<KS>::NB][Q4Geom<KS>::NJ]) {
-  q4_copy<KS>(Y, C0);
+  q4_copy<KS, JL>(Y, C0);
   MOM_STAMP(82);
 #if Q4_HORNER_SITES == 2
   int n = p - 1;
 #pragma nounroll
   for (; n >= 2; n -= 2) {
     real Z[Q4Geom<KS>::NB][Q4Geom<KS>::NJ];
-    q4_mul_c<KS, 0, false, NBW>(M, Y, C0, Z);
-    q4_mul_c<KS, 0, false, NBW>(M, Z, C0, Y);
+    q4_mul_c<KS, 0, false, NBW, JL>(M, Y, C0, Z);
+    q4_mul_c<KS, 0, false, NBW, JL>(M, Z, C0, Y);
   }
   if (n == 1) {
     real acc[Q4Geom<KS>::NB][Q4Geom<KS>::NJ];
-    q4_mul_c<KS, 0, false, NBW>(M, Y, C0, acc);
-    q4_copy<KS>(Y, acc);
+    q4_mul_c<KS, 0, false, NBW, JL>(M, Y, C0, acc);
+    q4_copy<KS, JL>(Y, acc);
   }
 #else
 #pragma nounroll
   for (int kk = 1; kk < p; ++kk) {
     real acc[Q4Geom<KS>::NB][Q4Geom<KS>::NJ];
     MOM_STAMP(74);
-    q4_mul_c<KS, 0, false, NBW>(M, Y, C0, acc);
+    q4_mul_c<KS, 0, false, NBW, JL>(M, Y, C0, acc);
 #ifdef MOM_DIAG_STAMPS
     if (kk == 1) { MOM_STAMP(75); } else { MOM_STAMP(77); }
     if (threadIdx.x == 0 && blockIdx.x == (gridDim.x >> 1)) mom_diag_acc[kk == 1 ? 78 : 79] += 1;
 #endif
-    q4_copy<KS>(Y, acc);
+    q4_copy<KS, JL>(Y, acc);
     MOM_STAMP(76);
   }
 #endif
@@ -283,12 +284,12 @@
     if (sg[4 * K + q.k] < 0.0) m |= 1u << K;
   return m;
 }
-template <int KS>
+template <int KS, int JL = 0>
 __device__ __forceinline__ void q4_flip(real (&W)[Q4Geom<KS>::NB][Q4Geom<KS>::NJ], unsigned mask) {
 #pragma unroll
   for (int K = 0; K < Q4Geom<KS>::NB; ++K)
 #pragma unroll
-    for (int J = 0; J < Q4Geom<KS>::NJ; ++J) {
+    for (int J = JL; J < Q4Geom<KS>::NJ; ++J) {
       const real v = W[K][J];
       W[K][J] = ((mask >> K) & 1u) ? -v : v;
     }
@@ -412,10 +413,11 @@
   return expk;
 }
 
-template <int KS, int NBW = Q4Geom<KS>::NB, bool SRC = false>
+template <int KS, int NBW = Q4Geom<KS>::NB, bool SRC = false, int JLO = 0>
 __device__ __forceinline__ bool interaction_q4(Ctx &c, const CompPtrs &g) {
   using G = Q4Geom<KS>;
   constexpr int N = G::N, NB = G::NB, NJ = G::NJ, NN = N * N;
+  static_assert(JLO == 0 || (SRC && JLO < NJ), "interaction_q4: the restricted chain 1 exists in the sources-only form alone");
   const Q4Lane q;
   const int lane = wg_lane();
   real *r = c.r, *t = c.t, *P = c.P;
@@ -471,7 +473,7 @@
   real vt[UT], vj;
   {
     real T1[NB][NJ];
-    q4_load_glb_T<KS>(g.T_mm, q, T1);
+    q4_load_glb_T<KS, JLO>(g.T_mm, q, T1);
     __builtin_amdgcn_sched_barrier(0);
     q4_horner<KS, NBW>(P, W0, p, Y2);
     if constexpr (!SRC) {
@@ -487,7 +489,7 @@
     }
     vj = (lane < N) ? g.J0p[lane] : 0.0;
     __builtin_amdgcn_sched_barrier(0);
-    q4_horner<KS, NBW>(P, T1, p, Y1);
+    q4_horner<KS, NBW, JLO>(P, T1, p, Y1);
   }
   q4_fence();
   MOM_STAMP(55);
@@ -506,24 +508,24 @@
   {
     {
       real Yf[NB][NJ], o[NB][NJ];
-      q4_copy<KS>(Yf, Y1);
-      q4_flip<KS>(Yf, mask);
-      q4_mul_z<KS, 0, NBW>(t, Yf, o);
-      q4_flip<KS>(o, mask);
-      q4_store_glb_T<KS>(g.T_mm, q, o);
+      q4_copy<KS, JLO>(Yf, Y1);
+      q4_flip<KS, JLO>(Yf, mask);
+      q4_mul_z<KS, 0, NBW, JLO>(t, Yf, o);
+      q4_flip<KS, JLO>(o, mask);
+      q4_store_glb_T<KS, JLO>(g.T_mm, q, o);
     }
     real V[NB][NJ], Vr[NJ], Rr[NJ];
 #pragma unroll
     for (int J = 0; J < NJ; ++J) { Vr[J] = 0.0; Rr[J] = 0.0; }
-    q4_mul_z<KS, 1, NBW>(r, Y1, V, c.jm, &Vr);
+    q4_mul_z<KS, 1, NBW, JLO>(r, Y1, V, c.jm, &Vr);
     if constexpr (SRC) {
-      q4_ride<KS, 1, NBW>(c.v1, V, Rr);
+      q4_ride<KS, 1, NBW, JLO>(c.v1, V, Rr);
     } else {
       q4_mul<KS, 1, NBW>(P, V, Radd, c.v1, &Rr);
       q4_store_glb_T<KS>(g.R_mp, q, Radd);
     }
 #pragma unroll
-    for (int J = 0; J < NJ; ++J) {
+    for (int J = JLO; J < NJ; ++J) {
       const int col = 16 * J + q.c16;
       if (col < N && q.k == 0) g.J0m[col] = g.J0m[col] + (Rr[J] + Vr[J]);
     }
@@ -571,7 +573,7 @@
 #else
 #define MOM_Q4_ATTR
 #endif
-template <int KS, int NBW = Q4Geom<KS>::NB, bool SRC = false, bool EL = false>
+template <int KS, int NBW = Q4Geom<KS>::NB, bool SRC = false, bool EL = false, int JLO = 0>
 __global__ void __launch_bounds__(64) MOM_Q4_ATTR k_layer_q4(const LayerArgs a) {
   using G = Q4Geom<KS>;
   constexpr int N = G::N;
@@ -621,7 +623,7 @@
           q4_fence();
           MOM_STAMP(42);
         } else {
-          bail = !interaction_q4<KS, NBW, SRC>(c, g);
+          bail = !interaction_q4<KS, NBW, SRC, JLO>(c, g);
         }
       }
       if (bail) {
diff --git a/radiativetransfer.jl_amd/csrc/mom_scene.hip b/radiativetransfer.jl_amd/csrc/mom_scene.hip
--- a/radiativetransfer.jl_amd/csrc/mom_scene.hip
+++ b/radiativetransfer.jl_amd/csrc/mom_scene.hip
@@ -1,5 +1,6 @@
 #include "mom_handle.hpp"
 #include "mom_elemental_tab.hpp"
+#include "mom_image_variants.hpp"
 #include "mom_images.hpp"
 #include "mom_reduce.hpp"
 
@@ -252,6 +253,7 @@
     HIPCHK(h, hipStreamSynchronize(h->stream));
   }
   HIPCHK(h, mom_upload(h->d_node, node_1based, (size_t)nVza, h->stream));
+  h->h_node.assign(node_1based, node_1based + nVza);
   HIPCHK(h, mom_upload(h->d_cos, cos_mphi, (size_t)nVza * M, h->stream));
   HIPCHK(h, mom_upload(h->d_sin, sin_mphi, (size_t)nVza * M, h->stream));
   h->d_R.reset(); h->d_hdr.reset(); h->d_T = nullptr;
@@ -446,6 +448,10 @@
   if (h->opt_zero_skip & (quad ? 1 : two_buffer ? 2 : 0)) form.nbw = nbw;
   form.row_blocks = two_buffer && (h->opt_zero_skip & 4);
   form.sources_only = sources_only && (two_buffer || quad);
+  if (form.sources_only && quad && h->opt_sources_only >= 2) {
+    form.q4_jlo = mom_q4_jlo(h->h_node.data(), (int)h->h_node.size(), a.q.nS, a.q.N);
+    h->last_q4_jlo[a.m_first == 0 ? 1 : 0] = form.q4_jlo;
+  }
   form.elemental_tab = (two_buffer || quad) && mom_elemental_tab_applies(a.q, a.K, a.etab);
   if (two_buffer) {
     h->resume2_units = units; h->resume2_nz = nzr;
@@ -644,6 +650,7 @@
     return rc ? fail(h, rc, momf_error(h->f32)) : MOM_OK;
   }
   h->launches = 0; h->launches_full = 0; h->launches_red = 0;
+  h->last_q4_jlo[0] = h->last_q4_jlo[1] = 0;
   h->comp_pitched = true;
   h->comp_on_chip = true;
   if (h->N <= 4 && h->opt_small && !h->opt_force_generic && h->nVza <= 4 && h->surf_kind == 0 && h->K <= 4) return rt_run_small(h);
diff --git a/radiativetransfer.jl_amd/csrc/momcore.hip b/radiativetransfer.jl_amd/csrc/momcore.hip
--- a/radiativetransfer.jl_amd/csrc/momcore.hip
+++ b/radiativetransfer.jl_amd/csrc/momcore.hip
@@ -210,6 +210,13 @@
   return MOM_OK;
 }
 
+extern "C" int mom_live_rows_launched(mom_t *h, int *q4_jlo_full, int *q4_jlo_sub) {
+  if (!h || !q4_jlo_full || !q4_jlo_sub) return fail(h, MOM_EINVAL, "mom_live_rows_launched: null argument");
+  *q4_jlo_full = h->last_q4_jlo[0];
+  *q4_jlo_sub = h->last_q4_jlo[1];
+  return MOM_OK;
+}
+
 extern "C" int mom_check(mom_t *h) {
   if (!h) return fail(nullptr, MOM_EINVAL, "null handle");
   HIPCHK(h, hipSetDevice(h->device));
@@ -236,7 +243,10 @@
     if (value < 0 || value > 7) return fail(h, MOM_EINVAL, "mom_set_option: MOM_OPT_ZERO_SKIP takes a mask of bits 0, 1 and 2");
     h->opt_zero_skip = value;
   }
-  else if (option == MOM_OPT_SOURCES_ONLY) h->opt_sources_only = value;
+  else if (option == MOM_OPT_SOURCES_ONLY) {
+    if (value < 0 || value > 2) return fail(h, MOM_EINVAL, "mom_set_option: MOM_OPT_SOURCES_ONLY takes 0, 1 or 2");
+    h->opt_sources_only = value;
+  }
   else if (option == MOM_OPT_ELEMENTAL) h->opt_elemental = value;
   else if (option == MOM_OPT_LUT_BATCH) {
     if (value < 0) return fail(h, MOM_EINVAL, "mom_set_option: MOM_OPT_LUT_BATCH takes a number of (p, T) nodes >= 0 (0 = the default of 64)");
diff --git a/radiativetransfer.jl_amd/csrc/momcore_q4.hip b/radiativetransfer.jl_amd/csrc/momcore_q4.hip
--- a/radiativetransfer.jl_amd/csrc/momcore_q4.hip
+++ b/radiativetransfer.jl_amd/csrc/momcore_q4.hip
@@ -12,22 +12,29 @@
 
 static_assert(MOM_STRIP_KS > kQ4Skip[kSkipVariants - 1], "momcore_q4.hip: NB - 4 >= 1");
 using LayerKernel = void (*)(LayerArgs);
-static LayerKernel q4_kernel(int v, bool src, bool el) {
+constexpr int kQ4LastGroup = Q4Geom<MOM_STRIP_KS>::NJ - 1;
+static_assert(kQ4LastGroup >= 1, "momcore_q4.hip: the images have two column groups at least");
+static LayerKernel q4_kernel(int v, bool src, bool el, int jlo) {
   return mom_with_int<0, kSkipVariants - 1>(v, [&](auto V) {
     return mom_with_bool(src, [&](auto SRC) {
-      return mom_with_bool(el, [&](auto EL) -> LayerKernel { return k_layer_q4<MOM_STRIP_KS, MOM_STRIP_KS - kQ4Skip[V], SRC, EL>; });
+      return mom_with_bool(el, [&](auto EL) {
+        return mom_with_int<0, kQ4LastGroup>(jlo, [&](auto JLO) -> LayerKernel {
+          return k_layer_q4<MOM_STRIP_KS, MOM_STRIP_KS - kQ4Skip[V], SRC, EL, SRC ? (int)JLO : 0>;
+        });
+      });
     });
   });
 }
 static hipError_t image_launch(const void *layer_args, const MomLaunchForm &f, int grid, hipStream_t st) {
-  const LayerKernel k = q4_kernel(mom_skip_variant(kQ4Skip, MOM_STRIP_KS, f.nbw), f.sources_only, f.elemental_tab);
+  const int jlo = (f.sources_only && f.q4_jlo >= 1 && f.q4_jlo <= kQ4LastGroup) ? f.q4_jlo : 0;
+  const LayerKernel k = q4_kernel(mom_skip_variant(kQ4Skip, MOM_STRIP_KS, f.nbw), f.sources_only, f.elemental_tab, jlo);
   return mom_launch_lds(k, grid, 64, q4_lds_bytes(4 * MOM_STRIP_KS), st, *reinterpret_cast<const LayerArgs *>(layer_args));
 }
 static int query_per_cu() {
   const size_t smem = q4_lds_bytes(4 * MOM_STRIP_KS);
   int per_cu = 1 << 30;
-  for (int key = 0; key < 4 * kSkipVariants; ++key) {
-    const LayerKernel k = q4_kernel(key >> 2, (key & 1) != 0, (key & 2) != 0);
+  for (int key = 0; key < 4 * kSkipVariants * (kQ4LastGroup + 1); ++key) {
+    const LayerKernel k = q4_kernel((key >> 2) % kSkipVariants, (key & 1) != 0, (key & 2) != 0, (key >> 2) / kSkipVariants);
     int nb = 0;
     if (mom_allow_lds(reinterpret_cast<const void *>(k), smem) != hipSuccess ||
         hipOccupancyMaxActiveBlocksPerMultiprocessor(&nb, k, 64, smem) != hipSuccess || nb < 1)
```

After: 39770 spectral points/s (median of 6 runs). No clear change (+0.6%).
